# qirui-chen/RGA3-release

Hardware: AMD Instinct MI355X
Metric: video-QA samples/sec (fwd+bwd) at 7B/16-frame — full RGA3 training step (Qwen2.5-VL-7B + SAM2-L + mask losses + AdamW) (higher is better)
Workload: dtype bf16

## Files before the change

### include/rga3_hip.h

```cpp
#ifndef RGA3_HIP_H
#define RGA3_HIP_H

#include <stddef.h>
#include <stdint.h>

#ifdef __cplusplus
extern "C" {
#endif

#define RGA3_EINVAL (-22)

#define RGA3_BF16 0
#define RGA3_F32 1

#define RGA3_ACT_NONE 0
#define RGA3_ACT_GELU 1
#define RGA3_ACT_SWIGLU 2
#define RGA3_ACT_RELU 3

int rga3_version(void);
int rga3_last_error(char* buf, size_t n);

int rga3_gemm_bf16(const void* A, const void* W, const void* bias, const void* residual, const void* colscale, void* C, int64_t M, int64_t N,
                   int64_t K, int64_t lda, int64_t ldw, int64_t ldc, int64_t ldr, int act, int out_dtype, int tile,
                   void* workspace, int64_t workspace_bytes, void* stream);
int rga3_gemm_rms_bf16(const void* A, const void* W, const void* bias, const void* residual, void* C, int64_t M, int64_t N, int64_t K, int64_t lda,
                       int64_t ldw, int64_t ldc, int64_t ldr, int act, int tile, void* workspace, int64_t workspace_bytes, const uint64_t* row_sumsq_in,
                       int64_t norm_width, float eps, uint64_t* row_sumsq_out, void* stream);
int rga3_gemm_swiglu_pre_bf16(const void* A, const void* W, const void* bias, void* C, void* pre, int64_t M, int64_t N, int64_t K, int64_t lda, int64_t ldw,
                              int64_t ldc, int64_t ldpre, int tile, void* workspace, int64_t workspace_bytes, void* stream);
int rga3_gemm_cat_bf16(const void* A, const void* W, const void* bias, void* C, int64_t M, int64_t N, int64_t K, int64_t lda, int64_t ldw, int64_t ldc,
                       const void* A2, const void* W2, int64_t K2, int64_t lda2, int64_t ldw2, const void* Wn, void* Cn, int64_t N2, int64_t ldwn, int64_t ldcn,
                       int tile, void* stream);

int64_t rga3_gemm_workspace_bytes(void);
int rga3_gemm_tn_bf16(const void* A, const void* B, const void* bias, void* C, int64_t M, int64_t N, int64_t K, int64_t lda, int64_t ldb,
                      int64_t ldc, int out_dtype, void* workspace, int64_t workspace_bytes, void* counters, void* stream);
int rga3_gemm_tn_many(const void* const* ptrs, const int64_t* dims, int n, void* workspace, int64_t workspace_bytes, void* stream);


int rga3_attn_varlen_fwd(const void* q, const void* k, const void* v, void* o, float* lse, const int32_t* cu_q,
                         const int32_t* cu_k, int nseg, int max_q, int64_t total_q, int Hq, int Hkv, int D, int64_t q_st, int64_t q_sh,
                         int64_t k_st, int64_t k_sh, int64_t v_st, int64_t v_sh, int64_t o_st, int64_t o_sh,
                         float scale, int causal, int impl, float* split_ws, int64_t split_ws_elems, int max_k, int block_q, int block_k, void* stream);
int rga3_attn_varlen_fwd_rope(const void* q, const void* k, const void* v, void* o, float* lse, const int32_t* cu_q, const int32_t* cu_k, int nseg, int max_q,
                              int64_t total_q, int Hq, int Hkv, int D, int64_t q_st, int64_t q_sh, int64_t k_st, int64_t k_sh, int64_t v_st, int64_t v_sh,
                              int64_t o_st, int64_t o_sh, float scale, int causal, const float* cos_q, const float* sin_q, const float* cos_k,
                              const float* sin_k, void* stream);

int rga3_rmsnorm_fwd(const void* x, const void* add, const void* weight, void* y, void* res_out, int64_t rows,
                     int64_t dim, int64_t ldx, float eps, void* stream);

int rga3_layernorm_fwd(const void* x, const void* weight, const void* bias, void* y, int64_t rows, int64_t dim,
                       int64_t ldx, int64_t ldy, float eps, int act, void* stream);
int rga3_layernorm_stats(const void* x, float* stats, int64_t rows, int64_t dim, int64_t ldx, float eps, void* stream);
int rga3_gemm_ln_bf16(const void* A, const void* Wf, const void* bias, const float* colc, const float* rowstat, void* C, int64_t M, int64_t N, int64_t K,
                      int64_t lda, int64_t ldw, int64_t ldc, int act, int tile, void* stream);
int64_t rga3_gemm_lnsum_slices(int64_t N, int tile);
int rga3_gemm_lnsum_bf16(const void* A, const void* W, const void* bias, const void* residual, void* C, int64_t M, int64_t N, int64_t K, int64_t lda,
                         int64_t ldw, int64_t ldc, int64_t ldr, int tile, float* row_parts, void* stream);
int rga3_gemm_lnq_bf16(const void* A, const void* Wf, const void* bias, const float* colc, const float* row_parts, int64_t slices, int64_t norm_width, float eps,
                       void* C, int64_t M, int64_t N, int64_t K, int64_t lda, int64_t ldw, int64_t ldc, int act, int tile, void* stream);

int rga3_rope_inplace(void* x, const float* cos, const float* sin, int64_t T, int h0, int nh, int D, int64_t st,
                      int64_t sh, void* stream);

int rga3_gather_rows(const void* table, const int64_t* idx, void* out, int64_t n_idx, int64_t rows_per_idx,
                     int64_t dim, int64_t ld_table, int64_t ld_out, void* stream);
int rga3_scatter_rows(const void* src, const int64_t* idx, void* out, int64_t n_idx, int64_t rows_per_idx, int64_t dim,
                      int64_t ld_src, int64_t ld_out, void* stream);

int rga3_pad_cols(const void* src, void* dst, int64_t rows, int64_t cols, int64_t ld_src, int64_t ld_dst, void* stream);

int rga3_silu_mul(const void* a, const void* b, void* out, int64_t n, void* stream);
int rga3_add(const void* a, const void* b, void* out, int64_t n, void* stream);

int rga3_cross_entropy_rows(const void* logits, int logits_dtype, const int64_t* labels, float* row_loss,
                            void* dlogits, int64_t rows, int64_t V, int64_t ld, float grad_scale, void* stream);


int rga3_im2col(const void* img, void* out, int64_t F, int C, int H, int W, int ks, int stride, int pad, int64_t ld_out,
                void* stream);
int rga3_maxpool2x2_win(const void* x, void* y, int64_t nwin, int w, int C, int64_t ldx, int64_t ldy, void* stream);
int rga3_upsample2x_add(const void* a, const void* b, void* out, int64_t F, int H, int W, int C, void* stream);
int rga3_add_bcast(const void* a, const void* b, void* out, int64_t rows, int64_t rows_b, int C, int64_t lda, int64_t ldb,
                   int64_t ldo, float alpha, void* stream);
int rga3_bilinear(const void* in, int in_dtype, float* out, const int32_t* plane_idx, int64_t N, int Hi, int Wi, int Ho, int Wo,
                  void* stream);
int rga3_conv3x3s2(const void* x, int x_dtype, const void* w, const void* bias, void* y, int64_t F, int H, int W, int Cin, int Cout,
                   float sig_scale, float sig_bias, void* stream);
int rga3_decimg_rows(const void* keys, int64_t keys_stride, const void* pe, int64_t pe_stride, int hw, const void* kt, const void* vt, int nk, const void* wq, const void* bq,
                     const void* wo, const void* bo, const void* ln_w, const void* ln_b, float eps, const void* wk2, const void* bk2, const void* wv2, const void* bv2,
                     void* keys_out, int64_t keys_out_stride, void* k2, void* v2, int64_t kv_stride, int v2_transposed, float scale, int64_t M, void* stream);
int rga3_attn_fewq(const void* q, int64_t q_stride, const void* k, int64_t k_stride, int64_t k_head_stride, const void* vt, const void* vbias, void* out, int64_t out_stride,
                   int frames, int nq, int nk, int H, float scale, void* stream);
int rga3_copy_many(void* const* dst, const void* const* src, const int64_t* bytes, int n, void* stream);
int rga3_conv3x3s2_ln_gelu(const void* x, int x_dtype, const void* w, const void* bias, const void* ln_w, const void* ln_b, float eps, void* y, int64_t F, int H, int W,
                           int Cin, int Cout, float sig_scale, float sig_bias, void* stream);
int rga3_im2col3x3s2(const void* x, void* cols, int64_t F, int H, int W, int C, void* stream);
int rga3_dwconv7x7(const void* x, const void* w, const void* bias, void* y, int64_t F, int H, int W, int C, void* stream);
int rga3_rope_axial_inplace(void* x, const float* cos, const float* sin, int64_t n_rope, int nq, int C, int64_t ldx, void* stream);
int rga3_pixel_shuffle2x(const void* g, const void* bias, const void* add, void* out, int64_t F, int H, int W, int Co, int act, void* stream);
int rga3_bce_dice_sums(const float* logits, const float* targets, float* out4, int64_t n_masks, int64_t hw, void* stream);
int64_t rga3_bce_dice_sums_ws_floats(int64_t n_masks, int64_t hw);
int rga3_bce_dice_sums_det(const float* logits, const float* targets, float* out4, float* ws, int64_t ws_floats, int64_t n_masks, int64_t hw, void* stream);


int rga3_attn_varlen_bwd(const void* q, const void* k, const void* v, const void* o, const void* dout, const float* lse, void* dq,
                         void* dk, void* dv, float* delta_ws, const int32_t* cu_q, const int32_t* cu_k, int nseg, int max_q,
                         int max_k, int64_t total_q, int Hq, int Hkv, int D, const int64_t* strides16, float scale, int causal,
                         float* dkv_ws, int64_t total_k, void* stream);
int rga3_hiera_mlp144(const void* x, const void* w1f, const float* c1, const void* d1, const void* w2, const void* b2, void* y, int64_t M, float eps, void* stream);
int64_t rga3_hiera_mlp288_pack_bytes(void);
int rga3_hiera_mlp288_pack(const void* w1f, const float* c1, const void* d1, const void* w2, void* pack, void* stream);
int rga3_hiera_mlp288(const void* x, const void* pack, const void* b2, void* y, int64_t M, float eps, void* stream);
int rga3_mlp3_rows(const void* const* ptrs, const int64_t* dims, int n, int64_t B, void* stream);
int rga3_sam_select_objptr(const void* iou, const void* obj, const void* toks, int64_t tok_bstride, int C, const void* w0, const void* b0, const void* w1, const void* b1,
                           const void* w2, const void* b2, const void* no_obj_ptr, int64_t* best, int32_t* sel, void* obj_ptr, int64_t B, void* stream);
int64_t rga3_memattn_cross_ws_floats(int64_t Nq, int nsplit);
int rga3_memattn_cross(const void* q, const void* k, const void* m, void* out, int64_t Nq, int64_t Nk, int64_t q_stride, int64_t k_stride, int64_t m_stride,
                       int64_t out_stride, float scale, int nsplit, float* ws, void* stream);
int rga3_memlayer_rows(const void* a, int64_t a_stride, int K1, const float* part_o, const float* part_ml, int nsplit, const void* w1, const void* b1,
                       const void* res, int64_t res_stride, void* x_out, int64_t x_stride, const void* ln_w, const void* ln_b, float eps, void* t_out,
                       int64_t t_stride, const void* w2, const void* b2, int N2, void* y_out, int64_t y_stride, const float* cos, const float* sin,
                       int rope_cols, int nq, int64_t M, void* stream);
int rga3_gemm_rows16_many(const void* const* ptrs, const int64_t* dims, int n, void* stream);
int rga3_gemm_stream_k_timeouts(const void* workspace);
int64_t rga3_gemm_timeout_counter_offset(void);
int rga3_gemm_ragged_plan(int64_t M, int64_t N, int64_t K, int cus, int split, int* plan, unsigned* start);
int rga3_rmsnorm_bwd(const void* x, const void* weight, const void* dy, const void* add, void* dx, int64_t rows, int64_t dim, float eps,
                     void* stream);
int rga3_dropout_bf16(const void* x, void* y, int64_t n, float p, int64_t seed, int accumulate, void* stream);
int rga3_dropout_pair_bf16(const void* xa, const void* xb, void* ya, void* yb, int64_t n, float pa, int64_t seed_a, float pb, int64_t seed_b, int sum, void* stream);
int rga3_swiglu_fwd(const void* gu, void* a, int64_t T, int64_t I, void* stream);
int rga3_swiglu_bwd(const void* gu, const void* da, void* dgu, int64_t T, int64_t I, void* stream);
int rga3_transpose16(const void* in, void* out, int64_t R, int64_t C, int64_t ld_in, int64_t ld_out, void* stream);
int rga3_transpose16_many(const void* const* ptrs, const int64_t* dims, int n, void* stream);
int rga3_segment_sum_rows(const void* x, const int64_t* rows, const int64_t* offsets, void* out, int64_t n_out, int64_t dim, int64_t ldx,
                          void* stream);
int rga3_adamw_step(void* param, float* master, const void* grad, float* m, float* v, int64_t n, float lr, float beta1, float beta2,
                    float eps, float weight_decay, int step, float grad_scale, void* stream);
int rga3_sumsq_accum(const void* g, float* out, int64_t n, void* stream);
int rga3_sumsq_det(const void* g, int64_t n, float* partials, int64_t partials_cap, float* out, int accumulate, void* stream);
int rga3_adamw_step_clip(void* param, float* master, const void* grad, float* m, float* v, int64_t n, float lr, float beta1, float beta2,
                         float eps, float weight_decay, int step, const float* sumsq, float max_norm, void* stream);
int rga3_adamw_step_clip_rows(void* param, float* master, const void* grad, float* m, float* v, int64_t rows, int64_t row_len, const uint8_t* row_active,
                              float lr, float beta1, float beta2, float eps, int step, const float* sumsq, float max_norm, void* stream);
int rga3_scatter_add_rows(void* dst, const int64_t* idx, const void* src, int64_t n, int64_t dim, int64_t ld_dst, int64_t ld_src, float scale,
                          void* stream);


int64_t rga3_layernorm_bwd_ws_floats(int64_t rows, int64_t dim);
int rga3_layernorm_bwd(const void* x, const void* weight, const void* dy, void* dx, float* dweight, float* dbias, int64_t rows, int64_t dim,
                       float eps, float* ws, int64_t ws_floats, void* stream);
int rga3_colsum_accum(const void* x, float* out, int64_t rows, int64_t cols, int64_t ld, void* stream);
int64_t rga3_colsum_ws_floats(int64_t rows, int64_t cols);
int rga3_colsum(const void* x, float* out, int64_t rows, int64_t cols, int64_t ld, float* ws, int64_t ws_floats, void* counters, void* stream);
int rga3_act(const void* a, const void* dy, void* out, int64_t n, int kind, void* stream);
int rga3_bilinear_bwd(const float* dout, float* din, const int32_t* plane_idx, int64_t N, int Hi, int Wi, int Ho, int Wo, void* stream);
int rga3_mask_product(const void* hyper, const void* up, float* masks, int64_t B, int64_t NM, int64_t P, int64_t C, void* stream);
int64_t rga3_mask_product_bwd_ws_floats(int64_t B, int64_t NM, int64_t P, int64_t C);
int rga3_mask_product_bwd(const float* dmasks, const void* hyper, const void* up, void* dup, void* dhyper, int64_t B, int64_t NM, int64_t P, int64_t C,
                          float* ws, int64_t ws_floats, void* stream);
int rga3_pixel_shuffle2x_bwd(const void* dout, void* dg, int64_t F, int H, int W, int Co, void* stream);
int rga3_bce_dice_grad(const float* logits, const float* targets, const float* sums4, float* dlogits, int64_t n_masks, int64_t hw,
                       float coef_bce, float coef_dice, void* stream);
int rga3_bce_dice_grad_dev(const float* logits, const float* targets, const float* sums4, float* dlogits, int64_t n_masks, int64_t hw,
                           const float* coef_bce_dev, const float* coef_dice_dev, void* stream);

int rga3_pil_bicubic_coeffs(int in_size, int out_size, int32_t* bounds, int32_t* kk, int64_t kk_capacity, int* ksize_out);
int rga3_sam_preprocess_u8(const void* frames, int64_t T, int H, int W, int out_h, int out_w, const int32_t* bh, const int32_t* kh,
                           int ksize_h, const int32_t* bv, const int32_t* kv, int ksize_v, void* tmp, void* dst_u8, void* dst_bf16,
                           const float* mean3, const float* std3, void* stream);

int rga3_qwen_norm_lut(const float* mean3, const float* std3, int fused, float* lut768);
int rga3_qwen_patchify_u8(const void* frames, int64_t T, int h, int w, const float* lut768, void* out, int out_dtype, int patch, int tpatch,
                          int merge, void* stream);

int rga3_quant_fp8_rows(const void* x, void* q, float* scales, int64_t rows, int64_t K, int64_t ldx, int64_t ldq, void* stream);
int rga3_gemm_fp8(const void* Aq, const void* Wq, const float* sa, const float* sw, const void* bias, const void* residual, void* C, int64_t M,
                  int64_t N, int64_t K, int64_t lda, int64_t ldw, int64_t ldc, int64_t ldr, void* stream);
int rga3_swiglu_fwd_quant_fp8(const void* gu, void* q, float* scales, int64_t T, int64_t I, void* stream);
int rga3_swiglu_bwd_quant_fp8(const void* gu, const void* da, void* q, float* scales, int64_t T, int64_t I, void* stream);

#ifdef __cplusplus
}
#endif
#endif
```

### rga3-release_amd/csrc/attn_bwd.hip

```cpp
#include "common.h"

#include <mutex>
#include <set>

namespace rga3 {

struct AttnBwdArgs {
    const unsigned short *q, *k, *v, *o, *dout;
    unsigned short *dq, *dk, *dv;
    const float* lse;
    float* delta;
    const int *cu_q, *cu_k;
    long q_st, q_sh, k_st, k_sh, v_st, v_sh, o_st, o_sh, do_st, do_sh, dq_st, dq_sh, dk_st, dk_sh, dv_st, dv_sh;
    int Hq, Hkv, D;
    long total_q;
    float scale, scale_log2;
    int causal;
    float* dkv_ws;
    long total_k;
    int gx, gy;
};

constexpr int BT = 64;

template <int DP, int QT, int NWAVE, bool PAIR>
__global__ __launch_bounds__(64 * NWAVE) void attn_bwd_dq_kernel(AttnBwdArgs p) {
    constexpr int NT = 64 * NWAVE;
    constexpr int BLOCK_M = NWAVE * QT * 16;
    constexpr int CH = DP / 8;
    constexpr int STRIDE = DP * 2 + 32;
    constexpr int DS = DP / 32, DT = DP / 16;
    constexpr int LOADS = (BT * CH) / NT;
    static_assert((BT * CH) % NT == 0, "tile chunks must divide evenly over threads");

    extern __shared__ __attribute__((aligned(16))) char smem[];
    char* Ks = smem;
    char* Vs = smem + BT * STRIDE;

    const int tid = threadIdx.x, lane = tid & 63;
    const int wid = __builtin_amdgcn_readfirstlane(tid >> 6);
    const int g = lane >> 4, c = lane & 15;
    const Wg3 wg = xcd_decode3(p.gx, p.gy);
    const int seg = wg.z, hq = wg.y;
    const int hk = hq / (p.Hq / p.Hkv);
    const int qs = p.cu_q[seg], Lq = p.cu_q[seg + 1] - qs;
    const int ks = p.cu_k[seg], Lk = p.cu_k[seg + 1] - ks;
    const int shift = Lk - Lq;
    const int nqb = (Lq + BLOCK_M - 1) / BLOCK_M;
    int qb_first = wg.x, qb_second = -1;
    if constexpr (PAIR) {
        qb_first = nqb - 1 - wg.x;
        qb_second = wg.x;
        if (qb_second > qb_first) return;
        if (qb_second == qb_first) qb_second = -1;
    } else if (qb_first >= nqb) {
        return;
    }
    for (int pass = 0; pass < (PAIR ? 2 : 1); ++pass) {
    const int qbi = pass == 0 ? qb_first : qb_second;
    if (qbi < 0) break;
    if (pass == 1) __syncthreads();
    const int qb0 = qbi * BLOCK_M;
    const int qw0 = qb0 + wid * (QT * 16);

    bf16x8 qf[QT][DS], dof[QT][DS];
    float lse2[QT], dl[QT];
#pragma unroll
    for (int t = 0; t < QT; ++t) {
        const int qi = qw0 + t * 16 + c;
        const bool ok = qi < Lq;
#pragma unroll
        for (int ds = 0; ds < DS; ++ds) {
            const int d = ds * 32 + g * 8;
            u32x4 z = {0u, 0u, 0u, 0u}, y = {0u, 0u, 0u, 0u};
            if (ok && d < p.D) {
                z = *(const u32x4*)(p.q + (long)(qs + qi) * p.q_st + (long)hq * p.q_sh + d);
                y = *(const u32x4*)(p.dout + (long)(qs + qi) * p.do_st + (long)hq * p.do_sh + d);
            }
            qf[t][ds] = __builtin_bit_cast(bf16x8, z);
            dof[t][ds] = __builtin_bit_cast(bf16x8, y);
        }
        lse2[t] = ok ? p.lse[(long)hq * p.total_q + qs + qi] * 1.4426950408889634f : 0.f;
    }
#pragma unroll
    for (int t = 0; t < QT; ++t) {
        const int qi = qw0 + t * 16 + c;
        const bool ok = qi < Lq;
        float dp = 0.f;
#pragma unroll
        for (int ds = 0; ds < DS; ++ds) {
            const int d = ds * 32 + g * 8;
            if (ok && d < p.D) {
                const u32x4 ov = *(const u32x4*)(p.o + (long)(qs + qi) * p.o_st + (long)hq * p.o_sh + d);
                const u32x4 dv = __builtin_bit_cast(u32x4, dof[t][ds]);
#pragma unroll
                for (int i = 0; i < 4; ++i) {
                    dp += __uint_as_float(ov[i] << 16) * __uint_as_float(dv[i] << 16);
                    dp += __uint_as_float(ov[i] & 0xffff0000u) * __uint_as_float(dv[i] & 0xffff0000u);
                }
            }
        }
        dp += __shfl_xor(dp, 16, 64);
        dp += __shfl_xor(dp, 32, 64);
        dl[t] = ok ? dp : 0.f;
        if (ok && g == 0) p.delta[(long)hq * p.total_q + qs + qi] = dp;
    }

    f32x4 dqacc[QT][DT];
#pragma unroll
    for (int t = 0; t < QT; ++t)
#pragma unroll
        for (int d = 0; d < DT; ++d) dqacc[t][d] = f32x4{0.f, 0.f, 0.f, 0.f};

    int kv_end = Lk;
    if (p.causal) kv_end = min(Lk, qb0 + BLOCK_M + shift);
    if (kv_end < 0) kv_end = 0;
    const int ntiles = (kv_end + BT - 1) / BT;

    u32x4 kreg[LOADS], vreg[LOADS];
    auto load_tile = [&](int kt) {
#pragma unroll
        for (int i = 0; i < LOADS; ++i) {
            const int idx = tid + i * NT;
            const int r = idx / CH, ch = idx % CH;
            const int key = kt * BT + r;
            u32x4 zk = {0u, 0u, 0u, 0u}, zv = {0u, 0u, 0u, 0u};
            if (key < Lk && ch * 8 < p.D) {
                zk = *(const u32x4*)(p.k + (long)(ks + key) * p.k_st + (long)hk * p.k_sh + ch * 8);
                zv = *(const u32x4*)(p.v + (long)(ks + key) * p.v_st + (long)hk * p.v_sh + ch * 8);
            }
            kreg[i] = zk;
            vreg[i] = zv;
        }
    };
    auto store_tile = [&]() {
#pragma unroll
        for (int i = 0; i < LOADS; ++i) {
            const int idx = tid + i * NT;
            const int r = idx / CH, ch = idx % CH;
            *(u32x4*)(Ks + r * STRIDE + ch * 16) = kreg[i];
            *(u32x4*)(Vs + r * STRIDE + ch * 16) = vreg[i];
        }
    };

    if (ntiles > 0) load_tile(0);
    for (int kt = 0; kt < ntiles; ++kt) {
        __syncthreads();
        store_tile();
        __syncthreads();
        if (kt + 1 < ntiles) load_tile(kt + 1);
        const int k0 = kt * BT;
        const bool need_mask = (k0 + BT > Lk) || (p.causal && (k0 + BT - 1 > qb0 + shift));
#pragma unroll
        for (int t = 0; t < QT; ++t) {
            const int qi = qw0 + t * 16 + c;
            f32x4 s[4], dp[4];
#pragma unroll
            for (int j = 0; j < 4; ++j) { s[j] = f32x4{0.f, 0.f, 0.f, 0.f}; dp[j] = f32x4{0.f, 0.f, 0.f, 0.f}; }
#pragma unroll
            for (int j = 0; j < 4; ++j)
#pragma unroll
                for (int ds = 0; ds < DS; ++ds) {
                    bf16x8 kf = *(const bf16x8*)(Ks + (j * 16 + c) * STRIDE + ds * 64 + g * 16);
                    bf16x8 vf = *(const bf16x8*)(Vs + (j * 16 + c) * STRIDE + ds * 64 + g * 16);
                    s[j] = __builtin_amdgcn_mfma_f32_16x16x32_bf16(kf, qf[t][ds], s[j], 0, 0, 0);
                    dp[j] = __builtin_amdgcn_mfma_f32_16x16x32_bf16(vf, dof[t][ds], dp[j], 0, 0, 0);
                }
            bf16x8 dsf[2];
#pragma unroll
            for (int ss = 0; ss < 2; ++ss) {
                float e[8];
#pragma unroll
                for (int u = 0; u < 8; ++u) {
                    const int j = 2 * ss + (u >> 2), r = u & 3;
                    float pr = __builtin_amdgcn_exp2f(s[j][r] * p.scale_log2 - lse2[t]);
                    if (need_mask) {
                        const int key = k0 + j * 16 + 4 * g + r;
                        const bool ok = (key < Lk) && (!p.causal || key <= qi + shift);
                        pr = ok ? pr : 0.f;
                    }
                    if (qi >= Lq) pr = 0.f;
                    e[u] = pr * (dp[j][r] - dl[t]) * p.scale;
                }
                u32x4 pk;
                pk[0] = pack_bf2(e[0], e[1]); pk[1] = pack_bf2(e[2], e[3]); pk[2] = pack_bf2(e[4], e[5]); pk[3] = pack_bf2(e[6], e[7]);
                dsf[ss] = __builtin_bit_cast(bf16x8, pk);
            }
#pragma unroll
            for (int d = 0; d < DT; ++d)
#pragma unroll
                for (int ss = 0; ss < 2; ++ss) {
                    const char* a0 = Ks + (ss * 32 + 4 * g + (c >> 2)) * STRIDE + (d * 16 + 4 * (c & 3)) * 2;
                    bf16x4 lo = __builtin_amdgcn_ds_read_tr16_b64_v4bf16((__attribute__((address_space(3))) bf16x4*)(a0));
                    bf16x4 hi = __builtin_amdgcn_ds_read_tr16_b64_v4bf16((__attribute__((address_space(3))) bf16x4*)(a0 + 16 * STRIDE));
                    bf16x8 kt8;
                    kt8[0] = lo[0]; kt8[1] = lo[1]; kt8[2] = lo[2]; kt8[3] = lo[3];
                    kt8[4] = hi[0]; kt8[5] = hi[1]; kt8[6] = hi[2]; kt8[7] = hi[3];
                    dqacc[t][d] = __builtin_amdgcn_mfma_f32_16x16x32_bf16(kt8, dsf[ss], dqacc[t][d], 0, 0, 0);
                }
        }
    }
#pragma unroll
    for (int t = 0; t < QT; ++t) {
        const int qi = qw0 + t * 16 + c;
        if (qi < Lq) {
            unsigned short* row = p.dq + (long)(qs + qi) * p.dq_st + (long)hq * p.dq_sh;
#pragma unroll
            for (int d = 0; d < DT; ++d) {
                const int dd = d * 16 + 4 * g;
                if (dd < p.D) {
                    u32x2 pk;
                    pk[0] = pack_bf2(dqacc[t][d][0], dqacc[t][d][1]);
                    pk[1] = pack_bf2(dqacc[t][d][2], dqacc[t][d][3]);
                    *(u32x2*)(row + dd) = pk;
                }
            }
        }
    }
    }
}

template <int DP, int NWAVE, bool SPLIT, bool PAIR>
__global__ __launch_bounds__(64 * NWAVE) void attn_bwd_dkv_kernel(AttnBwdArgs p) {
    constexpr int NT = 64 * NWAVE;
    constexpr int BLOCK_N = NWAVE * 16;
    constexpr int CH = DP / 8;
    constexpr int STRIDE = DP * 2 + 32;
    constexpr int DS = DP / 32, DT = DP / 16;
    constexpr int LOADS = (BT * CH) / NT;
    static_assert((BT * CH) % NT == 0, "tile chunks must divide evenly over threads");

    extern __shared__ __attribute__((aligned(16))) char smem[];
    char* Qs = smem;
    char* Os = smem + BT * STRIDE;
    float* Ls = (float*)(smem + 2 * BT * STRIDE);

    const int tid = threadIdx.x, lane = tid & 63;
    const int wid = __builtin_amdgcn_readfirstlane(tid >> 6);
    const int g = lane >> 4, c = lane & 15;
    const Wg3 wg = xcd_decode3(p.gx, p.gy);
    const int seg = wg.z;
    const int group = p.Hq / p.Hkv;
    const int hk = SPLIT ? wg.y / group : wg.y;
    const int hh0 = SPLIT ? wg.y % group : 0, hh1 = SPLIT ? hh0 + 1 : group;
    const int qs = p.cu_q[seg], Lq = p.cu_q[seg + 1] - qs;
    const int ks = p.cu_k[seg], Lk = p.cu_k[seg + 1] - ks;
    const int shift = Lk - Lq;
    const int nkb = (Lk + BLOCK_N - 1) / BLOCK_N;
    int kb_first = wg.x, kb_second = -1;
    if constexpr (PAIR) {
        kb_first = wg.x;
        kb_second = nkb - 1 - wg.x;
        if (kb_first > kb_second) return;
        if (kb_second == kb_first) kb_second = -1;
    } else if (kb_first >= nkb) {
        return;
    }
    for (int pass = 0; pass < (PAIR ? 2 : 1); ++pass) {
    const int kbi = pass == 0 ? kb_first : kb_second;
    if (kbi < 0) break;
    if (pass == 1) __syncthreads();
    const int kb0 = kbi * BLOCK_N;
    const int key = kb0 + wid * 16 + c;

    bf16x8 kf[DS], vf[DS];
#pragma unroll
    for (int ds = 0; ds < DS; ++ds) {
        const int d = ds * 32 + g * 8;
        u32x4 z = {0u, 0u, 0u, 0u}, y = {0u, 0u, 0u, 0u};
        if (key < Lk && d < p.D) {
            z = *(const u32x4*)(p.k + (long)(ks + key) * p.k_st + (long)hk * p.k_sh + d);
            y = *(const u32x4*)(p.v + (long)(ks + key) * p.v_st + (long)hk * p.v_sh + d);
        }
        kf[ds] = __builtin_bit_cast(bf16x8, z);
        vf[ds] = __builtin_bit_cast(bf16x8, y);
    }
    f32x4 dkacc[DT], dvacc[DT];
#pragma unroll
    for (int d = 0; d < DT; ++d) { dkacc[d] = f32x4{0.f, 0.f, 0.f, 0.f}; dvacc[d] = f32x4{0.f, 0.f, 0.f, 0.f}; }

    int q_begin = 0;
    if (p.causal) q_begin = max(0, kb0 - shift);
    const int t0 = q_begin / BT;
    const int ntq = (Lq + BT - 1) / BT;

    u32x4 qreg[LOADS], oreg[LOADS];
    float lreg = 0.f, dreg = 0.f;
    auto load_tile = [&](int hq_, int qt_) {
#pragma unroll
        for (int i = 0; i < LOADS; ++i) {
            const int idx = tid + i * NT;
            const int r = idx / CH, ch = idx % CH;
            const int qi = qt_ * BT + r;
            u32x4 zq = {0u, 0u, 0u, 0u}, zo = {0u, 0u, 0u, 0u};
            if (qi < Lq && ch * 8 < p.D) {
                zq = *(const u32x4*)(p.q + (long)(qs + qi) * p.q_st + (long)hq_ * p.q_sh + ch * 8);
                zo = *(const u32x4*)(p.dout + (long)(qs + qi) * p.do_st + (long)hq_ * p.do_sh + ch * 8);
            }
            qreg[i] = zq;
            oreg[i] = zo;
        }
        if (tid < BT) {
            const int qi = qt_ * BT + tid;
            lreg = (qi < Lq) ? p.lse[(long)hq_ * p.total_q + qs + qi] * 1.4426950408889634f : 0.f;
            dreg = (qi < Lq) ? p.delta[(long)hq_ * p.total_q + qs + qi] : 0.f;
        }
    };
    auto store_tile = [&]() {
#pragma unroll
        for (int i = 0; i < LOADS; ++i) {
            const int idx = tid + i * NT;
            const int r = idx / CH, ch = idx % CH;
            *(u32x4*)(Qs + r * STRIDE + ch * 16) = qreg[i];
            *(u32x4*)(Os + r * STRIDE + ch * 16) = oreg[i];
        }
        if (tid < BT) {
            Ls[tid] = lreg;
            Ls[BT + tid] = dreg;
        }
    };
    if (t0 < ntq) load_tile(hk * group + hh0, t0);
    for (int hh = hh0; hh < hh1; ++hh) {
        const int hq = hk * group + hh;
        for (int qt = t0; qt < ntq; ++qt) {
            __syncthreads();
            store_tile();
            __syncthreads();
            if (qt + 1 < ntq) load_tile(hq, qt + 1);
            else if (hh + 1 < hh1) load_tile(hq + 1, t0);
            const int q0 = qt * BT;
            f32x4 s[4], dp[4];
#pragma unroll
            for (int j = 0; j < 4; ++j) { s[j] = f32x4{0.f, 0.f, 0.f, 0.f}; dp[j] = f32x4{0.f, 0.f, 0.f, 0.f}; }
#pragma unroll
            for (int j = 0; j < 4; ++j)
#pragma unroll
                for (int ds = 0; ds < DS; ++ds) {
                    bf16x8 qa = *(const bf16x8*)(Qs + (j * 16 + c) * STRIDE + ds * 64 + g * 16);
                    bf16x8 oa = *(const bf16x8*)(Os + (j * 16 + c) * STRIDE + ds * 64 + g * 16);
                    s[j] = __builtin_amdgcn_mfma_f32_16x16x32_bf16(qa, kf[ds], s[j], 0, 0, 0);
                    dp[j] = __builtin_amdgcn_mfma_f32_16x16x32_bf16(oa, vf[ds], dp[j], 0, 0, 0);
                }
            bf16x8 pf[2], dsf[2];
#pragma unroll
            for (int ss = 0; ss < 2; ++ss) {
                float e[8], f[8];
#pragma unroll
                for (int u = 0; u < 8; ++u) {
                    const int j = 2 * ss + (u >> 2), r = u & 3;
                    const int ql = j * 16 + 4 * g + r;
                    const int qi = q0 + ql;
                    float pr = __builtin_amdgcn_exp2f(s[j][r] * p.scale_log2 - Ls[ql]);
                    const bool ok = (qi < Lq) && (key < Lk) && (!p.causal || key <= qi + shift);
                    pr = ok ? pr : 0.f;
                    e[u] = pr;
                    f[u] = pr * (dp[j][r] - Ls[BT + ql]) * p.scale;
                }
                u32x4 a, b;
                a[0] = pack_bf2(e[0], e[1]); a[1] = pack_bf2(e[2], e[3]); a[2] = pack_bf2(e[4], e[5]); a[3] = pack_bf2(e[6], e[7]);
                b[0] = pack_bf2(f[0], f[1]); b[1] = pack_bf2(f[2], f[3]); b[2] = pack_bf2(f[4], f[5]); b[3] = pack_bf2(f[6], f[7]);
                pf[ss] = __builtin_bit_cast(bf16x8, a);
                dsf[ss] = __builtin_bit_cast(bf16x8, b);
            }
#pragma unroll
            for (int d = 0; d < DT; ++d)
#pragma unroll
                for (int ss = 0; ss < 2; ++ss) {
                    const int roff = (ss * 32 + 4 * g + (c >> 2)) * STRIDE + (d * 16 + 4 * (c & 3)) * 2;
                    bf16x4 ol = __builtin_amdgcn_ds_read_tr16_b64_v4bf16((__attribute__((address_space(3))) bf16x4*)(Os + roff));
                    bf16x4 oh = __builtin_amdgcn_ds_read_tr16_b64_v4bf16((__attribute__((address_space(3))) bf16x4*)(Os + roff + 16 * STRIDE));
                    bf16x4 ql_ = __builtin_amdgcn_ds_read_tr16_b64_v4bf16((__attribute__((address_space(3))) bf16x4*)(Qs + roff));
                    bf16x4 qh_ = __builtin_amdgcn_ds_read_tr16_b64_v4bf16((__attribute__((address_space(3))) bf16x4*)(Qs + roff + 16 * STRIDE));
                    bf16x8 ot, qt8;
                    ot[0] = ol[0]; ot[1] = ol[1]; ot[2] = ol[2]; ot[3] = ol[3]; ot[4] = oh[0]; ot[5] = oh[1]; ot[6] = oh[2]; ot[7] = oh[3];
                    qt8[0] = ql_[0]; qt8[1] = ql_[1]; qt8[2] = ql_[2]; qt8[3] = ql_[3]; qt8[4] = qh_[0]; qt8[5] = qh_[1]; qt8[6] = qh_[2]; qt8[7] = qh_[3];
                    dvacc[d] = __builtin_amdgcn_mfma_f32_16x16x32_bf16(ot, pf[ss], dvacc[d], 0, 0, 0);
                    dkacc[d] = __builtin_amdgcn_mfma_f32_16x16x32_bf16(qt8, dsf[ss], dkacc[d], 0, 0, 0);
                }
        }
    }
    if constexpr (SPLIT) {
        if (key < Lk) {
            const long half = (long)group * p.total_k * p.Hkv * p.D;
            float* wk = p.dkv_ws + (((long)hh0 * p.total_k + ks + key) * p.Hkv + hk) * p.D;
#pragma unroll
            for (int d = 0; d < DT; ++d) {
                const int dd = d * 16 + 4 * g;
                if (dd < p.D) {
                    *(f32x4*)(wk + dd) = dkacc[d];
                    *(f32x4*)(wk + half + dd) = dvacc[d];
                }
            }
        }
        continue;
    }
    if (key < Lk) {
        unsigned short* rk = p.dk + (long)(ks + key) * p.dk_st + (long)hk * p.dk_sh;
        unsigned short* rv = p.dv + (long)(ks + key) * p.dv_st + (long)hk * p.dv_sh;
#pragma unroll
        for (int d = 0; d < DT; ++d) {
            const int dd = d * 16 + 4 * g;
            if (dd < p.D) {
                u32x2 a, b;
                a[0] = pack_bf2(dkacc[d][0], dkacc[d][1]); a[1] = pack_bf2(dkacc[d][2], dkacc[d][3]);
                b[0] = pack_bf2(dvacc[d][0], dvacc[d][1]); b[1] = pack_bf2(dvacc[d][2], dvacc[d][3]);
                *(u32x2*)(rk + dd) = a;
                *(u32x2*)(rv + dd) = b;
            }
        }
    }
    }
}

__global__ __launch_bounds__(256) void attn_dkv_reduce_kernel(AttnBwdArgs p) {
    const int group = p.Hq / p.Hkv;
    const int d4 = p.D / 4;
    const long idx = (long)blockIdx.x * 256 + threadIdx.x;
    const long total = p.total_k * p.Hkv * d4;
    if (idx >= total) return;
    const int dd = (int)(idx % d4) * 4;
    const long row = idx / d4;
    const int hk = (int)(row % p.Hkv);
    const long key = row / p.Hkv;
    const long plane = p.total_k * p.Hkv * (long)p.D, half = (long)group * plane;
    const float* w = p.dkv_ws + row * p.D + dd;
    f32x4 sk = *(const f32x4*)w, sv = *(const f32x4*)(w + half);
    for (int h = 1; h < group; ++h) {
        sk += *(const f32x4*)(w + h * plane);
        sv += *(const f32x4*)(w + half + h * plane);
    }
    u32x2 a, b;
    a[0] = pack_bf2(sk[0], sk[1]); a[1] = pack_bf2(sk[2], sk[3]);
    b[0] = pack_bf2(sv[0], sv[1]); b[1] = pack_bf2(sv[2], sv[3]);
    *(u32x2*)(p.dk + key * p.dk_st + (long)hk * p.dk_sh + dd) = a;
    *(u32x2*)(p.dv + key * p.dv_st + (long)hk * p.dv_sh + dd) = b;
}

template <int DP>
static int launch_bwd(const AttnBwdArgs& a0, int nseg, int max_q, int max_k, hipStream_t st) {
    AttnBwdArgs a = a0;
    a.gx = 1; a.gy = 1;
    constexpr int NW = (DP == 128) ? 8 : 4;
#ifdef RGA3_BWD_DQ_QT2
    constexpr int QT = 2, NWQ = 4;
#else
    constexpr int QT = (DP >= 128) ? 1 : 2, NWQ = NW;
#endif
    constexpr int BLOCK_M = NWQ * QT * 16;
    constexpr int LDS_DQ = 2 * BT * (DP * 2 + 32);
    constexpr int LDS_DKV = 2 * BT * (DP * 2 + 32) + 2 * BT * 4;
    auto prep = [](const void* k, int lds) -> int {
        if (lds <= 48 * 1024) return 0;
        static std::mutex mu;
        static std::set<std::pair<const void*, int>> done;
        int dev = 0;
        if (hipGetDevice(&dev) != hipSuccess) dev = 0;
        std::lock_guard<std::mutex> lk(mu);
        if (done.count({k, dev})) return 0;
        hipError_t e = hipFuncSetAttribute(k, hipFuncAttributeMaxDynamicSharedMemorySize, lds);
        if (e != hipSuccess) return fail(-(int)e, "attn_bwd: hipFuncSetAttribute: %s", hipGetErrorString(e));
        done.insert({k, dev});
        return 0;
    };
    const unsigned nqb = (unsigned)cdiv(max_q, BLOCK_M), nkb = (unsigned)cdiv(max_k, 16 * NW);
    const bool pair = a.causal && nqb >= 4 && nkb >= 4;
    if (pair) {
        auto kq = attn_bwd_dq_kernel<DP, QT, NWQ, true>;
        if (int rc = prep((const void*)kq, LDS_DQ)) return rc;
        a.gx = (int)((nqb + 1) / 2); a.gy = a.Hq;
        hipLaunchKernelGGL(kq, dim3((unsigned)a.gx * (unsigned)a.gy * (unsigned)nseg), dim3(64 * NWQ), LDS_DQ, st, a);
    } else {
        auto kq = attn_bwd_dq_kernel<DP, QT, NWQ, false>;
        if (int rc = prep((const void*)kq, LDS_DQ)) return rc;
        a.gx = (int)nqb; a.gy = a.Hq;
        hipLaunchKernelGGL(kq, dim3((unsigned)a.gx * (unsigned)a.gy * (unsigned)nseg), dim3(64 * NWQ), LDS_DQ, st, a);
    }
    RGA3_CHECK_LAUNCH("attn_bwd_dq_kernel");
    const unsigned gx = pair ? (nkb + 1) / 2 : nkb;
    if (a.dkv_ws && a.Hq > a.Hkv) {
        if (pair) {
            auto ks_ = attn_bwd_dkv_kernel<DP, NW, true, true>;
            if (int rc = prep((const void*)ks_, LDS_DKV)) return rc;
            a.gx = (int)gx; a.gy = a.Hq;
            hipLaunchKernelGGL(ks_, dim3((unsigned)a.gx * (unsigned)a.gy * (unsigned)nseg), dim3(64 * NW), LDS_DKV, st, a);
        } else {
            auto ks_ = attn_bwd_dkv_kernel<DP, NW, true, false>;
            if (int rc = prep((const void*)ks_, LDS_DKV)) return rc;
            a.gx = (int)gx; a.gy = a.Hq;
            hipLaunchKernelGGL(ks_, dim3((unsigned)a.gx * (unsigned)a.gy * (unsigned)nseg), dim3(64 * NW), LDS_DKV, st, a);
        }
        RGA3_CHECK_LAUNCH("attn_bwd_dkv_kernel<split>");
        const long rows = a.total_k * a.Hkv;
        hipLaunchKernelGGL(attn_dkv_reduce_kernel, dim3((unsigned)cdiv(rows * (a.D / 4), 256)), dim3(256), 0, st, a);
        RGA3_CHECK_LAUNCH("attn_dkv_reduce_kernel");
        return 0;
    }
    if (pair) {
        auto kk = attn_bwd_dkv_kernel<DP, NW, false, true>;
        if (int rc = prep((const void*)kk, LDS_DKV)) return rc;
        a.gx = (int)gx; a.gy = a.Hkv;
        hipLaunchKernelGGL(kk, dim3((unsigned)a.gx * (unsigned)a.gy * (unsigned)nseg), dim3(64 * NW), LDS_DKV, st, a);
    } else {
        auto kk = attn_bwd_dkv_kernel<DP, NW, false, false>;
        if (int rc = prep((const void*)kk, LDS_DKV)) return rc;
        a.gx = (int)gx; a.gy = a.Hkv;
        hipLaunchKernelGGL(kk, dim3((unsigned)a.gx * (unsigned)a.gy * (unsigned)nseg), dim3(64 * NW), LDS_DKV, st, a);
    }
    RGA3_CHECK_LAUNCH("attn_bwd_dkv_kernel");
    return 0;
}

}

using namespace rga3;

extern "C" int rga3_attn_varlen_bwd(const void* q, const void* k, const void* v, const void* o, const void* dout, const float* lse,
                                    void* dq, void* dk, void* dv, float* delta_ws, const int32_t* cu_q, const int32_t* cu_k, int nseg,
                                    int max_q, int max_k, int64_t total_q, int Hq, int Hkv, int D, const int64_t* strides16, float scale,
                                    int causal, float* dkv_ws, int64_t total_k, void* stream) {
    RGA3_CHECK_ARG(q && k && v && o && dout && lse && dq && dk && dv && delta_ws && cu_q && cu_k && strides16, "attn_bwd: null pointer");
    RGA3_CHECK_ARG(nseg > 0 && max_q > 0 && max_k > 0 && total_q > 0, "attn_bwd: sizes");
    RGA3_CHECK_ARG(Hq > 0 && Hkv > 0 && Hq % Hkv == 0, "attn_bwd: Hq=%d Hkv=%d", Hq, Hkv);
    RGA3_CHECK_ARG(D >= 8 && D <= 128 && D % 8 == 0, "attn_bwd: head dim %d unsupported (multiple of 8, <= 128)", D);
    for (int i = 0; i < 16; ++i) RGA3_CHECK_ARG(strides16[i] % 4 == 0, "attn_bwd: stride %d must be a multiple of 4 elements", i);
    for (int i = 0; i < 10; ++i) RGA3_CHECK_ARG(strides16[i] % 8 == 0, "attn_bwd: input stride %d must be a multiple of 8 elements", i);
    AttnBwdArgs a;
    a.q = (const unsigned short*)q; a.k = (const unsigned short*)k; a.v = (const unsigned short*)v; a.o = (const unsigned short*)o;
    a.dout = (const unsigned short*)dout; a.dq = (unsigned short*)dq; a.dk = (unsigned short*)dk; a.dv = (unsigned short*)dv;
    a.lse = lse; a.delta = delta_ws; a.cu_q = cu_q; a.cu_k = cu_k;
    a.q_st = strides16[0]; a.q_sh = strides16[1]; a.k_st = strides16[2]; a.k_sh = strides16[3]; a.v_st = strides16[4]; a.v_sh = strides16[5];
    a.o_st = strides16[6]; a.o_sh = strides16[7]; a.do_st = strides16[8]; a.do_sh = strides16[9]; a.dq_st = strides16[10]; a.dq_sh = strides16[11];
    a.dk_st = strides16[12]; a.dk_sh = strides16[13]; a.dv_st = strides16[14]; a.dv_sh = strides16[15];
    a.Hq = Hq; a.Hkv = Hkv; a.D = D; a.total_q = total_q; a.scale = scale; a.scale_log2 = scale * 1.4426950408889634f; a.causal = causal;
    a.dkv_ws = dkv_ws; a.total_k = total_k;
    RGA3_CHECK_ARG(!dkv_ws || (total_k > 0 && D % 4 == 0), "attn_bwd: dkv_ws needs total_k");
    hipStream_t st = (hipStream_t)stream;
    if (D <= 32) return launch_bwd<32>(a, nseg, max_q, max_k, st);
    if (D <= 64) return launch_bwd<64>(a, nseg, max_q, max_k, st);
    if (D <= 96) return launch_bwd<96>(a, nseg, max_q, max_k, st);
    return launch_bwd<128>(a, nseg, max_q, max_k, st);
}
```

### rga3-release_amd/csrc/gemm_bf16.hip

```cpp
#include "common.h"
#include "act_table.h"
#include <cstdlib>
#include <type_traits>
#include <utility>

namespace rga3 {


enum { ACT_NONE = 0, ACT_GELU = 1, ACT_SWIGLU = 2, ACT_RELU = 3 };

struct GemmArgs {
    const unsigned short* A;
    const unsigned short* W;
    void* C;
    const unsigned short* bias;
    const unsigned short* res;
    const unsigned short* colscale;
    int M, N, K;
    long lda, ldw, ldc, ldr;
    int ntm, ntn;
    int group_m;
    void* ws;
    long ws_bytes;
    const float* rowstat;
    const float* colc;
    int ksl;
    const unsigned long long* rs_in = nullptr;
    float rs_in_scale = 0.f;
    float rs_eps = 0.f;
    unsigned long long* rs_out = nullptr;
    float* ln_parts = nullptr;
    const float* ln_in = nullptr;
    int ln_ns = 0;
    const unsigned short* A2 = nullptr;
    const unsigned short* W2 = nullptr;
    long lda2 = 0, ldw2 = 0;
    int K2 = 0;
    unsigned short* pre = nullptr;
    long ldpre = 0;
    const unsigned short* Wn = nullptr;
    void* Cn = nullptr;
    long ldwn = 0, ldcn = 0;
    int N2 = 0;
};

constexpr float kRowSumFix = 1048576.0f;

__device__ const u32x4 g_zero16 = {0u, 0u, 0u, 0u};

__device__ __forceinline__ float gelu_erf(float x) {
    const float z = fabsf(x) * 0.70710678118654752f;
    const float t = __builtin_amdgcn_rcpf(1.0f + 0.3275911f * z);
    float poly = 1.061405429f;
    poly = poly * t - 1.453152027f;
    poly = poly * t + 1.421413741f;
    poly = poly * t - 0.284496736f;
    poly = poly * t + 0.254829592f;
    const float e = 1.0f - poly * t * __expf(-z * z);
    return 0.5f * x + 0.5f * fabsf(x) * e;
}
__device__ __forceinline__ float silu_f(float x) { return x * __builtin_amdgcn_rcpf(1.0f + __expf(-x)); }

template <int ACT> constexpr bool act_uses_table() { return ACT == ACT_GELU || ACT == ACT_SWIGLU; }

__device__ __forceinline__ f32x2 splat2(float s) {
    f32x2 v = {s, s};
    asm volatile("" : "+v"(v));
    return v;
}
__device__ __forceinline__ f32x2 widen_bf2(unsigned pk) { return f32x2{__uint_as_float(pk << 16), __uint_as_float(pk & 0xffff0000u)}; }
template <int NWAVES>
__device__ __forceinline__ void stage_act_table(char* dst, int which, int wid, int lane) {
    const char* src = (const char*)g_act_tab[which] + lane * 16;
#pragma unroll
    for (int pc = 0; pc < kActTabBytes / 1024; pc += NWAVES) {
        const int q = pc + wid;
        if (q < kActTabBytes / 1024) __builtin_amdgcn_global_load_lds((gbl_void*)(src + q * 1024), (lds_void*)(dst + q * 1024), 16, 0, 0);
    }
}

template <int NTL, int ACT, bool OUT_F32>
constexpr int epi_wave_bytes() {
    return 1024;
}

template <int ACT, bool OUT_F32>
constexpr bool pp_res_lds() { return ACT == ACT_NONE && !OUT_F32; }
template <int MT, int OW>
constexpr int res_stage_bytes() { return ((MT * 16 * (OW / 8 + 1) * 16 + 1023) / 1024) * 1024; }

template <int MT, int OW>
__device__ __forceinline__ void stage_residual(const GemmArgs& p, char* dst, int row0, int col0, int lane) {
    constexpr int CPR = OW / 8, CPRP = CPR + 1, SLOTS = MT * 16 * CPRP, NI = (SLOTS + 63) / 64;
#pragma unroll
    for (int k = 0; k < NI; ++k) {
        const int sl = min(k * 64 + lane, SLOTS - 1);
        const int row = sl / CPRP, ch = min(sl - row * CPRP, CPR - 1);
        const unsigned short* src = p.res + (long)min(row0 + row, p.M - 1) * p.ldr + col0 + ch * 8;
        __builtin_amdgcn_global_load_lds((gbl_void*)src, (lds_void*)(dst + k * 1024), 16, 0, 0);
    }
}
template <int OW, bool OUT_F32>
__device__ __forceinline__ bool residual_stageable(const GemmArgs& p, int col0, int Nout) {
    return !OUT_F32 && p.res && col0 + OW <= Nout && (p.ldr & 7) == 0 && (p.ldc & 7) == 0 && ((((size_t)p.res) & 15) == 0);
}

template <int MT, int NTL, int WTM, int WTN, int ACT, bool OUT_F32, int LNM = 0, bool PARTS = false>
__device__ __forceinline__ void gemm_epilogue(f32x4 (&acc)[MT][NTL], const GemmArgs& p, char* est, const char* tab, int lane, int m0, int n0,
                                              int wm, int wn, const f32x4* part1 = nullptr, const f32x4* part2 = nullptr, const char* resl = nullptr,
                                              float poison = 0.f, int nwn = 1) {
    constexpr bool LNF = LNM == 1, LNP = LNM == 2;
    static_assert(!(LNM != 0 && ACT == ACT_SWIGLU), "the LayerNorm-folded epilogues have no SwiGLU form");
    static_assert(!(LNP && (OUT_F32 || PARTS)), "the LayerNorm-sum producer writes bf16 from the single-pass kernels");
    constexpr int PD = 1;
    f32x4 pn[PD][NTL];
    auto load_part = [&](int i) {
#pragma unroll
        for (int j = 0; j < NTL; ++j) {
            f32x4 v = part1[(i * NTL + j) * 64];
            if (part2) v += part2[(i * NTL + j) * 64];
            v += f32x4{poison, poison, poison, poison};
            pn[i % PD][j] = v;
        }
    };
    if constexpr (PARTS) {
        load_part(0);
        if (PD > 1 && MT > 1) load_part(1);
    }
    auto load4 = [&](const unsigned short* v, int col, int n) -> u32x2 {
        u32x2 r;
        if (col + 3 < n && (((size_t)(v + col)) & 7) == 0) {
            r = *(const u32x2*)(v + col);
        } else {
            const unsigned a0 = v[min(col, n - 1)], a1 = v[min(col + 1, n - 1)], a2 = v[min(col + 2, n - 1)], a3 = v[min(col + 3, n - 1)];
            r[0] = a0 | (a1 << 16);
            r[1] = a2 | (a3 << 16);
        }
        return r;
    };
    auto pick = [](const u32x2& pk, int r) -> float { return __uint_as_float((r & 1) ? (pk[r >> 1] & 0xffff0000u) : (pk[r >> 1] << 16)); };
    u32x2 bpk[NTL];
    f32x4 cc[LNF ? NTL : 1];
    {
        const int g4 = (lane >> 4) * 4;
        if (p.bias) {
            if (n0 + wn * WTN + NTL * 16 <= p.N && (((size_t)p.bias) & 7) == 0) {
#pragma unroll
                for (int j = 0; j < NTL; ++j) bpk[j] = *(const u32x2*)(p.bias + n0 + wn * WTN + j * 16 + g4);
            } else {
#pragma unroll
                for (int j = 0; j < NTL; ++j) bpk[j] = load4(p.bias, n0 + wn * WTN + j * 16 + g4, p.N);
            }
        }
        if constexpr (LNF) {
#pragma unroll
            for (int j = 0; j < NTL; ++j) {
                const int col = n0 + wn * WTN + j * 16 + g4;
                cc[j] = (col + 3 < p.N) ? *(const f32x4*)(p.colc + col) : f32x4{0.f, 0.f, 0.f, 0.f};
            }
        }
    }

    constexpr int OUT_NT = (ACT == ACT_SWIGLU) ? NTL / 2 : NTL;
    constexpr int OW = OUT_NT * 16;
    constexpr int ESZ = OUT_F32 ? 4 : 2;
    constexpr int EDAT = OW * ESZ;
    constexpr int EROW = EDAT + 16;
    const int g = lane >> 4, c = lane & 15;
    const int ncol0 = (ACT == ACT_SWIGLU) ? (n0 / 2 + wn * OW) : (n0 + wn * OW);
    const int Nout = (ACT == ACT_SWIGLU) ? p.N / 2 : p.N;

    float* const rs_lds = (float*)est;
    const unsigned tb = act_uses_table<ACT>() ? act_tab_base(tab) : 0u;
    if constexpr (LNF) {
        if (p.ln_in) {
            const double sc = (double)p.rs_in_scale;
#pragma unroll
            for (int q = 0; q < (MT * 16 + 63) / 64; ++q) {
                const int rl = lane + 64 * q;
                if (rl < MT * 16) {
                    const float2* pp = (const float2*)p.ln_in + (long)min(m0 + wm * WTM + rl, p.M - 1) * p.ln_ns;
                    double sx = 0.0, sxx = 0.0;
                    for (int k = 0; k < p.ln_ns; ++k) {
                        const float2 v = pp[k];
                        sx += (double)v.x;
                        sxx += (double)v.y;
                    }
                    const double mean = sx * sc;
                    const double var = fmax(sxx * sc - mean * mean, 0.0);
                    *(float2*)(rs_lds + 2 * rl) = make_float2((float)mean, __builtin_amdgcn_rsqf((float)var + p.rs_eps));
                }
            }
        } else {
#pragma unroll
            for (int q = 0; q < (MT * 16 + 63) / 64; ++q) {
                const int rl = lane + 64 * q;
                if (rl < MT * 16) *(float2*)(rs_lds + 2 * rl) = *(const float2*)(p.rowstat + 2L * min(m0 + wm * WTM + rl, p.M - 1));
            }
        }
    }
    if (p.rs_in) {
#pragma unroll
        for (int q = 0; q < (MT * 16 + 63) / 64; ++q) {
            const int rl = lane + 64 * q;
            if (rl < MT * 16) {
                const uint2 raw = *(const uint2*)(p.rs_in + min(m0 + wm * WTM + rl, p.M - 1));
                rs_lds[rl] = __builtin_amdgcn_rsqf(__builtin_fmaf((float)raw.y, 4294967296.0f, (float)raw.x) * p.rs_in_scale + p.rs_eps);
            }
        }
    }
    if (resl) asm volatile("s_waitcnt vmcnt(0)" ::: "memory");
#pragma unroll
    for (int i = 0; i < MT; ++i) {
        f32x4 x[NTL];
#pragma unroll
        for (int j = 0; j < NTL; ++j) {
            x[j] = acc[i][j];
            if constexpr (PARTS) x[j] += pn[i % PD][j];
        }
        if constexpr (PARTS) {
            if (i + PD < MT) load_part(i + PD);
        }
        if constexpr (LNF) {
            const float2 st2 = *(const float2*)(rs_lds + 2 * (i * 16 + (lane & 15)));
            const float ln_rinv = st2.y, nmr = -st2.x * st2.y;
            const f32x2 ri2 = splat2(ln_rinv), nm2 = splat2(nmr);
#pragma unroll
            for (int j = 0; j < NTL; ++j) {
                const f32x2 lo = x[j].xy * ri2 + cc[j].xy * nm2, hi = x[j].zw * ri2 + cc[j].zw * nm2;
                x[j] = f32x4{lo[0], lo[1], hi[0], hi[1]};
            }
        } else if (p.rs_in) {
            const float rs_rinv = rs_lds[i * 16 + (lane & 15)];
            const f32x2 rs2 = splat2(rs_rinv);
#pragma unroll
            for (int j = 0; j < NTL; ++j) {
                const f32x2 lo = x[j].xy * rs2, hi = x[j].zw * rs2;
                x[j] = f32x4{lo[0], lo[1], hi[0], hi[1]};
            }
        }
        if (p.bias) {
#pragma unroll
            for (int j = 0; j < NTL; ++j)
                x[j] += f32x4{__uint_as_float(bpk[j][0] << 16), __uint_as_float(bpk[j][0] & 0xffff0000u), __uint_as_float(bpk[j][1] << 16),
                              __uint_as_float(bpk[j][1] & 0xffff0000u)};
        }
        f32x4 v[OUT_NT];
#pragma unroll
        for (int jo = 0; jo < OUT_NT; ++jo) {
            if constexpr (ACT == ACT_SWIGLU) {
                const f32x4 &gq = x[2 * jo], &uq = x[2 * jo + 1];
                const unsigned pg0 = pack_bf2(gq[0], gq[1]), pg1 = pack_bf2(gq[2], gq[3]), pu0 = pack_bf2(uq[0], uq[1]), pu1 = pack_bf2(uq[2], uq[3]);
                const f32x2 s01 = act_tab2(pg0, tb), s23 = act_tab2(pg1, tb);
                const f32x2 v01 = widen_bf2(pack_bf2(s01[0], s01[1])) * widen_bf2(pu0);
                const f32x2 v23 = widen_bf2(pack_bf2(s23[0], s23[1])) * widen_bf2(pu1);
                v[jo] = f32x4{v01[0], v01[1], v23[0], v23[1]};
                if (p.pre) {
                    const auto q0 = __builtin_amdgcn_permlane16_swap(pg0, pu0, false, false);
                    const auto q1 = __builtin_amdgcn_permlane16_swap(pg1, pu1, false, false);
                    const u32x4 pv = {(unsigned)q0[0], (unsigned)q1[0], (unsigned)q0[1], (unsigned)q1[1]};
                    const int prow = m0 + wm * WTM + i * 16 + (lane & 15);
                    const int pcol = n0 + wn * WTN + ((g & 1) ? (2 * jo + 1) * 16 + 4 * (g - 1) : 2 * jo * 16 + 4 * g);
                    if (prow < p.M && pcol < p.N) {
                        unsigned short* dp = p.pre + (long)prow * p.ldpre + pcol;
                        if (pcol + 8 <= p.N && (p.ldpre & 7) == 0) {
                            *(u32x4*)dp = pv;
                        } else {
                            for (int e = 0; e < 8 && pcol + e < p.N; ++e) dp[e] = (unsigned short)(pv[e >> 1] >> (16 * (e & 1)));
                        }
                    }
                }
            } else if constexpr (ACT == ACT_GELU) {
                const f32x2 y01 = act_tab2(pack_bf2(x[jo][0], x[jo][1]), tb), y23 = act_tab2(pack_bf2(x[jo][2], x[jo][3]), tb);
                v[jo] = f32x4{y01[0], y01[1], y23[0], y23[1]};
            } else if constexpr (ACT == ACT_RELU) {
#pragma unroll
                for (int r = 0; r < 4; ++r) v[jo][r] = fmaxf(x[jo][r], 0.f);
            } else {
                v[jo] = x[jo];
            }
        }
        if (p.colscale) {
#pragma unroll
            for (int jo = 0; jo < OUT_NT; ++jo)
#pragma unroll
                for (int r = 0; r < 4; ++r) {
                    const float cs = bf2f(p.colscale[min(ncol0 + jo * 16 + 4 * g + r, Nout - 1)]);
                    v[jo][r] = ((ACT == ACT_SWIGLU) ? v[jo][r] : bf2f(f2bf(v[jo][r]))) * cs;
                }
        }
        u32x2 pk[OUT_NT];
        f32x4 vf[OUT_F32 ? OUT_NT : 1];
#pragma unroll
        for (int jo = 0; jo < OUT_NT; ++jo) {
            if constexpr (OUT_F32) {
                vf[jo] = v[jo];
            } else {
                pk[jo][0] = pack_bf2(v[jo][0], v[jo][1]);
                pk[jo][1] = pack_bf2(v[jo][2], v[jo][3]);
            }
        }
        const int row = m0 + wm * WTM + i * 16 + c;
        const bool row_ok = row < p.M;
        if constexpr (OUT_F32) {
#pragma unroll
            for (int jo = 0; jo < OUT_NT; ++jo) {
                const int col = ncol0 + jo * 16 + 4 * g;
                if (row_ok && col < Nout) {
                    float* dst = (float*)p.C + (long)row * p.ldc + col;
                    if (col + 4 <= Nout && ((p.ldc & 3) == 0)) {
                        *(f32x4*)dst = vf[jo];
                    } else {
                        for (int e = 0; e < 4 && col + e < Nout; ++e) dst[e] = vf[jo][e];
                    }
                }
            }
        } else {
            float rs_ss = 0.f, rs_s = 0.f;
#pragma unroll
            for (int jo = 0; jo + 1 < OUT_NT; jo += 2) {
                const auto r0 = __builtin_amdgcn_permlane16_swap(pk[jo][0], pk[jo + 1][0], false, false);
                const auto r1 = __builtin_amdgcn_permlane16_swap(pk[jo][1], pk[jo + 1][1], false, false);
                u32x4 val = {(unsigned)r0[0], (unsigned)r1[0], (unsigned)r0[1], (unsigned)r1[1]};
                const int col = ncol0 + ((g & 1) ? (jo + 1) * 16 + 4 * (g - 1) : jo * 16 + 4 * g);
                if (row_ok && col < Nout) {
                    unsigned short* dst = (unsigned short*)p.C + (long)row * p.ldc + col;
                    const bool vec = (col + 8 <= Nout) && ((p.ldc & 7) == 0);
                    if (p.res) {
                        const unsigned short* rs = p.res + (long)row * p.ldr + col;
                        u32x4 rv;
                        if (resl) {
                            rv = *(const u32x4*)(resl + (((i * 16 + c) * (OW / 8 + 1) + ((col - ncol0) >> 3)) << 4));
                        } else if (vec && ((p.ldr & 7) == 0) && ((((size_t)p.res) & 15) == 0)) {
                            rv = *(const u32x4*)rs;
                        } else {
#pragma unroll
                            for (int e = 0; e < 4; ++e) {
                                const unsigned lo = (col + 2 * e < Nout) ? rs[2 * e] : 0u, hi = (col + 2 * e + 1 < Nout) ? rs[2 * e + 1] : 0u;
                                rv[e] = lo | (hi << 16);
                            }
                        }
#pragma unroll
                        for (int e = 0; e < 4; ++e)
                            val[e] = pack_bf2(__uint_as_float(val[e] << 16) + __uint_as_float(rv[e] << 16),
                                              __uint_as_float(val[e] & 0xffff0000u) + __uint_as_float(rv[e] & 0xffff0000u));
                    }
                    if (vec) {
                        *(u32x4*)dst = val;
                    } else {
                        for (int e = 0; e < 8 && col + e < Nout; ++e) dst[e] = (unsigned short)(val[e >> 1] >> (16 * (e & 1)));
                    }
                    if (LNP || p.rs_out) {
#pragma unroll
                        for (int e = 0; e < 8; ++e) {
                            const float v1 = (col + e < Nout) ? __uint_as_float((e & 1) ? (val[e >> 1] & 0xffff0000u) : (val[e >> 1] << 16)) : 0.f;
                            rs_ss = __builtin_fmaf(v1, v1, rs_ss);
                            if constexpr (LNP) rs_s += v1;
                        }
                    }
                }
            }
            if constexpr (OUT_NT % 2 == 1) {
            const int col = ncol0 + (OUT_NT - 1) * 16 + 4 * g;
            if (row_ok && col < Nout) {
                u32x2 val = pk[OUT_NT - 1];
                unsigned short* dst = (unsigned short*)p.C + (long)row * p.ldc + col;
                if (p.res && resl) {
                    const u32x2 rv = *(const u32x2*)(resl + (((i * 16 + c) * (OW / 8 + 1) + ((col - ncol0) >> 3)) << 4) + (((col - ncol0) & 4) << 1));
#pragma unroll
                    for (int e = 0; e < 2; ++e)
                        val[e] = pack_bf2(__uint_as_float(val[e] << 16) + __uint_as_float(rv[e] << 16), __uint_as_float(val[e] & 0xffff0000u) + __uint_as_float(rv[e] & 0xffff0000u));
                } else if (p.res) {
                    const unsigned short* rs = p.res + (long)row * p.ldr + col;
#pragma unroll
                    for (int e = 0; e < 2; ++e) {
                        const float lo = (col + 2 * e < Nout) ? bf2f(rs[2 * e]) : 0.f, hi = (col + 2 * e + 1 < Nout) ? bf2f(rs[2 * e + 1]) : 0.f;
                        val[e] = pack_bf2(__uint_as_float(val[e] << 16) + lo, __uint_as_float(val[e] & 0xffff0000u) + hi);
                    }
                }
                if (col + 4 <= Nout && ((p.ldc & 3) == 0)) {
                    *(u32x2*)dst = val;
                } else {
                    for (int e = 0; e < 4 && col + e < Nout; ++e) dst[e] = (unsigned short)(val[e >> 1] >> (16 * (e & 1)));
                }
                if (LNP || p.rs_out) {
#pragma unroll
                    for (int e = 0; e < 4; ++e) {
                        const float v1 = (col + e < Nout) ? __uint_as_float((e & 1) ? (val[e >> 1] & 0xffff0000u) : (val[e >> 1] << 16)) : 0.f;
                        rs_ss = __builtin_fmaf(v1, v1, rs_ss);
                        if constexpr (LNP) rs_s += v1;
                    }
                }
            }
            }
            if constexpr (LNP) {
                rs_ss += __shfl_xor(rs_ss, 16, 64);
                rs_ss += __shfl_xor(rs_ss, 32, 64);
                rs_s += __shfl_xor(rs_s, 16, 64);
// ... 1855 lines not shown
    __syncthreads();
    if (w != 0) return;
    f32x4 v = red[0][lane];
#pragma unroll
    for (int i = 1; i < R16_NW; ++i) v += red[i][lane];
    const int col = n0 + 4 * g;
    if (c >= p.M || col >= p.N) return;
    unsigned short* dst = (unsigned short*)p.C + (long)c * p.ldc + col;
#pragma unroll
    for (int r = 0; r < 4; ++r) {
        if (col + r >= p.N) break;
        float x = v[r];
        if (p.bias) x += bf2f(p.bias[col + r]);
        if constexpr (ACT == ACT_GELU) x = gelu_erf(bf2f(f2bf(x)));
        if constexpr (ACT == ACT_RELU) x = fmaxf(x, 0.f);
        if (p.res) x = bf2f(f2bf(x)) + bf2f(p.res[(long)c * p.ldr + col + r]);
        dst[r] = f2bf(x);
    }
}

constexpr int R16_MAXSETS = 4;
struct Rows16Set {
    const unsigned short *A, *A2, *W, *bias, *res;
    unsigned short* C;
    int M, N, K, act;
    long lda, lda2, ldw, ldc, ldr;
};
struct Rows16Many { Rows16Set s[R16_MAXSETS]; };

__global__ __launch_bounds__(64 * R16_NW) void gemm_rows16_many_kernel(Rows16Many P) {
    __shared__ f32x4 red[R16_NW][64];
    const Rows16Set& p = P.s[blockIdx.y];
    const int n0 = blockIdx.x * 16;
    if (n0 >= p.N) return;
    const int lane = threadIdx.x & 63, w = threadIdx.x >> 6;
    const int c = lane & 15, g = lane >> 4;
    const unsigned short* arow = p.W + (long)min(n0 + c, p.N - 1) * p.ldw + g * 8;
    const unsigned short* brow = p.A + (long)min(c, p.M - 1) * p.lda + g * 8;
    const unsigned short* brow2 = p.A2 ? p.A2 + (long)min(c, p.M - 1) * p.lda2 + g * 8 : nullptr;
    const int nks = (p.K + 31) >> 5;
    f32x4 acc = {0.f, 0.f, 0.f, 0.f};
    for (int ks0 = w; ks0 < nks; ks0 += R16_NW * R16_U) {
        bf16x8 af[R16_U], bf[R16_U];
#pragma unroll
        for (int u = 0; u < R16_U; ++u) {
            const int k = (ks0 + u * R16_NW) * 32 + g * 8;
            u32x4 za = {0u, 0u, 0u, 0u}, zb = {0u, 0u, 0u, 0u};
            if (k < p.K) {
                za = *(const u32x4*)(arow + (ks0 + u * R16_NW) * 32);
                zb = *(const u32x4*)(brow + (ks0 + u * R16_NW) * 32);
                if (brow2) {
                    const u32x4 z2 = *(const u32x4*)(brow2 + (ks0 + u * R16_NW) * 32);
#pragma unroll
                    for (int e = 0; e < 4; ++e)
                        zb[e] = pack_bf2(__uint_as_float(zb[e] << 16) + __uint_as_float(z2[e] << 16), __uint_as_float(zb[e] & 0xffff0000u) + __uint_as_float(z2[e] & 0xffff0000u));
                }
            }
            af[u] = __builtin_bit_cast(bf16x8, za);
            bf[u] = __builtin_bit_cast(bf16x8, zb);
        }
#pragma unroll
        for (int u = 0; u < R16_U; ++u) acc = __builtin_amdgcn_mfma_f32_16x16x32_bf16(af[u], bf[u], acc, 0, 0, 0);
    }
    red[w][lane] = acc;
    __syncthreads();
    if (w != 0) return;
    f32x4 v = red[0][lane];
#pragma unroll
    for (int i = 1; i < R16_NW; ++i) v += red[i][lane];
    const int col = n0 + 4 * g;
    if (c >= p.M || col >= p.N) return;
    unsigned short* dst = p.C + (long)c * p.ldc + col;
#pragma unroll
    for (int r = 0; r < 4; ++r) {
        if (col + r >= p.N) break;
        float x = v[r];
        if (p.bias) x += bf2f(p.bias[col + r]);
        if (p.act == ACT_GELU) x = gelu_erf(bf2f(f2bf(x)));
        if (p.act == ACT_RELU) x = fmaxf(x, 0.f);
        if (p.res) x = bf2f(f2bf(x)) + bf2f(p.res[(long)c * p.ldr + col + r]);
        dst[r] = f2bf(x);
    }
}

template <int ACT, bool OUT_F32>
static int launch_rows16(const GemmArgs& a, hipStream_t st) {
    if constexpr (OUT_F32 || ACT == ACT_SWIGLU) {
        return fail(-1, "gemm: tile 41 (token rows) writes bf16 and has no SwiGLU form");
    } else {
        hipLaunchKernelGGL(gemm_rows16_kernel<ACT>, dim3((unsigned)cdiv(a.N, 16)), dim3(64 * R16_NW), 0, st, a);
        RGA3_CHECK_LAUNCH("gemm_rows16_kernel");
        return 0;
    }
}

static int pick_tile(int M, int N, int K, bool plain, int forced) {
    if (forced >= 0) return forced;
    if (plain && K >= 8192 && cdiv(M, 256) * cdiv(N, 256) <= 4 && K % 64 == 0) return 25;
    struct Cfg { int bm, bn, slots; double prior; };
    static const Cfg cfgs[3] = {{256, 256, 1, 1.00}, {256, 128, 1, 0.90}, {128, 128, 2, 0.78}};
    int best = 0;
    double bs = -1;
    for (int i = 0; i < 3; ++i) {
        double tiles = (double)cdiv(M, cfgs[i].bm) * (double)cdiv(N, cfgs[i].bn);
        double cap = 256.0 * cfgs[i].slots;
        double waves = (double)cdiv((int64_t)tiles, (int64_t)cap);
        double fill = tiles / (waves * cap);
        double useful = ((double)M * N) / (tiles * cfgs[i].bm * cfgs[i].bn);
        double s = fill * useful * cfgs[i].prior;
        if (s > bs) { bs = s; best = i; }
    }
    static const int ids[3] = {20, 11, 12};
    return ids[best];
}

template <int ACT, bool OUT_F32>
static int launch_act(const GemmArgs& a, int tile, hipStream_t st) {
    switch (tile) {
        case 3: return launch_cfg<128, 256, 2, 4, ACT, OUT_F32, 0>(a, st);
        case 4:
            if constexpr (ACT != ACT_SWIGLU) return launch_cfg<128, 320, 2, 4, ACT, OUT_F32, 0>(a, st);
            else return launch_cfg<128, 256, 2, 4, ACT, OUT_F32, 0>(a, st);
        case 5:
            if constexpr (ACT != ACT_SWIGLU) return launch_cfg<128, 192, 2, 4, ACT, OUT_F32, 0>(a, st);
            else return launch_cfg<128, 256, 2, 4, ACT, OUT_F32, 0>(a, st);
        case 6: return launch_cfg<128, 256, 2, 4, ACT, OUT_F32, 3>(a, st);
        case 7:
            if constexpr (ACT != ACT_SWIGLU) return launch_cfg<128, 192, 2, 4, ACT, OUT_F32, 3>(a, st);
            else return launch_cfg<128, 256, 2, 4, ACT, OUT_F32, 3>(a, st);
        case 8: return launch_cfg<128, 128, 2, 2, ACT, OUT_F32, 3>(a, st);
        case 10: return launch_cfg<256, 256, 2, 4, ACT, OUT_F32, 0>(a, st);
        case 13: return launch_cfg<64, 64, 2, 2, ACT, OUT_F32, 0>(a, st);
        case 14:
            if constexpr (ACT == ACT_NONE) return launch_split64<OUT_F32>(a, st);
            else return launch_cfg<64, 64, 2, 2, ACT, OUT_F32, 0>(a, st);
        case 20: return launch_pp<ACT, OUT_F32>(a, st);
        case 23:
            if constexpr (ACT == ACT_NONE) return launch_pp<ACT, OUT_F32, false, true>(a, st);
            else return launch_pp<ACT, OUT_F32>(a, st);
        case 21: return launch_sk<ACT, OUT_F32>(a, false, st);
        case 22: return launch_sk<ACT, OUT_F32>(a, true, st);
        case 26: return launch_sk<ACT, OUT_F32>(a, true, st, true);
        case 27: return launch_sk<ACT, OUT_F32>(a, false, st, true);
        case 31: return launch_sk<ACT, OUT_F32, 3>(a, false, st);
        case 32: return launch_sk<ACT, OUT_F32, 3>(a, true, st);
        case 25: return launch_splitk<ACT, OUT_F32>(a, st);
        case 28: return launch_w4<ACT, OUT_F32>(a, st);
        case 40: return launch_gemv<ACT, OUT_F32>(a, st);
        case 41: return launch_rows16<ACT, OUT_F32>(a, st);
        default: return launch_cfg<128, 128, 2, 2, ACT, OUT_F32, 0>(a, st);
    }
}

}

using namespace rga3;

extern "C" int rga3_gemm_rows16_many(const void* const* ptrs, const int64_t* dims, int n, void* stream) {
    RGA3_CHECK_ARG(ptrs && dims && n >= 1 && n <= R16_MAXSETS, "gemm_rows16_many: n %d (1..%d)", n, R16_MAXSETS);
    Rows16Many P;
    int64_t maxn = 0;
    for (int i = 0; i < n; ++i) {
        Rows16Set& s = P.s[i];
        const void* const* q = ptrs + 6 * i;
        const int64_t* d = dims + 9 * i;
        s.A = (const unsigned short*)q[0]; s.A2 = (const unsigned short*)q[1]; s.W = (const unsigned short*)q[2]; s.bias = (const unsigned short*)q[3];
        s.res = (const unsigned short*)q[4]; s.C = (unsigned short*)q[5];
        s.M = (int)d[0]; s.N = (int)d[1]; s.K = (int)d[2]; s.act = (int)d[3]; s.lda = d[4]; s.lda2 = d[5]; s.ldw = d[6]; s.ldc = d[7]; s.ldr = d[8];
        RGA3_CHECK_ARG(s.A && s.W && s.C && s.M >= 1 && s.M <= 16 && s.N >= 1 && s.K >= 8 && s.K % 8 == 0, "gemm_rows16_many: set %d: M %d (1..16), N %d, K %d", i, s.M, s.N, s.K);
        RGA3_CHECK_ARG(s.lda % 8 == 0 && s.ldw % 8 == 0 && (!s.A2 || s.lda2 % 8 == 0), "gemm_rows16_many: set %d: strides must be multiples of 8", i);
        RGA3_CHECK_ARG((((uintptr_t)s.A | (uintptr_t)s.A2 | (uintptr_t)s.W) & 15) == 0, "gemm_rows16_many: set %d: 16-byte alignment", i);
        RGA3_CHECK_ARG(s.act == ACT_NONE || s.act == ACT_GELU || s.act == ACT_RELU, "gemm_rows16_many: set %d: act %d", i, s.act);
        RGA3_CHECK_ARG(s.ldc >= s.N && (!s.res || s.ldr >= s.N), "gemm_rows16_many: set %d: ldc %ld / ldr %ld shorter than N %d (a residual row stride below N reads out of bounds)",
                       i, (long)s.ldc, (long)s.ldr, s.N);
        if (s.N > maxn) maxn = s.N;
    }
    hipLaunchKernelGGL(gemm_rows16_many_kernel, dim3((unsigned)cdiv(maxn, 16), (unsigned)n), dim3(64 * R16_NW), 0, (hipStream_t)stream, P);
    RGA3_CHECK_LAUNCH("gemm_rows16_many_kernel");
    return 0;
}

extern "C" int64_t rga3_gemm_workspace_bytes(void) {
    const int cus = cu_count();
    return cus > 0 ? (int64_t)(kSkFlagBytes + (size_t)cus * 512 * 32 * 16) : 0;
}

extern "C" int rga3_gemm_stream_k_timeouts(const void* workspace) {
    SkWorkspace ws;
    if (sk_workspace((void*)workspace, (int64_t)1 << 40, ws)) return -1;
    unsigned v = 0;
    if (hipDeviceSynchronize() != hipSuccess || hipMemcpy(&v, ws.flags + ws.P, sizeof(v), hipMemcpyDeviceToHost) != hipSuccess) return -1;
    return (int)(v > 0x7fffffffu ? 0x7fffffffu : v);
}

extern "C" int rga3_gemm_ragged_plan(int64_t M, int64_t N, int64_t K, int cus, int split, int* plan, unsigned* start) {
    RGA3_CHECK_ARG(M > 0 && N > 0 && K > 0 && K % 64 == 0 && cus > 0 && cus <= kSkMaxP && plan && start, "gemm_ragged_plan: M, N > 0, K a multiple of 64, 0 < cus <= %d", kSkMaxP);
    GemmArgs a{};
    a.M = (int)M; a.N = (int)N; a.K = (int)K;
    a.ntm = (int)cdiv(M, 256);
    a.ntn = (int)cdiv(N, 256);
    for (int i = 0; i < 8; ++i) plan[i] = 0;
    if (a.ntm < 2 || M - (int64_t)(a.ntm - 1) * 256 > 64) return 1;
    a.group_m = pick_group_m(a.ntm - 1, 256);
    SkArgs sk;
    if (!sk_plan_ragged(sk, a, (int)(K / 64), cus, split != 0)) return 1;
    plan[0] = sk.t_dp; plan[1] = sk.sk_tiles; plan[2] = sk.ragged; plan[3] = sk.rg_wgs; plan[4] = 0; plan[5] = sk.P; plan[6] = sk.P_sk; plan[7] = a.group_m;
    for (int w = 0; w <= cus; ++w) start[w] = sk.start[w];
    return 0;
}

extern "C" int64_t rga3_gemm_timeout_counter_offset(void) {
    const int cus = cu_count();
    if (cus <= 0 || cus * 4 + 16 > (int)kSkFlagBytes) return -1;
    return (int64_t)cus * 4;
}

static int gemm_bf16_impl(const void* A, const void* W, const void* bias, const void* residual, const void* colscale, void* C,
                          int64_t M, int64_t N, int64_t K, int64_t lda, int64_t ldw, int64_t ldc, int64_t ldr,
                          int act, int out_dtype, int tile, void* workspace, int64_t workspace_bytes, const unsigned long long* rs_in, int64_t rs_width, float rs_eps,
                          unsigned long long* rs_out, void* stream, void* pre = nullptr, int64_t ldpre = 0);

extern "C" int rga3_gemm_bf16(const void* A, const void* W, const void* bias, const void* residual, const void* colscale, void* C,
                              int64_t M, int64_t N, int64_t K, int64_t lda, int64_t ldw, int64_t ldc, int64_t ldr,
                              int act, int out_dtype, int tile, void* workspace, int64_t workspace_bytes, void* stream) {
    return gemm_bf16_impl(A, W, bias, residual, colscale, C, M, N, K, lda, ldw, ldc, ldr, act, out_dtype, tile, workspace, workspace_bytes, nullptr, 0, 0.f, nullptr, stream);
}

extern "C" int rga3_gemm_rms_bf16(const void* A, const void* W, const void* bias, const void* residual, void* C, int64_t M, int64_t N, int64_t K, int64_t lda,
                                  int64_t ldw, int64_t ldc, int64_t ldr, int act, int tile, void* workspace, int64_t workspace_bytes, const uint64_t* row_sumsq_in,
                                  int64_t norm_width, float eps, uint64_t* row_sumsq_out, void* stream) {
    RGA3_CHECK_ARG(row_sumsq_in || row_sumsq_out, "gemm_rms: neither row_sumsq_in nor row_sumsq_out given (use rga3_gemm_bf16)");
    RGA3_CHECK_ARG(!row_sumsq_in || (norm_width > 0 && eps >= 0.f), "gemm_rms: norm_width %ld eps %g", (long)norm_width, (double)eps);
    RGA3_CHECK_ARG((((uintptr_t)row_sumsq_in | (uintptr_t)row_sumsq_out) & 7) == 0, "gemm_rms: row sums must be 8-byte aligned");
    RGA3_CHECK_ARG(tile != 14 && tile != 25 && tile != 40 && tile != 41, "gemm_rms: tile %d has its own epilogue", tile);
    RGA3_CHECK_ARG(M > 16, "gemm_rms: M %ld (token-row products take the unfused route)", (long)M);
    return gemm_bf16_impl(A, W, bias, residual, nullptr, C, M, N, K, lda, ldw, ldc, ldr, act, RGA3_BF16, tile, workspace, workspace_bytes,
                          (const unsigned long long*)row_sumsq_in, norm_width, eps, (unsigned long long*)row_sumsq_out, stream);
}

static int lnsum_tile_width(int tile) { return (tile == 3 || tile == 20) ? 256 : (tile == 5 || tile == 23) ? 192 : (tile == 13) ? 64 : 128; }
extern "C" int64_t rga3_gemm_lnsum_slices(int64_t N, int tile) {
    if (N <= 0 || !(tile == -1 || tile == 3 || tile == 5 || tile == 12 || tile == 13 || tile == 20 || tile == 23)) return -1;
    return cdiv(N, lnsum_tile_width(tile));
}
extern "C" int rga3_gemm_lnsum_bf16(const void* A, const void* W, const void* bias, const void* residual, void* C, int64_t M, int64_t N, int64_t K, int64_t lda,
                                    int64_t ldw, int64_t ldc, int64_t ldr, int tile, float* row_parts, void* stream) {
    RGA3_CHECK_ARG(A && W && C && row_parts && (((uintptr_t)row_parts) & 7) == 0, "gemm_lnsum: null pointer / row_parts must be 8-byte aligned");
    RGA3_CHECK_ARG(M > 16 && N > 0 && K > 0 && K % 8 == 0, "gemm_lnsum: bad shape M=%ld N=%ld K=%ld (M > 16, K %% 8)", (long)M, (long)N, (long)K);
    RGA3_CHECK_ARG(lda % 8 == 0 && ldw % 8 == 0, "gemm_lnsum: lda/ldw must be multiples of 8 elements (16-byte rows)");
    RGA3_CHECK_ARG((((uintptr_t)A | (uintptr_t)W | (uintptr_t)C) & 15) == 0, "gemm_lnsum: pointers must be 16-byte aligned");
    RGA3_CHECK_ARG(tile == -1 || tile == 3 || tile == 5 || tile == 12 || tile == 13 || tile == 20 || tile == 23, "gemm_lnsum: tile %d (3 / 5 / 12 / 13 / 20 / 23)", tile);
    RGA3_CHECK_ARG(M * lda < (1LL << 32) && N * ldw < (1LL << 32), "gemm_lnsum: operands must be < 2^32 elements (32-bit staging offsets)");
    GemmArgs a;
    a.A = (const unsigned short*)A; a.W = (const unsigned short*)W; a.C = C;
    a.bias = (const unsigned short*)bias; a.res = (const unsigned short*)residual; a.colscale = nullptr;
    a.M = (int)M; a.N = (int)N; a.K = (int)K;
    a.lda = lda; a.ldw = ldw; a.ldc = ldc; a.ldr = ldr;
    a.ws = nullptr; a.ws_bytes = 0; a.ksl = 0; a.rowstat = nullptr; a.colc = nullptr;
    a.ln_parts = row_parts;
    hipStream_t st = (hipStream_t)stream;
    switch (tile) {
        case 3: return launch_cfg<128, 256, 2, 4, ACT_NONE, false, 0, 2>(a, st);
        case 5: return launch_cfg<128, 192, 2, 4, ACT_NONE, false, 0, 2>(a, st);
        case 13: return launch_cfg<64, 64, 2, 2, ACT_NONE, false, 0, 2>(a, st);
        case 20: return launch_pp<ACT_NONE, false, 2, false>(a, st);
        case 23: return launch_pp<ACT_NONE, false, 2, true>(a, st);
        default: return launch_cfg<128, 128, 2, 2, ACT_NONE, false, 0, 2>(a, st);
    }
}

extern "C" int rga3_gemm_swiglu_pre_bf16(const void* A, const void* W, const void* bias, void* C, void* pre, int64_t M, int64_t N, int64_t K, int64_t lda, int64_t ldw,
                                         int64_t ldc, int64_t ldpre, int tile, void* workspace, int64_t workspace_bytes, void* stream) {
    RGA3_CHECK_ARG(pre, "gemm_swiglu_pre: null pre-activation output");
    return gemm_bf16_impl(A, W, bias, nullptr, nullptr, C, M, N, K, lda, ldw, ldc, 0, ACT_SWIGLU, RGA3_BF16, tile, workspace, workspace_bytes, nullptr, 0, 0.f, nullptr, stream, pre,
                          ldpre);
}

extern "C" int rga3_gemm_cat_bf16(const void* A, const void* W, const void* bias, void* C, int64_t M, int64_t N, int64_t K, int64_t lda, int64_t ldw, int64_t ldc,
                                  const void* A2, const void* W2, int64_t K2, int64_t lda2, int64_t ldw2, const void* Wn, void* Cn, int64_t N2, int64_t ldwn,
                                  int64_t ldcn, int tile, void* stream) {
    RGA3_CHECK_ARG(A && W && C && M > 16 && N > 0 && K > 0, "gemm_cat: bad args");
    RGA3_CHECK_ARG((A2 != nullptr) == (W2 != nullptr) && (A2 != nullptr) == (K2 > 0), "gemm_cat: the K side takes A2, W2 and K2 together");
    RGA3_CHECK_ARG((Wn != nullptr) == (Cn != nullptr) && (Wn != nullptr) == (N2 > 0), "gemm_cat: the N side takes Wn, Cn and N2 together");
    RGA3_CHECK_ARG(A2 || Wn, "gemm_cat: nothing concatenated (use rga3_gemm_bf16)");
    RGA3_CHECK_ARG(K % 64 == 0 && K2 % 64 == 0, "gemm_cat: K = %ld and K2 = %ld must be multiples of 64", (long)K, (long)K2);
    RGA3_CHECK_ARG(lda % 8 == 0 && ldw % 8 == 0 && lda2 % 8 == 0 && ldw2 % 8 == 0 && ldwn % 8 == 0 && N % 8 == 0 && N2 % 8 == 0, "gemm_cat: strides / widths must be multiples of 8 elements");
    RGA3_CHECK_ARG((((uintptr_t)A | (uintptr_t)W | (uintptr_t)C | (uintptr_t)A2 | (uintptr_t)W2 | (uintptr_t)Wn | (uintptr_t)Cn) & 15) == 0, "gemm_cat: pointer alignment");
    RGA3_CHECK_ARG(M * lda < (1LL << 32) && N * ldw < (1LL << 32) && M * (lda2 ? lda2 : 1) < (1LL << 32) && N * (ldw2 ? ldw2 : 1) < (1LL << 32) && N2 * (ldwn ? ldwn : 1) < (1LL << 32),
                   "gemm_cat: operands must be < 2^32 elements");
    const int bn = (tile == 3 || tile == 6) ? 256 : (tile == 4) ? 320 : (tile == 5) ? 192 : (tile == 13) ? 64 : 128;
    RGA3_CHECK_ARG(tile == -1 || tile == 3 || tile == 6 || tile == 12 || tile == 13 || (!Wn && (tile == 4 || tile == 5)), "gemm_cat: tile %d", tile);
    RGA3_CHECK_ARG(!Wn || N % bn == 0, "gemm_cat: with an N side, N = %ld must be a multiple of the tile width %d", (long)N, bn);
    GemmArgs a;
    a.A = (const unsigned short*)A; a.W = (const unsigned short*)W; a.C = C;
    a.bias = (const unsigned short*)bias; a.res = nullptr; a.colscale = nullptr;
    a.M = (int)M; a.N = (int)N; a.K = (int)K;
    a.lda = lda; a.ldw = ldw; a.ldc = ldc; a.ldr = 0;
    a.ws = nullptr; a.ws_bytes = 0; a.ksl = 0; a.rowstat = nullptr; a.colc = nullptr;
    a.A2 = (const unsigned short*)A2; a.W2 = (const unsigned short*)W2; a.K2 = (int)K2; a.lda2 = lda2; a.ldw2 = ldw2;
    a.Wn = (const unsigned short*)Wn; a.Cn = Cn; a.N2 = (int)N2; a.ldwn = ldwn; a.ldcn = ldcn;
    hipStream_t st = (hipStream_t)stream;
    switch (tile) {
        case 3: return launch_cfg<128, 256, 2, 4, ACT_NONE, false, 0>(a, st);
        case 4: return launch_cfg<128, 320, 2, 4, ACT_NONE, false, 0>(a, st);
        case 5: return launch_cfg<128, 192, 2, 4, ACT_NONE, false, 0>(a, st);
        case 6: return launch_cfg<128, 256, 2, 4, ACT_NONE, false, 3>(a, st);
        case 13: return launch_cfg<64, 64, 2, 2, ACT_NONE, false, 0>(a, st);
        default: return launch_cfg<128, 128, 2, 2, ACT_NONE, false, 0>(a, st);
    }
}

static int gemm_bf16_impl(const void* A, const void* W, const void* bias, const void* residual, const void* colscale, void* C,
                          int64_t M, int64_t N, int64_t K, int64_t lda, int64_t ldw, int64_t ldc, int64_t ldr,
                          int act, int out_dtype, int tile, void* workspace, int64_t workspace_bytes, const unsigned long long* rs_in, int64_t rs_width, float rs_eps,
                          unsigned long long* rs_out, void* stream, void* pre, int64_t ldpre) {
    RGA3_CHECK_ARG(A && W && C, "gemm: null pointer");
    RGA3_CHECK_ARG(!pre || (act == ACT_SWIGLU && M > 4 && tile != 40 && tile != 41 && (((uintptr_t)pre) & 15) == 0 && ldpre >= N), "gemm: the pre-activation output goes with the SwiGLU tile epilogues (M > 4)");
    RGA3_CHECK_ARG(M > 0 && N > 0 && K > 0, "gemm: bad shape M=%ld N=%ld K=%ld", (long)M, (long)N, (long)K);
    RGA3_CHECK_ARG(K % 8 == 0, "gemm: K=%ld must be a multiple of 8 (16-byte staging chunks)", (long)K);
    RGA3_CHECK_ARG(lda % 8 == 0 && ldw % 8 == 0, "gemm: lda/ldw must be multiples of 8 elements (16-byte rows)");
    RGA3_CHECK_ARG((((uintptr_t)A | (uintptr_t)W | (uintptr_t)C) & 15) == 0, "gemm: pointers must be 16-byte aligned");
    RGA3_CHECK_ARG(out_dtype == RGA3_BF16 || out_dtype == RGA3_F32, "gemm: out_dtype %d", out_dtype);
    RGA3_CHECK_ARG(act >= 0 && act <= 3, "gemm: act %d", act);
    RGA3_CHECK_ARG(!(out_dtype == RGA3_F32 && (act != ACT_NONE || residual || colscale)), "gemm: f32 output supports bias only");
    RGA3_CHECK_ARG(act != ACT_SWIGLU || N % 32 == 0, "gemm: swiglu needs N %% 32 == 0");
    RGA3_CHECK_ARG(tile == -1 || (tile >= 3 && tile <= 8) || (tile >= 10 && tile <= 14) || (tile >= 20 && tile <= 23) || tile == 25 || (tile >= 26 && tile <= 28) || tile == 31 || tile == 32 || tile == 40 || tile == 41, "gemm: tile %d", tile);
    RGA3_CHECK_ARG(M * lda < (1LL << 32) && N * ldw < (1LL << 32), "gemm: operands must be < 2^32 elements (32-bit staging offsets)");
    GemmArgs a;
    a.A = (const unsigned short*)A;
    a.W = (const unsigned short*)W;
    a.C = C;
    a.bias = (const unsigned short*)bias;
    a.res = (const unsigned short*)residual;
    a.colscale = (const unsigned short*)colscale;
    a.M = (int)M; a.N = (int)N; a.K = (int)K;
    a.lda = lda; a.ldw = ldw; a.ldc = ldc; a.ldr = ldr;
    a.ws = workspace; a.ws_bytes = workspace_bytes; a.ksl = 0; a.rowstat = nullptr; a.colc = nullptr;
    a.rs_in = rs_in; a.rs_in_scale = rs_in ? 1.0f / (kRowSumFix * (float)rs_width) : 0.f; a.rs_eps = rs_eps; a.rs_out = rs_out;
    a.pre = (unsigned short*)pre; a.ldpre = ldpre;
    hipStream_t st = (hipStream_t)stream;
    RGA3_CHECK_ARG(tile != 40 || (M <= 4 && !colscale), "gemm: the skinny kernel (tile 40) takes M <= 4 rows and no column scale");
    const bool rows16_ok = M <= 16 && !colscale && out_dtype == RGA3_BF16 && act != ACT_SWIGLU;
    RGA3_CHECK_ARG(tile != 41 || rows16_ok, "gemm: the token-row kernel (tile 41) takes M <= 16 rows, bf16 output, no column scale, no SwiGLU");
    int tl = (tile == -1 && M <= 4 && !colscale) ? 40 : (tile == -1 && rows16_ok) ? 41 : pick_tile((int)M, (int)N, (int)K, act == ACT_NONE && !residual && !colscale && !rs_in && !rs_out, tile);
    if (out_dtype == RGA3_F32) return launch_act<ACT_NONE, true>(a, tl, st);
    switch (act) {
        case ACT_NONE: return launch_act<ACT_NONE, false>(a, tl, st);
        case ACT_GELU: return launch_act<ACT_GELU, false>(a, tl, st);
        case ACT_SWIGLU: return launch_act<ACT_SWIGLU, false>(a, tl, st);
        default: return launch_act<ACT_RELU, false>(a, tl, st);
    }
}

template <int ACT>
static int launch_ln(const GemmArgs& a, int tile, hipStream_t st) {
    switch (tile) {
        case 3: return launch_cfg<128, 256, 2, 4, ACT, false, 0, true>(a, st);
        case 5: return launch_cfg<128, 192, 2, 4, ACT, false, 0, true>(a, st);
        case 6: return launch_cfg<128, 256, 2, 4, ACT, false, 3, true>(a, st);
        case 7: return launch_cfg<128, 192, 2, 4, ACT, false, 3, true>(a, st);
        case 13: return launch_cfg<64, 64, 2, 2, ACT, false, 0, true>(a, st);
        case 20: return launch_pp<ACT, false, true>(a, st);
        default: return launch_cfg<128, 128, 2, 2, ACT, false, 0, true>(a, st);
    }
}

extern "C" int rga3_gemm_ln_bf16(const void* A, const void* Wf, const void* bias, const float* colc, const float* rowstat, void* C, int64_t M, int64_t N, int64_t K,
                                 int64_t lda, int64_t ldw, int64_t ldc, int act, int tile, void* stream) {
    RGA3_CHECK_ARG(A && Wf && C && colc && rowstat, "gemm_ln: null pointer");
    RGA3_CHECK_ARG(M > 0 && N > 0 && K > 0 && K % 8 == 0 && N % 4 == 0, "gemm_ln: bad shape M=%ld N=%ld K=%ld (K %% 8, N %% 4)", (long)M, (long)N, (long)K);
    RGA3_CHECK_ARG(lda % 8 == 0 && ldw % 8 == 0, "gemm_ln: lda/ldw must be multiples of 8 elements");
    RGA3_CHECK_ARG((((uintptr_t)A | (uintptr_t)Wf | (uintptr_t)C | (uintptr_t)colc) & 15) == 0 && (((uintptr_t)rowstat) & 7) == 0, "gemm_ln: pointer alignment");
    RGA3_CHECK_ARG(act == ACT_NONE || act == ACT_GELU || act == ACT_RELU, "gemm_ln: act %d", act);
    RGA3_CHECK_ARG(tile == -1 || tile == 3 || (tile >= 5 && tile <= 7) || tile == 12 || tile == 13 || tile == 20, "gemm_ln: tile %d", tile);
    RGA3_CHECK_ARG(M * lda < (1LL << 32) && N * ldw < (1LL << 32), "gemm_ln: operands must be < 2^32 elements");
    GemmArgs a;
    a.A = (const unsigned short*)A; a.W = (const unsigned short*)Wf; a.C = C;
    a.bias = (const unsigned short*)bias; a.res = nullptr; a.colscale = nullptr;
    a.M = (int)M; a.N = (int)N; a.K = (int)K;
    a.lda = lda; a.ldw = ldw; a.ldc = ldc; a.ldr = 0;
    a.ws = nullptr; a.ws_bytes = 0; a.ksl = 0; a.rowstat = rowstat; a.colc = colc;
    hipStream_t st = (hipStream_t)stream;
    if (act == ACT_GELU) return launch_ln<ACT_GELU>(a, tile, st);
    if (act == ACT_RELU) return launch_ln<ACT_RELU>(a, tile, st);
    return launch_ln<ACT_NONE>(a, tile, st);
}

extern "C" int rga3_gemm_lnq_bf16(const void* A, const void* Wf, const void* bias, const float* colc, const float* row_parts, int64_t slices, int64_t norm_width,
                                  float eps, void* C, int64_t M, int64_t N, int64_t K, int64_t lda, int64_t ldw, int64_t ldc, int act, int tile, void* stream) {
    RGA3_CHECK_ARG(A && Wf && C && colc && row_parts, "gemm_lnq: null pointer");
    RGA3_CHECK_ARG(M > 0 && N > 0 && K > 0 && K % 8 == 0 && N % 4 == 0 && norm_width > 0 && eps >= 0.f && slices >= 1 && slices <= 4096,
                   "gemm_lnq: bad shape M=%ld N=%ld K=%ld slices=%ld (K %% 8, N %% 4)", (long)M, (long)N, (long)K, (long)slices);
    RGA3_CHECK_ARG(lda % 8 == 0 && ldw % 8 == 0, "gemm_lnq: lda/ldw must be multiples of 8 elements");
    RGA3_CHECK_ARG((((uintptr_t)A | (uintptr_t)Wf | (uintptr_t)C | (uintptr_t)colc) & 15) == 0 && (((uintptr_t)row_parts) & 7) == 0, "gemm_lnq: pointer alignment");
    RGA3_CHECK_ARG(act == ACT_NONE || act == ACT_GELU || act == ACT_RELU, "gemm_lnq: act %d", act);
    RGA3_CHECK_ARG(tile == -1 || tile == 3 || (tile >= 5 && tile <= 7) || tile == 12 || tile == 13 || tile == 20, "gemm_lnq: tile %d", tile);
    RGA3_CHECK_ARG(M * lda < (1LL << 32) && N * ldw < (1LL << 32), "gemm_lnq: operands must be < 2^32 elements");
    GemmArgs a;
    a.A = (const unsigned short*)A; a.W = (const unsigned short*)Wf; a.C = C;
    a.bias = (const unsigned short*)bias; a.res = nullptr; a.colscale = nullptr;
    a.M = (int)M; a.N = (int)N; a.K = (int)K;
    a.lda = lda; a.ldw = ldw; a.ldc = ldc; a.ldr = 0;
    a.ws = nullptr; a.ws_bytes = 0; a.ksl = 0; a.rowstat = nullptr; a.colc = colc;
    a.ln_in = row_parts; a.ln_ns = (int)slices; a.rs_in_scale = 1.0f / (float)norm_width; a.rs_eps = eps;
    hipStream_t st = (hipStream_t)stream;
    if (act == ACT_GELU) return launch_ln<ACT_GELU>(a, tile, st);
    if (act == ACT_RELU) return launch_ln<ACT_RELU>(a, tile, st);
    return launch_ln<ACT_NONE>(a, tile, st);
}

extern "C" int rga3_gemm_tn_bf16(const void* A, const void* B, const void* bias, void* C, int64_t M, int64_t N, int64_t K, int64_t lda,
                                 int64_t ldb, int64_t ldc, int out_dtype, void* workspace, int64_t workspace_bytes, void* counters, void* stream) {
    RGA3_CHECK_ARG(A && B && C, "gemm_tn: null pointer");
    RGA3_CHECK_ARG(M >= 8 && N >= 8 && K > 0 && M % 8 == 0 && N % 8 == 0, "gemm_tn: bad shape M=%ld N=%ld K=%ld (M, N multiples of 8)", (long)M, (long)N, (long)K);
    RGA3_CHECK_ARG(lda % 8 == 0 && ldb % 8 == 0 && ldc % 4 == 0, "gemm_tn: lda/ldb must be multiples of 8 elements, ldc of 4");
    RGA3_CHECK_ARG((((uintptr_t)A | (uintptr_t)B | (uintptr_t)C | (uintptr_t)workspace) & 15) == 0, "gemm_tn: pointers must be 16-byte aligned");
    RGA3_CHECK_ARG(out_dtype == RGA3_BF16 || out_dtype == RGA3_F32, "gemm_tn: out_dtype %d", out_dtype);
    RGA3_CHECK_ARG(cdiv(M, 128) <= 65535, "gemm_tn: M too large");
    GemmArgs a;
    a.A = nullptr; a.W = nullptr; a.C = C;
    a.bias = (const unsigned short*)bias; a.res = nullptr; a.colscale = nullptr;
    a.M = (int)M; a.N = (int)N; a.K = (int)K;
    a.lda = 0; a.ldw = 0; a.ldc = ldc; a.ldr = 0;
    a.ntm = (int)cdiv(M, 128); a.ntn = (int)cdiv(N, 128); a.group_m = 1;
    a.ws = nullptr; a.ws_bytes = 0; a.ksl = 0; a.rowstat = nullptr; a.colc = nullptr;
    TnArgs t;
    t.A = (const unsigned short*)A; t.B = (const unsigned short*)B; t.lda = lda; t.ldb = ldb; t.K = (int)K;
    t.counters = nullptr; t.out = nullptr; t.ldo = 0; t.out_f32 = 0;
// ... 96 lines not shown
```

### rga3-release_amd/rga3/hip/lib.py

```python
from __future__ import annotations

import ctypes as C
import os

_HERE = os.path.dirname(os.path.abspath(__file__))
LIB_PATH = os.path.normpath(os.path.join(_HERE, "..", "..", "librga3_hip.so"))

_p, _i, _i64, _f, _sz = C.c_void_p, C.c_int, C.c_int64, C.c_float, C.c_size_t

SIGNATURES = {
    "rga3_version": [],
    "rga3_last_error": [C.c_char_p, _sz],
    "rga3_gemm_bf16": [_p, _p, _p, _p, _p, _p, _i64, _i64, _i64, _i64, _i64, _i64, _i64, _i, _i, _i, _p, _i64, _p],
    "rga3_gemm_rms_bf16": [_p, _p, _p, _p, _p, _i64, _i64, _i64, _i64, _i64, _i64, _i64, _i, _i, _p, _i64, _p, _i64, _f, _p, _p],
    "rga3_gemm_workspace_bytes": [],
    "rga3_gemm_tn_bf16": [_p, _p, _p, _p, _i64, _i64, _i64, _i64, _i64, _i64, _i, _p, _i64, _p, _p],
    "rga3_gemm_tn_many": [_p, _p, _i, _p, _i64, _p],
    "rga3_gemm_swiglu_pre_bf16": [_p, _p, _p, _p, _p, _i64, _i64, _i64, _i64, _i64, _i64, _i64, _i, _p, _i64, _p],
    "rga3_gemm_cat_bf16": [_p, _p, _p, _p, _i64, _i64, _i64, _i64, _i64, _i64, _p, _p, _i64, _i64, _i64, _p, _p, _i64, _i64, _i64, _i, _p],
    "rga3_attn_varlen_fwd": [_p, _p, _p, _p, _p, _p, _p, _i, _i, _i64, _i, _i, _i, _i64, _i64, _i64, _i64, _i64, _i64,
                             _i64, _i64, _f, _i, _i, _p, _i64, _i, _i, _i, _p],
    "rga3_attn_varlen_fwd_rope": [_p, _p, _p, _p, _p, _p, _p, _i, _i, _i64, _i, _i, _i, _i64, _i64, _i64, _i64, _i64, _i64, _i64, _i64, _f, _i, _p, _p, _p, _p, _p],
    "rga3_rmsnorm_fwd": [_p, _p, _p, _p, _p, _i64, _i64, _i64, _f, _p],
    "rga3_layernorm_fwd": [_p, _p, _p, _p, _i64, _i64, _i64, _i64, _f, _i, _p],
    "rga3_layernorm_stats": [_p, _p, _i64, _i64, _i64, _f, _p],
    "rga3_gemm_ln_bf16": [_p, _p, _p, _p, _p, _p, _i64, _i64, _i64, _i64, _i64, _i64, _i, _i, _p],
    "rga3_gemm_lnsum_slices": [_i64, _i],
    "rga3_gemm_lnsum_bf16": [_p, _p, _p, _p, _p, _i64, _i64, _i64, _i64, _i64, _i64, _i64, _i, _p, _p],
    "rga3_gemm_lnq_bf16": [_p, _p, _p, _p, _p, _i64, _i64, _f, _p, _i64, _i64, _i64, _i64, _i64, _i64, _i, _i, _p],
    "rga3_rope_inplace": [_p, _p, _p, _i64, _i, _i, _i, _i64, _i64, _p],
    "rga3_gather_rows": [_p, _p, _p, _i64, _i64, _i64, _i64, _i64, _p],
    "rga3_scatter_rows": [_p, _p, _p, _i64, _i64, _i64, _i64, _i64, _p],
    "rga3_pad_cols": [_p, _p, _i64, _i64, _i64, _i64, _p],
    "rga3_silu_mul": [_p, _p, _p, _i64, _p],
    "rga3_add": [_p, _p, _p, _i64, _p],
    "rga3_cross_entropy_rows": [_p, _i, _p, _p, _p, _i64, _i64, _i64, _f, _p],
    "rga3_im2col": [_p, _p, _i64, _i, _i, _i, _i, _i, _i, _i64, _p],
    "rga3_maxpool2x2_win": [_p, _p, _i64, _i, _i, _i64, _i64, _p],
    "rga3_upsample2x_add": [_p, _p, _p, _i64, _i, _i, _i, _p],
    "rga3_add_bcast": [_p, _p, _p, _i64, _i64, _i, _i64, _i64, _i64, _f, _p],
    "rga3_bilinear": [_p, _i, _p, _p, _i64, _i, _i, _i, _i, _p],
    "rga3_conv3x3s2": [_p, _i, _p, _p, _p, _i64, _i, _i, _i, _i, _f, _f, _p],
    "rga3_decimg_rows": [_p, _i64, _p, _i64, _i, _p, _p, _i, _p, _p, _p, _p, _p, _p, _f, _p, _p, _p, _p, _p, _i64, _p, _p, _i64, _i, _f, _i64, _p],
    "rga3_attn_fewq": [_p, _i64, _p, _i64, _i64, _p, _p, _p, _i64, _i, _i, _i, _i, _f, _p],
    "rga3_copy_many": [_p, _p, _p, _i, _p],
    "rga3_conv3x3s2_ln_gelu": [_p, _i, _p, _p, _p, _p, _f, _p, _i64, _i, _i, _i, _i, _f, _f, _p],
    "rga3_dwconv7x7": [_p, _p, _p, _p, _i64, _i, _i, _i, _p],
    "rga3_rope_axial_inplace": [_p, _p, _p, _i64, _i, _i, _i64, _p],
    "rga3_pixel_shuffle2x": [_p, _p, _p, _p, _i64, _i, _i, _i, _i, _p],
    "rga3_bce_dice_sums": [_p, _p, _p, _i64, _i64, _p],
    "rga3_bce_dice_sums_ws_floats": [_i64, _i64],
    "rga3_bce_dice_sums_det": [_p, _p, _p, _p, _i64, _i64, _i64, _p],
    "rga3_attn_varlen_bwd": [_p, _p, _p, _p, _p, _p, _p, _p, _p, _p, _p, _p, _i, _i, _i, _i64, _i, _i, _i, _p, _f, _i, _p, _i64, _p],
    "rga3_transpose16_many": [_p, _p, _i, _p],
    "rga3_hiera_mlp144": [_p, _p, _p, _p, _p, _p, _p, _i64, _f, _p],
    "rga3_hiera_mlp288_pack_bytes": [],
    "rga3_hiera_mlp288_pack": [_p, _p, _p, _p, _p, _p],
    "rga3_hiera_mlp288": [_p, _p, _p, _p, _i64, _f, _p],
    "rga3_mlp3_rows": [_p, _p, _i, _i64, _p],
    "rga3_sam_select_objptr": [_p, _p, _p, _i64, _i, _p, _p, _p, _p, _p, _p, _p, _p, _p, _p, _i64, _p],
    "rga3_memattn_cross_ws_floats": [_i64, _i],
    "rga3_memattn_cross": [_p, _p, _p, _p, _i64, _i64, _i64, _i64, _i64, _i64, _f, _i, _p, _p],
    "rga3_memlayer_rows": [_p, _i64, _i, _p, _p, _i, _p, _p, _p, _i64, _p, _i64, _p, _p, _f, _p, _i64, _p, _p, _i, _p, _i64, _p, _p, _i, _i, _i64, _p],
    "rga3_gemm_rows16_many": [_p, _p, _i, _p],
    "rga3_gemm_stream_k_timeouts": [_p],
    "rga3_gemm_timeout_counter_offset": [],
    "rga3_gemm_ragged_plan": [_i64, _i64, _i64, _i, _i, _p, _p],
    "rga3_quant_fp8_rows": [_p, _p, _p, _i64, _i64, _i64, _i64, _p],
    "rga3_gemm_fp8": [_p, _p, _p, _p, _p, _p, _p, _i64, _i64, _i64, _i64, _i64, _i64, _i64, _p],
    "rga3_swiglu_fwd_quant_fp8": [_p, _p, _p, _i64, _i64, _p],
    "rga3_swiglu_bwd_quant_fp8": [_p, _p, _p, _p, _i64, _i64, _p],
    "rga3_im2col3x3s2": [_p, _p, _i64, _i, _i, _i, _p],
    "rga3_pil_bicubic_coeffs": [_i, _i, _p, _p, _i64, _p],
    "rga3_sam_preprocess_u8": [_p, _i64, _i, _i, _i, _i, _p, _p, _i, _p, _p, _i, _p, _p, _p, _p, _p, _p],
    "rga3_qwen_norm_lut": [_p, _p, _i, _p],
    "rga3_qwen_patchify_u8": [_p, _i64, _i, _i, _p, _p, _i, _i, _i, _i, _p],
    "rga3_rmsnorm_bwd": [_p, _p, _p, _p, _p, _i64, _i64, _f, _p],
    "rga3_dropout_bf16": [_p, _p, _i64, _f, _i64, _i, _p],
    "rga3_dropout_pair_bf16": [_p, _p, _p, _p, _i64, _f, _i64, _f, _i64, _i, _p],
    "rga3_swiglu_fwd": [_p, _p, _i64, _i64, _p],
    "rga3_swiglu_bwd": [_p, _p, _p, _i64, _i64, _p],
    "rga3_transpose16": [_p, _p, _i64, _i64, _i64, _i64, _p],
    "rga3_segment_sum_rows": [_p, _p, _p, _p, _i64, _i64, _i64, _p],
    "rga3_adamw_step": [_p, _p, _p, _p, _p, _i64, _f, _f, _f, _f, _f, _i, _f, _p],
    "rga3_sumsq_accum": [_p, _p, _i64, _p],
    "rga3_sumsq_det": [_p, _i64, _p, _i64, _p, _i, _p],
    "rga3_adamw_step_clip": [_p, _p, _p, _p, _p, _i64, _f, _f, _f, _f, _f, _i, _p, _f, _p],
    "rga3_adamw_step_clip_rows": [_p, _p, _p, _p, _p, _i64, _i64, _p, _f, _f, _f, _f, _i, _p, _f, _p],
    "rga3_scatter_add_rows": [_p, _p, _p, _i64, _i64, _i64, _i64, _f, _p],
    "rga3_layernorm_bwd_ws_floats": [_i64, _i64],
    "rga3_layernorm_bwd": [_p, _p, _p, _p, _p, _p, _i64, _i64, _f, _p, _i64, _p],
    "rga3_colsum_accum": [_p, _p, _i64, _i64, _i64, _p],
    "rga3_colsum_ws_floats": [_i64, _i64],
    "rga3_colsum": [_p, _p, _i64, _i64, _i64, _p, _i64, _p, _p],
    "rga3_act": [_p, _p, _p, _i64, _i, _p],
    "rga3_bilinear_bwd": [_p, _p, _p, _i64, _i, _i, _i, _i, _p],
    "rga3_mask_product": [_p, _p, _p, _i64, _i64, _i64, _i64, _p],
    "rga3_mask_product_bwd_ws_floats": [_i64, _i64, _i64, _i64],
    "rga3_mask_product_bwd": [_p, _p, _p, _p, _p, _i64, _i64, _i64, _i64, _p, _i64, _p],
    "rga3_pixel_shuffle2x_bwd": [_p, _p, _i64, _i, _i, _i, _p],
    "rga3_bce_dice_grad": [_p, _p, _p, _p, _i64, _i64, _f, _f, _p],
    "rga3_bce_dice_grad_dev": [_p, _p, _p, _p, _i64, _i64, _p, _p, _p],
}

_INT64_RESULTS = ("rga3_gemm_lnsum_slices", "rga3_hiera_mlp288_pack_bytes", "rga3_gemm_workspace_bytes", "rga3_memattn_cross_ws_floats", "rga3_gemm_timeout_counter_offset", "rga3_layernorm_bwd_ws_floats", "rga3_colsum_ws_floats", "rga3_mask_product_bwd_ws_floats", "rga3_bce_dice_sums_ws_floats")

_lib = None


class Rga3Error(RuntimeError):
    pass


def load():
    global _lib
    if _lib is not None:
        return _lib
    if not os.path.exists(LIB_PATH):
        raise Rga3Error(
            f"{LIB_PATH} not found: the HIP extension is required (no fallback path). "
            "Run `make -C rga3-release_amd/csrc` or `python -c 'import __graft_entry__ as g; g.build()'`.")
    import torch

    _thip = os.path.join(os.path.dirname(torch.__file__), "lib", "libamdhip64.so")
    if os.path.exists(_thip):
        C.CDLL(_thip, mode=C.RTLD_GLOBAL)
    lib = C.CDLL(LIB_PATH)
    for name, argtypes in SIGNATURES.items():
        fn = getattr(lib, name)
        fn.argtypes = argtypes
        fn.restype = C.c_int64 if name in _INT64_RESULTS else C.c_int
    _lib = lib
    return lib


def last_error() -> str:
    buf = C.create_string_buffer(512)
    load().rga3_last_error(buf, 512)
    return buf.value.decode("utf-8", "replace")


def check(rc: int, what: str):
    if rc != 0:
        raise Rga3Error(f"{what} failed (rc={rc}): {last_error()}")
```

### rga3-release_amd/rga3/hip/ops.py

```python
from __future__ import annotations

import torch

from . import lib as _lib
from . import tuner as _tuner

BF16, F32 = 0, 1
ACT = {"none": 0, "gelu": 1, "swiglu": 2, "relu": 3}


def _stream():
    return torch.cuda.current_stream().cuda_stream


def _ptr(t):
    return 0 if t is None else t.data_ptr()


def _need_cuda(*ts):
    for t in ts:
        if t is not None and not t.is_cuda:
            raise _lib.Rga3Error("rga3 HIP ops need device tensors (no CPU fallback on the product path)")


def pad_cols(x: torch.Tensor, ld: int) -> torch.Tensor:
    _need_cuda(x)
    assert x.dtype == torch.bfloat16 and x.dim() == 2 and x.stride(1) == 1
    rows, cols = x.shape
    out = torch.empty((rows, ld), dtype=torch.bfloat16, device=x.device)
    _lib.check(_lib.load().rga3_pad_cols(x.data_ptr(), out.data_ptr(), rows, cols, x.stride(0), ld, _stream()), "pad_cols")
    return out


_gemm_ws = {}
_ws_scope = [None]


class workspace_scope:

    def __init__(self, token):
        self.token = ("scope", token)

    def __enter__(self):
        self.old, _ws_scope[0] = _ws_scope[0], self.token
        return self

    def __exit__(self, *exc):
        _ws_scope[0] = self.old


def _ws_key(device):
    dev = device.index if device.index is not None else torch.cuda.current_device()
    return (dev, _ws_scope[0] if _ws_scope[0] is not None else torch.cuda.current_stream(device).cuda_stream)


def gemm_workspace(device) -> torch.Tensor:
    key = _ws_key(device)
    t = _gemm_ws.get(key)
    if t is None:
        with torch.cuda.device(device):
            n = int(_lib.load().rga3_gemm_workspace_bytes())
        if n <= 0:
            raise _lib.Rga3Error("rga3_gemm_workspace_bytes failed: " + _lib.last_error())
        t = _gemm_ws[key] = torch.zeros(n, dtype=torch.uint8, device=device)
    return t


def gemm_stream_k_timeouts(device=None) -> int:
    tot = 0
    for (dev, _), t in _gemm_ws.items():
        if device is None or dev == (device.index if device.index is not None else torch.cuda.current_device()):
            with torch.cuda.device(dev):
                tot += int(_lib.load().rga3_gemm_stream_k_timeouts(t.data_ptr()))
    return tot


_LNSUM_TILES = (20, 3, 5, 12, 13, 23)


def gemm(a: torch.Tensor, w: torch.Tensor, bias=None, residual=None, act: str = "none", out_dtype=torch.bfloat16,
         out=None, tile: int = -1, colscale=None, rms_in=None, rms_out=None) -> torch.Tensor:
    _need_cuda(a, w, bias, residual, out, colscale)
    assert a.dtype == torch.bfloat16 and w.dtype == torch.bfloat16
    assert a.dim() == 2 and w.dim() == 2 and a.shape[1] == w.shape[1], (a.shape, w.shape)
    assert a.stride(1) == 1 and w.stride(1) == 1
    M, K = a.shape
    N = w.shape[0]
    if K % 8 != 0 or a.stride(0) % 8 != 0 or w.stride(0) % 8 != 0:
        Kp = (K + 7) // 8 * 8
        if a.shape[1] != Kp or a.stride(0) % 8 != 0:
            a = pad_cols(a, Kp)
        if w.shape[1] != Kp or w.stride(0) % 8 != 0:
            w = pad_cols(w, Kp)
        K = Kp
    n_out = N // 2 if act == "swiglu" else N
    if out is None:
        out = torch.empty((M, n_out), dtype=out_dtype, device=a.device)
    assert out.shape == (M, n_out) and out.stride(1) == 1 and out.dtype == out_dtype
    if bias is not None:
        assert bias.dtype == torch.bfloat16 and bias.numel() == N and bias.is_contiguous()
    ldr = 0
    if residual is not None:
        assert residual.dtype == torch.bfloat16 and residual.shape == (M, n_out) and residual.stride(1) == 1
        ldr = residual.stride(0)
    if colscale is not None:
        assert colscale.dtype == torch.bfloat16 and colscale.numel() == n_out and colscale.is_contiguous()
    fn = _lib.load().rga3_gemm_bf16
    odt = BF16 if out_dtype == torch.bfloat16 else F32
    ws = gemm_workspace(a.device)

    rms = rms_in is not None or rms_out is not None
    if rms:
        assert M > 16 and out_dtype == torch.bfloat16 and colscale is None, "gemm: the RMSNorm-folded form takes M > 16, bf16 output, no column scale"
        rs_t, rs_width, rs_eps = rms_in if rms_in is not None else (None, 0, 0.0)
        for t_ in (rs_t, rms_out):
            assert t_ is None or (t_.is_cuda and t_.dtype == torch.int64 and t_.numel() == M and t_.is_contiguous())
        fn_rms = _lib.load().rga3_gemm_rms_bf16

    def run(t, final=True):
        ro = rms_out if (rms and final) else None
        if rms and (rs_t is not None or ro is not None):
            _lib.check(fn_rms(a.data_ptr(), w.data_ptr(), _ptr(bias), _ptr(residual), out.data_ptr(), M, N, K, a.stride(0), w.stride(0), out.stride(0), ldr,
                              ACT[act], t, ws.data_ptr(), ws.numel(), _ptr(rs_t), int(rs_width), float(rs_eps), _ptr(ro), _stream()), "gemm_rms_bf16")
        else:
            _lib.check(fn(a.data_ptr(), w.data_ptr(), _ptr(bias), _ptr(residual), _ptr(colscale), out.data_ptr(), M, N, K, a.stride(0), w.stride(0),
                          out.stride(0), ldr, ACT[act], odt, t, ws.data_ptr(), ws.numel(), _stream()), "gemm_bf16")

    if rms:
        if tile == -1:
            tile = _tuner.pick(_tuner.key_of(M, N, K, act, odt, bias is not None, residual is not None), lambda t: run(t, final=False))
            if tile in (14, 25, 40, 41):
                tile = -1
        run(tile)
        return out
    if tile == -1 and M <= 4 and colscale is None:
        tile = 40
    if tile == -1 and M * N * K >= (1 << 24) and not (residual is not None and residual.data_ptr() == out.data_ptr()):
        plain = act == "none" and residual is None and colscale is None
        extra = (25,) if (M * N <= (1 << 20) and K >= 4096 and plain) else ()
        if plain and bias is None and N % 8 == 0 and M * N <= (1 << 19) and K >= 512:
            extra = extra + (14,)
        if M <= 16 and colscale is None and out_dtype == torch.bfloat16 and act != "swiglu":
            extra = extra + (41,)
        if act == "none" and N % 192 == 0 and N % 256 != 0 and M >= 1024:
            extra = extra + (23,)
        tile = _tuner.pick(_tuner.key_of(M, N, K, act, odt, bias is not None, residual is not None), run, extra)
    run(tile)
    return out


def gemm_swiglu_pre(a, w, bias=None, tile: int = -1):
    _need_cuda(a, w, bias)
    assert a.dtype == w.dtype == torch.bfloat16 and a.dim() == w.dim() == 2 and a.shape[1] == w.shape[1] and a.stride(1) == w.stride(1) == 1
    M, K = a.shape
    N = w.shape[0]
    assert N % 32 == 0 and M > 4
    out = torch.empty((M, N // 2), dtype=torch.bfloat16, device=a.device)
    pre = torch.empty((M, N), dtype=torch.bfloat16, device=a.device)
    ws = gemm_workspace(a.device)
    fn = _lib.load().rga3_gemm_swiglu_pre_bf16

    def run(t):
        _lib.check(fn(a.data_ptr(), w.data_ptr(), _ptr(bias), out.data_ptr(), pre.data_ptr(), M, N, K, a.stride(0), w.stride(0), out.stride(0), pre.stride(0), t,
                      ws.data_ptr(), ws.numel(), _stream()), "gemm_swiglu_pre_bf16")

    if tile == -1 and M * N * K >= (1 << 24):
        tile = _tuner.pick(_tuner.key_of(M, N, K, "swiglu+pre", BF16, bias is not None, False), run)
        if tile in (14, 25, 40, 41):
            tile = -1
    run(tile)
    return out, pre


def gemm_cat(a, w, bias=None, a2=None, w2=None, wn=None, tile: int = -1):
    _need_cuda(a, w, bias, a2, w2, wn)
    assert a.dtype == w.dtype == torch.bfloat16 and a.dim() == w.dim() == 2 and a.shape[1] == w.shape[1] and a.stride(1) == w.stride(1) == 1
    M, K = a.shape
    N = w.shape[0]
    assert (a2 is None) == (w2 is None) and (a2 is not None or wn is not None)
    K2 = 0
    if a2 is not None:
        assert a2.dtype == w2.dtype == torch.bfloat16 and a2.shape[0] == M and w2.shape[0] == N and a2.shape[1] == w2.shape[1] and a2.stride(1) == w2.stride(1) == 1
        K2 = a2.shape[1]
    N2 = 0
    out_n = None
    if wn is not None:
        assert wn.dtype == torch.bfloat16 and wn.dim() == 2 and wn.shape[1] == K and wn.stride(1) == 1
        N2 = wn.shape[0]
        out_n = torch.empty((M, N2), dtype=torch.bfloat16, device=a.device)
    out = torch.empty((M, N), dtype=torch.bfloat16, device=a.device)
    fn = _lib.load().rga3_gemm_cat_bf16

    def run(t):
        _lib.check(fn(a.data_ptr(), w.data_ptr(), _ptr(bias), out.data_ptr(), M, N, K, a.stride(0), w.stride(0), out.stride(0), _ptr(a2), _ptr(w2), K2,
                      a2.stride(0) if a2 is not None else 0, w2.stride(0) if w2 is not None else 0, _ptr(wn), _ptr(out_n), N2, wn.stride(0) if wn is not None else 0,
                      out_n.stride(0) if out_n is not None else 0, t, _stream()), "gemm_cat_bf16")

    if tile == -1:
        cands = tuple(t for t in ((12, 3, 6, 13) if wn is not None else (12, 3, 4, 5, 6, 13)) if wn is None or N % (256 if t in (3, 6) else 64 if t == 13 else 128) == 0)
        tile = _tuner.pick(_tuner.key_of(M, N + N2, K + K2, "cat", BF16, bias is not None, False), run, candidates=cands)
        if tile not in cands:
            tile = -1
    run(tile)
    return out if out_n is None else (out, out_n)


def gemm_rows16_many(sets):
    import ctypes
    n = len(sets)
    assert 1 <= n <= 4
    ptrs, dims, outs = (ctypes.c_void_p * (6 * n))(), (ctypes.c_int64 * (9 * n))(), []
    for i, st in enumerate(sets):
        a, a2, w, b = st[:4]
        res = st[4] if len(st) > 4 else None
        act = st[5] if len(st) > 5 else "none"
        _need_cuda(a, a2, w, b, res)
        assert a.dtype == w.dtype == torch.bfloat16 and a.dim() == 2 and w.dim() == 2 and a.shape[1] == w.shape[1] and a.stride(1) == 1 and w.stride(1) == 1
        M, K = a.shape
        N = w.shape[0]
        assert M <= 16 and K % 8 == 0 and (a2 is None or (a2.shape == a.shape and a2.stride(1) == 1 and a2.dtype == torch.bfloat16))
        assert b is None or (b.numel() == N and b.is_contiguous() and b.dtype == torch.bfloat16)
        assert res is None or (tuple(res.shape) == (M, N) and res.stride(1) == 1 and res.stride(0) >= N and res.dtype == torch.bfloat16)
        out = torch.empty((M, N), dtype=torch.bfloat16, device=a.device)
        outs.append(out)
        for j, t in enumerate((a, a2, w, b, res, out)):
            ptrs[6 * i + j] = _ptr(t) or None
        for j, v in enumerate((M, N, K, ACT[act], a.stride(0), a2.stride(0) if a2 is not None else 0, w.stride(0), N, res.stride(0) if res is not None else 0)):
            dims[9 * i + j] = int(v)
    _lib.check(_lib.load().rga3_gemm_rows16_many(ctypes.cast(ptrs, ctypes.c_void_p), ctypes.cast(dims, ctypes.c_void_p), n, _stream()), "gemm_rows16_many")
    return outs


def layernorm_stats(x, eps: float):
    _need_cuda(x)
    assert x.dtype == torch.bfloat16 and x.dim() == 2 and x.stride(1) == 1
    st = torch.empty((x.shape[0], 2), dtype=torch.float32, device=x.device)
    _lib.check(_lib.load().rga3_layernorm_stats(x.data_ptr(), st.data_ptr(), x.shape[0], x.shape[1], x.stride(0), float(eps), _stream()), "layernorm_stats")
    return st
# ... 480 lines not shown
        _lib.check(_lib.load().rga3_im2col3x3s2(x.data_ptr(), cols.data_ptr(), F, H, W, Cin, _stream()), "im2col3x3s2")
        return gemm(cols, wp, bias)
    y = torch.empty((F * (H // 2) * (W // 2), Cout), dtype=torch.bfloat16, device=x.device)
    rc = _lib.load().rga3_conv3x3s2(x.data_ptr(), F32 if x.dtype == torch.float32 else BF16, weight.data_ptr(), _ptr(bias), y.data_ptr(), F, H, W,
                                    Cin, Cout, float(sig_scale), float(sig_bias), _stream())
    _lib.check(rc, "conv3x3s2")
    return y


def dwconv7x7(x, weight, bias, F: int, H: int, W: int):
    _need_cuda(x, weight, bias)
    assert x.dtype == torch.bfloat16 and x.is_contiguous() and weight.is_contiguous()
    y = torch.empty_like(x)
    _lib.check(_lib.load().rga3_dwconv7x7(x.data_ptr(), weight.data_ptr(), _ptr(bias), y.data_ptr(), F, H, W, x.shape[1], _stream()), "dwconv7x7")
    return y


def rope_axial_(x, cos, sin, n_rope: int):
    _need_cuda(x, cos, sin)
    assert x.dtype == torch.bfloat16 and x.dim() == 2 and x.stride(1) == 1 and cos.dtype == torch.float32 and cos.is_contiguous() and sin.is_contiguous()
    assert cos.shape[1] * 2 == x.shape[1]
    _lib.check(_lib.load().rga3_rope_axial_inplace(x.data_ptr(), cos.data_ptr(), sin.data_ptr(), int(n_rope), cos.shape[0], x.shape[1], x.stride(0),
                                                  _stream()), "rope_axial")
    return x


def mlp3_rows(specs, B: int):
    import ctypes
    n = len(specs)
    assert 1 <= n <= 8
    ptrs, dims, outs, keep = (ctypes.c_void_p * (8 * n))(), (ctypes.c_int64 * (6 * n))(), [], []
    for i, sp in enumerate(specs):
        x, xs, (w0, b0, w1, b1, w2, b2), sig = sp[:4]
        _need_cuda(x, w0, b0, w1, b1, w2, b2)
        for t in (w0, w1, w2):
            assert t.dtype == torch.bfloat16 and t.is_contiguous()
        assert x.dtype == torch.bfloat16 and tuple(w1.shape) == (w0.shape[0], w0.shape[0]) and w2.shape[1] == w0.shape[0], (w0.shape, w1.shape, w2.shape)
        y = sp[4] if len(sp) > 4 and sp[4] is not None else torch.empty((B, w2.shape[0]), dtype=torch.bfloat16, device=x.device)
        assert y.dtype == torch.bfloat16 and tuple(y.shape) == (B, w2.shape[0]) and y.stride(1) == 1
        for j, t in enumerate((x, w0, b0, w1, b1, w2, b2, y)):
            ptrs[8 * i + j] = _ptr(t)
        for j, v in enumerate((int(xs), y.stride(0), w0.shape[1], w0.shape[0], w2.shape[0], 1 if sig else 0)):
            dims[6 * i + j] = v
        outs.append(y)
    _lib.check(_lib.load().rga3_mlp3_rows(ctypes.cast(ptrs, ctypes.c_void_p), ctypes.cast(dims, ctypes.c_void_p), n, int(B), _stream()), "mlp3_rows")
    return outs


def sam_select_objptr(iou, obj, toks, proj, no_obj_ptr):
    _need_cuda(iou, obj, toks, no_obj_ptr, *proj)
    B, _, C = toks.shape
    assert iou.dtype == obj.dtype == toks.dtype == torch.bfloat16 and iou.is_contiguous() and obj.is_contiguous() and toks.stride(2) == 1 and toks.stride(1) == C
    best = torch.empty((2, B), dtype=torch.int64, device=toks.device)
    sel = torch.empty(B, dtype=torch.int32, device=toks.device)
    ptr = torch.empty((B, C), dtype=torch.bfloat16, device=toks.device)
    w0, b0, w1, b1, w2, b2 = proj
    _lib.check(_lib.load().rga3_sam_select_objptr(iou.data_ptr(), obj.data_ptr(), toks.data_ptr(), toks.stride(0), C, w0.data_ptr(), _ptr(b0), w1.data_ptr(), _ptr(b1),
                                                  w2.data_ptr(), _ptr(b2), no_obj_ptr.data_ptr(), best.data_ptr(), sel.data_ptr(), ptr.data_ptr(), B, _stream()),
               "sam_select_objptr")
    return best[0], sel, best[1], ptr


_memattn_ws = {}


def memattn_cross(q, k, m, scale: float, nsplit: int = 0, partials: bool = False):
    _need_cuda(q, k, m)
    assert q.dtype == k.dtype == m.dtype == torch.bfloat16 and q.dim() == k.dim() == m.dim() == 2
    assert q.shape[1] == 256 and k.shape[1] == 256 and m.shape[1] == 64 and k.shape[0] == m.shape[0], (q.shape, k.shape, m.shape)
    assert q.stride(1) == 1 and k.stride(1) == 1 and m.stride(1) == 1
    Nq, Nk = q.shape[0], k.shape[0]
    if nsplit <= 0:
        nqb = (Nq + 255) // 256
        nsplit = max(1, min(32, 256 // nqb, (Nk + 63) // 64))
    L = _lib.load()
    n = int(L.rga3_memattn_cross_ws_floats(Nq, nsplit))
    if n < 0:
        raise _lib.Rga3Error("memattn_cross: bad workspace query")
    key = _ws_key(q.device)
    ws = _memattn_ws.get(key)
    if ws is None or ws.numel() < n:
        ws = _memattn_ws[key] = torch.empty(n, dtype=torch.float32, device=q.device)
    if partials:
        _lib.check(L.rga3_memattn_cross(q.data_ptr(), k.data_ptr(), m.data_ptr(), None, Nq, Nk, q.stride(0), k.stride(0), m.stride(0), 0,
                                        float(scale), int(nsplit), ws.data_ptr(), _stream()), "memattn_cross")
        return ws[:nsplit * Nq * 64], ws[nsplit * Nq * 64:nsplit * Nq * 66], nsplit
    out = torch.empty((Nq, 64), dtype=torch.bfloat16, device=q.device)
    _lib.check(L.rga3_memattn_cross(q.data_ptr(), k.data_ptr(), m.data_ptr(), out.data_ptr(), Nq, Nk, q.stride(0), k.stride(0), m.stride(0), out.stride(0),
                                    float(scale), int(nsplit), ws.data_ptr(), _stream()), "memattn_cross")
    return out


def memlayer_rows(res, ln, eps: float, a=None, partials=None, w1=None, b1=None, want_x=True, want_t=False, w2=None, b2=None, rope=None, rope_cols: int = 0):
    wln, bln = ln
    _need_cuda(res, wln, bln, a, w1, b1, w2, b2)
    assert res.dtype == torch.bfloat16 and res.dim() == 2 and res.shape[1] == 256 and res.stride(1) == 1
    M, dev = res.shape[0], res.device
    x = t = y = None
    K1, po, pml, ns = 0, None, None, 0
    if w1 is not None:
        assert w1.dtype == torch.bfloat16 and w1.is_contiguous() and w1.shape[0] == 256
        K1 = w1.shape[1]
        if partials is not None:
            po, pml, ns = partials
            assert a is None and K1 == 64 and po.numel() == ns * M * 64 and pml.numel() == ns * M * 2
        else:
            assert a is not None and a.dtype == torch.bfloat16 and tuple(a.shape) == (M, K1) and a.stride(1) == 1
        if want_x:
            x = torch.empty((M, 256), dtype=torch.bfloat16, device=dev)
    else:
        assert a is None and partials is None
    if want_t or w2 is None:
        t = torch.empty((M, 256), dtype=torch.bfloat16, device=dev)
    N2, cos, sin, nq = 0, None, None, 0
    if w2 is not None:
        assert w2.dtype == torch.bfloat16 and w2.is_contiguous() and w2.shape[1] == 256 and w2.shape[0] in (256, 768)
        N2 = w2.shape[0]
        y = torch.empty((M, N2), dtype=torch.bfloat16, device=dev)
        if rope_cols:
            cos, sin = rope
            assert cos.dtype == sin.dtype == torch.float32 and cos.is_contiguous() and sin.is_contiguous() and cos.shape[1] == 128 and cos.shape == sin.shape
            nq = cos.shape[0]
    _lib.check(_lib.load().rga3_memlayer_rows(_ptr(a), a.stride(0) if a is not None else 0, K1, _ptr(po), _ptr(pml), ns, _ptr(w1), _ptr(b1), res.data_ptr(), res.stride(0),
                                              _ptr(x), 256, wln.data_ptr(), _ptr(bln), float(eps), _ptr(t), 256, _ptr(w2), _ptr(b2), N2, _ptr(y), N2 if N2 else 0,
                                              _ptr(cos), _ptr(sin), int(rope_cols), nq, M, _stream()), "memlayer_rows")
    return x, t, y


def pixel_shuffle2x(g, bias, add, F: int, H: int, W: int, act: str = "none"):
    _need_cuda(g, bias, add)
    Co = g.shape[1] // 4
    assert g.dtype == torch.bfloat16 and g.is_contiguous()
    out = torch.empty((F * 4 * H * W, Co), dtype=torch.bfloat16, device=g.device)
    _lib.check(_lib.load().rga3_pixel_shuffle2x(g.data_ptr(), _ptr(bias), _ptr(add), out.data_ptr(), F, H, W, Co, 1 if act == "gelu" else 0, _stream()),
               "pixel_shuffle2x")
    return out


def bce_dice_sums(logits, targets):
    _need_cuda(logits, targets)
    assert logits.dtype == targets.dtype == torch.float32 and logits.is_contiguous() and targets.is_contiguous() and logits.shape == targets.shape
    n = logits.shape[0]
    out = torch.empty((n, 4), dtype=torch.float32, device=logits.device)
    if n == 0:
        return out
    L = _lib.load()
    hw = logits[0].numel()
    nws = int(L.rga3_bce_dice_sums_ws_floats(n, hw))
    ws = torch.empty(nws, dtype=torch.float32, device=logits.device)
    _lib.check(L.rga3_bce_dice_sums_det(logits.data_ptr(), targets.data_ptr(), out.data_ptr(), ws.data_ptr(), nws, n, hw, _stream()), "bce_dice_sums_det")
    return out


def attn_varlen_bwd(q, k, v, o, dout, lse, cu_q, cu_k, max_q: int, max_k: int, scale: float, causal: bool, dq=None, dk=None, dv=None):
    import ctypes
    _need_cuda(q, k, v, o, dout, lse)
    Tq, Hq, D = q.shape
    Hkv = k.shape[1]
    dq = torch.empty_like(q) if dq is None else dq
    dk = torch.empty((k.shape[0], Hkv, D), dtype=torch.bfloat16, device=q.device) if dk is None else dk
    dv = torch.empty((k.shape[0], Hkv, D), dtype=torch.bfloat16, device=q.device) if dv is None else dv
    for t in (q, k, v, o, dout, dq, dk, dv):
        assert t.dtype == torch.bfloat16 and t.stride(2) == 1
    delta = torch.empty((Hq, Tq), dtype=torch.float32, device=q.device)
    Tk = k.shape[0]
    dkv_ws = torch.empty((2 * Hq * Tk * D,), dtype=torch.float32, device=q.device) if (Hq > Hkv and D % 4 == 0) else None
    st = (ctypes.c_int64 * 16)(q.stride(0), q.stride(1), k.stride(0), k.stride(1), v.stride(0), v.stride(1), o.stride(0), o.stride(1),
                               dout.stride(0), dout.stride(1), dq.stride(0), dq.stride(1), dk.stride(0), dk.stride(1), dv.stride(0), dv.stride(1))
    rc = _lib.load().rga3_attn_varlen_bwd(q.data_ptr(), k.data_ptr(), v.data_ptr(), o.data_ptr(), dout.data_ptr(), lse.data_ptr(), dq.data_ptr(),
                                          dk.data_ptr(), dv.data_ptr(), delta.data_ptr(), cu_q.data_ptr(), cu_k.data_ptr(), cu_q.numel() - 1, int(max_q),
                                          int(max_k), Tq, Hq, Hkv, D, ctypes.cast(st, ctypes.c_void_p), float(scale), int(bool(causal)), _ptr(dkv_ws), Tk, _stream())
    _lib.check(rc, "attn_varlen_bwd")
    return dq, dk, dv


def rmsnorm_bwd(x, weight, dy, eps: float, add=None):
    _need_cuda(x, weight, dy, add)
    assert x.is_contiguous() and dy.is_contiguous() and x.dtype == dy.dtype == torch.bfloat16 and (add is None or add.is_contiguous())
    dx = torch.empty_like(x)
    _lib.check(_lib.load().rga3_rmsnorm_bwd(x.data_ptr(), weight.data_ptr(), dy.data_ptr(), _ptr(add), dx.data_ptr(), x.shape[0], x.shape[1], float(eps),
                                            _stream()), "rmsnorm_bwd")
    return dx


def quant_fp8_rows(x):
    _need_cuda(x)
    assert x.dtype == torch.bfloat16 and x.dim() == 2 and x.stride(1) == 1 and x.shape[1] % 8 == 0
    rows, K = x.shape
    q = torch.empty((rows, K), dtype=torch.uint8, device=x.device)
    sc = torch.empty((rows,), dtype=torch.float32, device=x.device)
    _lib.check(_lib.load().rga3_quant_fp8_rows(x.data_ptr(), q.data_ptr(), sc.data_ptr(), rows, K, x.stride(0), q.stride(0), _stream()), "quant_fp8_rows")
    return q, sc


def gemm_fp8(aq, sa, wq, sw, bias=None, residual=None, out=None):
    _need_cuda(aq, wq, sa, sw, bias, residual)
    assert aq.dtype == torch.uint8 and wq.dtype == torch.uint8 and aq.stride(1) == 1 and wq.stride(1) == 1 and aq.shape[1] == wq.shape[1]
    M, K = aq.shape
    N = wq.shape[0]
    if out is None:
        out = torch.empty((M, N), dtype=torch.bfloat16, device=aq.device)
    assert out.dtype == torch.bfloat16 and out.stride(1) == 1 and sa.dtype == torch.float32 and sw.dtype == torch.float32
    _lib.check(_lib.load().rga3_gemm_fp8(aq.data_ptr(), wq.data_ptr(), sa.data_ptr(), sw.data_ptr(), _ptr(bias), _ptr(residual), out.data_ptr(), M, N, K,
                                         aq.stride(0), wq.stride(0), out.stride(0), residual.stride(0) if residual is not None else 0, _stream()), "gemm_fp8")
    return out


def swiglu_fwd_quant(gu):
    _need_cuda(gu)
    assert gu.dtype == torch.bfloat16 and gu.is_contiguous() and gu.shape[1] % 32 == 0
    T, I = gu.shape[0], gu.shape[1] // 2
    q = torch.empty((T, I), dtype=torch.uint8, device=gu.device)
    sc = torch.empty((T,), dtype=torch.float32, device=gu.device)
    _lib.check(_lib.load().rga3_swiglu_fwd_quant_fp8(gu.data_ptr(), q.data_ptr(), sc.data_ptr(), T, I, _stream()), "swiglu_fwd_quant_fp8")
    return q, sc


def swiglu_bwd_quant(gu, da):
    _need_cuda(gu, da)
    assert gu.dtype == da.dtype == torch.bfloat16 and gu.is_contiguous() and da.is_contiguous() and gu.shape[1] == 2 * da.shape[1]
    T, I = da.shape
    q = torch.empty((T, 2 * I), dtype=torch.uint8, device=gu.device)
    sc = torch.empty((T,), dtype=torch.float32, device=gu.device)
    _lib.check(_lib.load().rga3_swiglu_bwd_quant_fp8(gu.data_ptr(), da.data_ptr(), q.data_ptr(), sc.data_ptr(), T, I, _stream()), "swiglu_bwd_quant_fp8")
    return q, sc


def dropout(x, p: float, seed: int, out=None, accumulate: bool = False):
    _need_cuda(x, out)
    assert x.dtype == torch.bfloat16 and x.is_contiguous() and x.numel() % 8 == 0
    if out is None:
        assert not accumulate
        out = torch.empty_like(x)
    assert out.is_contiguous() and out.shape == x.shape and out.dtype == torch.bfloat16
    _lib.check(_lib.load().rga3_dropout_bf16(x.data_ptr(), out.data_ptr(), x.numel(), float(p), int(seed) & 0x7FFFFFFFFFFFFFFF, int(bool(accumulate)), _stream()),
               "dropout")
    return out


def dropout_pair(xa, pa: float, seed_a: int, xb, pb: float, seed_b: int, accumulate_into=None):
    _need_cuda(xa, xb, accumulate_into)
    assert xa.dtype == xb.dtype == torch.bfloat16 and xa.is_contiguous() and xb.is_contiguous() and xa.shape == xb.shape and xa.numel() % 8 == 0
    L = _lib.load()
    if accumulate_into is None:
        ya, yb = torch.empty_like(xa), torch.empty_like(xb)
        _lib.check(L.rga3_dropout_pair_bf16(xa.data_ptr(), xb.data_ptr(), ya.data_ptr(), yb.data_ptr(), xa.numel(), float(pa), int(seed_a), float(pb), int(seed_b), 0,
                                            _stream()), "dropout_pair_bf16")
        return ya, yb
    out = accumulate_into
    assert out.dtype == torch.bfloat16 and out.is_contiguous() and out.shape == xa.shape
    _lib.check(L.rga3_dropout_pair_bf16(xa.data_ptr(), xb.data_ptr(), out.data_ptr(), None, xa.numel(), float(pa), int(seed_a), float(pb), int(seed_b), 1, _stream()),
               "dropout_pair_bf16")
    return out


def swiglu_fwd(gu):
    _need_cuda(gu)
    assert gu.dtype == torch.bfloat16 and gu.is_contiguous() and gu.shape[1] % 32 == 0
    a = torch.empty((gu.shape[0], gu.shape[1] // 2), dtype=torch.bfloat16, device=gu.device)
    _lib.check(_lib.load().rga3_swiglu_fwd(gu.data_ptr(), a.data_ptr(), gu.shape[0], gu.shape[1] // 2, _stream()), "swiglu_fwd")
    return a


def swiglu_bwd(gu, da):
    _need_cuda(gu, da)
    assert gu.is_contiguous() and da.is_contiguous() and gu.shape[1] == 2 * da.shape[1]
    dgu = torch.empty_like(gu)
    _lib.check(_lib.load().rga3_swiglu_bwd(gu.data_ptr(), da.data_ptr(), dgu.data_ptr(), gu.shape[0], da.shape[1], _stream()), "swiglu_bwd")
    return dgu


def transpose(x):
    _need_cuda(x)
    assert x.dim() == 2 and x.stride(1) == 1 and x.element_size() == 2
    R, C = x.shape
    out = torch.empty((C, R), dtype=x.dtype, device=x.device)
    _lib.check(_lib.load().rga3_transpose16(x.data_ptr(), out.data_ptr(), R, C, x.stride(0), R, _stream()), "transpose16")
    return out


def transpose_many(mats):
    import ctypes
    outs = []
    for a in range(0, len(mats), 64):
        grp = mats[a:a + 64]
        n = len(grp)
        ptrs, dims = (ctypes.c_void_p * (2 * n))(), (ctypes.c_int64 * (2 * n))()
        for i, x in enumerate(grp):
            _need_cuda(x)
            assert x.dim() == 2 and x.is_contiguous() and x.element_size() == 2
            o = torch.empty((x.shape[1], x.shape[0]), dtype=x.dtype, device=x.device)
            ptrs[2 * i], ptrs[2 * i + 1] = x.data_ptr(), o.data_ptr()
            dims[2 * i], dims[2 * i + 1] = x.shape[0], x.shape[1]
            outs.append(o)
        _lib.check(_lib.load().rga3_transpose16_many(ctypes.cast(ptrs, ctypes.c_void_p), ctypes.cast(dims, ctypes.c_void_p), n, _stream()), "transpose16_many")
    return outs


def segment_sum_rows(x, rows, offsets):
    _need_cuda(x, rows, offsets)
    assert x.dtype == torch.bfloat16 and x.stride(1) == 1 and rows.dtype == torch.int64 and offsets.dtype == torch.int64
    n = offsets.numel() - 1
    out = torch.empty((n, x.shape[1]), dtype=torch.bfloat16, device=x.device)
    if n > 0:
        _lib.check(_lib.load().rga3_segment_sum_rows(x.data_ptr(), rows.data_ptr(), offsets.data_ptr(), out.data_ptr(), n, x.shape[1], x.stride(0), _stream()),
                   "segment_sum_rows")
    return out


def adamw_step_(param, master, grad, m, v, lr, beta1, beta2, eps, weight_decay, step: int, grad_scale: float = 1.0):
    _need_cuda(param, master, grad, m, v)
    assert param.dtype == grad.dtype == torch.bfloat16 and master.dtype == m.dtype == v.dtype == torch.float32
    assert param.is_contiguous() and grad.is_contiguous() and master.is_contiguous()
    _lib.check(_lib.load().rga3_adamw_step(param.data_ptr(), master.data_ptr(), grad.data_ptr(), m.data_ptr(), v.data_ptr(), param.numel(), float(lr),
                                           float(beta1), float(beta2), float(eps), float(weight_decay), int(step), float(grad_scale), _stream()), "adamw_step")


def sumsq_accum_(g, out):
    _need_cuda(g, out)
    assert g.dtype == torch.bfloat16 and g.is_contiguous() and out.dtype == torch.float32
    _lib.check(_lib.load().rga3_sumsq_accum(g.data_ptr(), out.data_ptr(), g.numel(), _stream()), "sumsq_accum")


def sumsq_det_(g, partials, out, accumulate: bool):
    _need_cuda(g, partials, out)
# ... 189 lines not shown
```

### rga3-release_amd/rga3/model/qwen_train.py

```python
from __future__ import annotations

import math
import os

import numpy as np
import torch
import torch.nn as nn

from ..hip import ops
from ..utils.staging import upload
from . import qwen2_5_vl as _Q
from .qwen2_5_vl import GatedMLP, Linear, _versions


class LoRALinear(Linear):

    def __init__(self, base: Linear, r: int, alpha: float, dropout: float = 0.0):
        super().__init__(base.in_features, base.out_features, bias=base.bias is not None, device=base.weight.device, dtype=base.weight.dtype)
        self.weight, self.bias = base.weight, base.bias
        self.weight.requires_grad_(False)
        if self.bias is not None:
            self.bias.requires_grad_(False)
        mk = lambda i, o: Linear(i, o, bias=False, device=base.weight.device, dtype=base.weight.dtype)
        self.lora_A = nn.ModuleDict({"default": mk(base.in_features, r)})
        self.lora_B = nn.ModuleDict({"default": mk(r, base.out_features)})
        nn.init.kaiming_uniform_(self.lora_A["default"].weight, a=math.sqrt(5))
        nn.init.zeros_(self.lora_B["default"].weight)
        self.scaling = alpha / r
        self.r = r
        if not 0.0 <= dropout < 1.0:
            raise ValueError(f"lora dropout {dropout}")
        self.dropout_p = float(dropout)

    def forward(self, x, residual=None, act="none"):
        y = super().forward(x, residual=residual, act=act)
        xin = x.reshape(-1, x.shape[-1])
        if self.training and self.dropout_p > 0.0:
            xin = ops.dropout(xin.contiguous(), self.dropout_p, next_dropout_seed(0, 3))
        t = self.lora_A["default"](xin)
        bs = (self.lora_B["default"].weight.detach() * self.scaling).to(t.dtype)
        y2 = y.view(-1, y.shape[-1])
        ops.gemm(t, bs, residual=y2, out=y2)
        return y


def add_lora(model: nn.Module, r=128, alpha=256, dropout=0.0, targets=("q_proj", "v_proj"),
             exclude=("sam_model", "grounding_encodervisual", "text_hidden_fcs")):
    hits = []
    for name, mod in list(model.named_modules()):
        if isinstance(mod, nn.Linear) and not isinstance(mod, LoRALinear) and all(x not in name for x in exclude) and any(x in name for x in targets):
            parent = model
            parts = name.split(".")
            for p in parts[:-1]:
                parent = getattr(parent, p)
            setattr(parent, parts[-1], LoRALinear(mod, r, alpha, dropout))
            hits.append(name)
    return hits


def _wt(owner, key, *srcs, build):
    cache = owner.__dict__.setdefault("_wt_cache", {})
    ver = _versions(*srcs)
    hit = cache.get(key)
    if hit is None or hit[0] != ver:
        with torch.no_grad():
            cache[key] = (ver, build())
    return cache[key][1]


_fp8 = {"on": False}


def set_fp8_frozen_gemms(on: bool, vision: bool = True):
    _fp8["on"] = bool(on)
    _Q._VIT_BLOCK_FP8[0] = vision_block_forward_fp8 if (on and vision) else None


def fp8_frozen_gemms() -> bool:
    return _fp8["on"]


def _fp8_pack(owner, key, *srcs, build):
    def mk():
        w = build()
        q, sc = ops.quant_fp8_rows(w.contiguous())
        return (q, sc)
    return _wt(owner, "fp8:" + key, *srcs, build=mk)


_fp8_tap = [None]


def _fgemm(x, owner, key, srcs, build, bias=None, residual=None, out=None):
    if _fp8["on"] and x.shape[1] % 128 == 0:
        q, sc = _fp8_pack(owner, key, *srcs, build=build)
        xq, xs = ops.quant_fp8_rows(x)
        if _fp8_tap[0] is not None:
            _fp8_tap[0](key, xq, xs)
        return ops.gemm_fp8(xq, xs, q, sc, bias=bias, residual=residual, out=out)
    w = _wt(owner, key, *srcs, build=build)
    return ops.gemm(x, w, bias, residual=residual, out=out)


def _fgemm_q(xq, xs, owner, key, srcs, build, bias=None, residual=None, out=None):
    q, sc = _fp8_pack(owner, key, *srcs, build=build)
    if _fp8_tap[0] is not None:
        _fp8_tap[0](key, xq, xs)
    return ops.gemm_fp8(xq, xs, q, sc, bias=bias, residual=residual, out=out)


def _fp8_fused(k: int) -> bool:
    return _fp8["on"] and k % 128 == 0


def vision_block_forward_fp8(blk, x, cu, max_len, cos, sin):
    at, mlp = blk.attn, blk.mlp
    N = x.shape[0]
    H, D = at.num_heads, at.head_dim
    h1 = blk.norm1(x)
    qkv = _fgemm(h1, at, "wqkv", (at.qkv.weight,), lambda: at.qkv.weight.detach(), bias=at.qkv.bias).view(N, 3 * H, D)
    if ops.attn_rope_win_ok(max_len, D):
        att = ops.attn_varlen_rope(qkv[:, :H], qkv[:, H:2 * H], qkv[:, 2 * H:], cu, cu, max_len, D ** -0.5, cos, sin, causal=False, rope_k=True)
    else:
        ops.rope_(qkv, cos, sin, 0, 2 * H)
        att = ops.attn_varlen(qkv[:, :H], qkv[:, H:2 * H], qkv[:, 2 * H:], cu, cu, max_len, D ** -0.5, causal=False, max_k=max_len)
    x1 = _fgemm(att.view(N, H * D), at, "wproj", (at.proj.weight,), lambda: at.proj.weight.detach(), bias=at.proj.bias, residual=x)
    h2 = blk.norm2(x1)
    wgu, bgu, wd = mlp._packed()
    gu = _fgemm(h2, mlp, "wgu", (mlp.gate_proj.weight, mlp.up_proj.weight), lambda: wgu, bias=bgu)
    return _down_from_gu(mlp, gu, wd, x1)


def _lora_parts(lin):
    if isinstance(lin, LoRALinear):
        return lin.lora_A["default"].weight, lin.lora_B["default"].weight, lin.scaling
    return None


_lora_cache = {}


def _lora_versions(lin):
    A, B = lin.lora_A["default"].weight, lin.lora_B["default"].weight
    return A._version, A.data_ptr(), B._version, B.data_ptr()


def _lora_build(mods):
    groups = {}
    for m in mods:
        A, B = m.lora_A["default"].weight, m.lora_B["default"].weight
        groups.setdefault((tuple(A.shape), tuple(B.shape), float(m.scaling), A.dtype, A.device), []).append(m)
    with torch.no_grad():
        for (_, _, sc, _, _), grp in groups.items():
            A = torch.stack([m.lora_A["default"].weight.detach() for m in grp])
            B = torch.stack([m.lora_B["default"].weight.detach() for m in grp])
            As = A * sc
            At = A.transpose(1, 2).contiguous()
            Bts = (B * sc).transpose(1, 2).contiguous()
            for i, m in enumerate(grp):
                _lora_cache[id(m)] = (_lora_versions(m), As[i], At[i], Bts[i])


def lora_refresh(layers):
    mods = [p for layer in layers for p in (layer.self_attn.q_proj, layer.self_attn.v_proj) if isinstance(p, LoRALinear)]
    if mods and any((e := _lora_cache.get(id(m))) is None or e[0] != _lora_versions(m) for m in (mods[0], mods[-1])):
        _lora_build(mods)
    ats = [layer.self_attn for layer in layers if _lora_cat_ok(layer.self_attn)]
    if ats and len({(a.num_heads, a.num_kv, a.head_dim, a.q_proj.lora_A["default"].weight.shape[0], float(a.q_proj.scaling), float(a.v_proj.scaling)) for a in ats}) == 1:
        if any((e := _lora_cat.get(id(a))) is None or e[0] != _lora_versions(a.q_proj) + _lora_versions(a.v_proj) for a in (ats[0], ats[-1])):
            _lora_cat_build(ats)


_LORA_FOLD = os.environ.get("RGA3_LORA_FOLD", "1") != "0"
_SWIGLU_PRE = os.environ.get("RGA3_SWIGLU_PRE", "1") != "0"
_lora_cat = {}
_lora_cat_store = {}


def set_lora_fold(on: bool):
    global _LORA_FOLD
    _LORA_FOLD = bool(on)


def _lora_cat_ok(at) -> bool:
    q, v = at.q_proj, at.v_proj
    if not (_LORA_FOLD and isinstance(q, LoRALinear) and isinstance(v, LoRALinear)) or isinstance(at.k_proj, LoRALinear):
        return False
    rq, rv = q.lora_A["default"].weight.shape[0], v.lora_A["default"].weight.shape[0]
    return rq == rv and (2 * rq) % 64 == 0 and q.lora_A["default"].weight.dtype == torch.bfloat16 and q.weight.shape[1] % 64 == 0


def _lora_cat_build(ats):
    with torch.no_grad():
        at0 = ats[0]
        Hq, Hk, D = at0.num_heads, at0.num_kv, at0.head_dim
        r = at0.q_proj.lora_A["default"].weight.shape[0]
        Nq, Nall = Hq * D, (Hq + 2 * Hk) * D
        Bq = torch.stack([a.q_proj.lora_B["default"].weight.detach() for a in ats])
        Bv = torch.stack([a.v_proj.lora_B["default"].weight.detach() for a in ats])
        ids = tuple(id(a) for a in ats)
        key = (ids, Nall, r, Bq.dtype, Bq.device)
        st = _lora_cat_store.get(key)
        if st is None:
            for k in [k for k in _lora_cat_store if k != key and not set(k[0]).isdisjoint(ids)]:
                del _lora_cat_store[k]
            st = (torch.zeros((len(ats), Nall, 2 * r), dtype=Bq.dtype, device=Bq.device), torch.zeros((len(ats), 2 * r, Nall), dtype=Bq.dtype, device=Bq.device))
            _lora_cat_store[key] = st
        W2, Wn = st
        W2[:, :Nq, :r] = Bq
        W2[:, Nq + Hk * D:, r:] = Bv
        Wn[:, :r, :Nq] = (Bq * float(at0.q_proj.scaling)).transpose(1, 2)
        Wn[:, r:, Nq + Hk * D:] = (Bv * float(at0.v_proj.scaling)).transpose(1, 2)
        for i, a in enumerate(ats):
            _lora_cat[id(a)] = (_lora_versions(a.q_proj) + _lora_versions(a.v_proj), W2[i], Wn[i])


def _lora_cat_ops(at):
    e = _lora_cat.get(id(at))
    if e is None or e[0] != _lora_versions(at.q_proj) + _lora_versions(at.v_proj):
        _lora_cat_build([at])
        e = _lora_cat[id(at)]
    return e[1], e[2]


def _lora_ops(lin):
    e = _lora_cache.get(id(lin))
    if e is None or e[0] != _lora_versions(lin):
        _lora_build([lin])
        e = _lora_cache[id(lin)]
    return e[1], e[2], e[3]


_drop_state = {"step": 0}


def next_dropout_seed(layer_idx: int, which: int, advance: bool = True) -> int:
    if advance:
        _drop_state["step"] += 1
    base = torch.initial_seed() & 0xFFFFFF
    return ((base << 39) ^ (_drop_state["step"] << 12) ^ (layer_idx << 2) ^ which) & 0x7FFFFFFFFFFFFFFF


def preview_dropout_seeds(n_layers: int):
    saved = _drop_state["step"]
    try:
        return [(next_dropout_seed(li, 0), next_dropout_seed(li, 1, advance=False)) for li in range(n_layers)]
    finally:
        _drop_state["step"] = saved


def _lora_dropout(at):
    pq = at.q_proj.dropout_p if isinstance(at.q_proj, LoRALinear) and at.q_proj.training else 0.0
    pv = at.v_proj.dropout_p if isinstance(at.v_proj, LoRALinear) and at.v_proj.training else 0.0
    return pq, pv


def _drop_pair(h1, pq, pv, seeds):
    if pq > 0.0 and pv > 0.0 and h1.is_contiguous():
        return ops.dropout_pair(h1, pq, seeds[0], h1, pv, seeds[1])
    return (ops.dropout(h1, pq, seeds[0]) if pq > 0.0 else h1), (ops.dropout(h1, pv, seeds[1]) if pv > 0.0 else h1)


def qkv_with_lora(at, h1, seeds=None, want_inputs=False):
    Hq, Hk, D = at.num_heads, at.num_kv, at.head_dim
    wqkv, bqkv = at._packed()
    lq, lv = _lora_parts(at.q_proj), _lora_parts(at.v_proj)
    pq, pv = _lora_dropout(at)
    if seeds is None and (pq > 0.0 or pv > 0.0):
        lid = getattr(at, "layer_idx", 0) or 0
        seeds = (next_dropout_seed(lid, 0), next_dropout_seed(lid, 1, advance=False))
    if not _fp8["on"] and h1.shape[0] > 16 and _lora_cat_ok(at):
        r = lq[0].shape[0]
        hq, hv = _drop_pair(h1, pq, pv, seeds)
        tt = torch.empty((h1.shape[0], 2 * r), dtype=h1.dtype, device=h1.device)
        tq = ops.gemm(hq, _lora_ops(at.q_proj)[0], out=tt[:, :r])
        tv = ops.gemm(hv, _lora_ops(at.v_proj)[0], out=tt[:, r:])
        qkv2 = ops.gemm_cat(h1, wqkv, bqkv, a2=tt, w2=_lora_cat_ops(at)[0])
        return (qkv2, tq, tv, hq, hv) if want_inputs else (qkv2, tq, tv)
    if _fp8["on"] and h1.shape[1] % 128 == 0:
        qkv2 = _fgemm(h1, at, "wqkv", (at.q_proj.weight, at.k_proj.weight, at.v_proj.weight), lambda: wqkv, bias=bqkv)
    else:
        qkv2 = ops.gemm(h1, wqkv, bqkv)
    tq = tv = None
    hq = hv = h1
    if lq is not None and lv is not None and pq > 0.0 and pv > 0.0:
        hq, hv = _drop_pair(h1, pq, pv, seeds)
        pq = pv = 0.0
    if lq is not None:
        if pq > 0.0:
            hq = ops.dropout(h1, pq, seeds[0])
        tq = ops.gemm(hq, _lora_ops(at.q_proj)[0])
        oq = qkv2[:, : Hq * D]
        ops.gemm(tq, lq[1].detach(), residual=oq, out=oq)
    if lv is not None:
        if pv > 0.0:
            hv = ops.dropout(h1, pv, seeds[1])
        tv = ops.gemm(hv, _lora_ops(at.v_proj)[0])
        ov = qkv2[:, (Hq + Hk) * D:]
        ops.gemm(tv, lv[1].detach(), residual=ov, out=ov)
    return (qkv2, tq, tv, hq, hv) if want_inputs else (qkv2, tq, tv)


def _layer_forward_fp8(layer, x, cos, sin, cu, max_len, seeds):
    at, mlp = layer.self_attn, layer.mlp
    Hq, Hk, D = at.num_heads, at.num_kv, at.head_dim
    T = x.shape[0]
    w1, w2 = layer.input_layernorm, layer.post_attention_layernorm
    h1 = ops.rmsnorm(x, w1.weight, w1.variance_epsilon)
    qkv2 = qkv_with_lora(at, h1, seeds=seeds)[0]
    qkv = qkv2.view(T, Hq + 2 * Hk, D)
    ops.rope_(qkv, cos, sin, 0, Hq + Hk)
    att = ops.attn_varlen(qkv[:, :Hq], qkv[:, Hq:Hq + Hk], qkv[:, Hq + Hk:], cu, cu, max_len, D ** -0.5, causal=True)
    x1 = _fgemm(att.view(T, Hq * D), at, "wo", (at.o_proj.weight,), lambda: at.o_proj.weight.detach(), residual=x)
    h2 = ops.rmsnorm(x1, w2.weight, w2.variance_epsilon)
    wgu, bgu, wd = mlp._packed()
    gu = _fgemm(h2, mlp, "wgu", (mlp.gate_proj.weight, mlp.up_proj.weight), lambda: wgu, bias=bgu)
    return _down_from_gu(mlp, gu, wd, x1)


def _down_from_gu(mlp, gu, wd, x1):
    if _fp8_fused(gu.shape[1] // 2):
        aq, asc = ops.swiglu_fwd_quant(gu)
        return _fgemm_q(aq, asc, mlp, "wd", (mlp.down_proj.weight,), lambda: wd, bias=mlp.down_proj.bias, residual=x1)
    return _fgemm(ops.swiglu_fwd(gu), mlp, "wd", (mlp.down_proj.weight,), lambda: wd, bias=mlp.down_proj.bias, residual=x1)


_acts = {"store": True}


def set_activation_recompute(on: bool):
    _acts["store"] = not on


def _layer_forward_store(layer, x, cos, sin, cu, max_len, seeds):
    at, mlp = layer.self_attn, layer.mlp
    Hq, Hk, D = at.num_heads, at.num_kv, at.head_dim
    T = x.shape[0]
    w1, w2 = layer.input_layernorm, layer.post_attention_layernorm
    h1 = ops.rmsnorm(x, w1.weight, w1.variance_epsilon)
    qkv2, tq, tv, hq_in, hv_in = qkv_with_lora(at, h1, seeds=seeds, want_inputs=True)
    qkv = qkv2.view(T, Hq + 2 * Hk, D)
    ops.rope_(qkv, cos, sin, 0, Hq + Hk)
    att, lse = ops.attn_varlen(qkv[:, :Hq], qkv[:, Hq:Hq + Hk], qkv[:, Hq + Hk:], cu, cu, max_len, D ** -0.5, causal=True, return_lse=True)
    x1 = _fgemm(att.view(T, Hq * D), at, "wo", (at.o_proj.weight,), lambda: at.o_proj.weight.detach(), residual=x)
    h2 = ops.rmsnorm(x1, w2.weight, w2.variance_epsilon)
    wgu, bgu, wd = mlp._packed()
    if not _fp8["on"] and _SWIGLU_PRE and T > 4:
        a_, gu = ops.gemm_swiglu_pre(h2, wgu, bgu)
        y = _fgemm(a_, mlp, "wd", (mlp.down_proj.weight,), lambda: wd, bias=mlp.down_proj.bias, residual=x1)
    else:
        gu = _fgemm(h2, mlp, "wgu", (mlp.gate_proj.weight, mlp.up_proj.weight), lambda: wgu, bias=bgu)
        y = _down_from_gu(mlp, gu, wd, x1)
    return y, (h1, qkv, att, lse, x1, h2, gu, tq, tv, hq_in, hv_in)


_neg = {}


def _neg_table(sin):
    key = (sin.data_ptr(), sin._version, tuple(sin.shape))
    if _neg.get("key") != key:
        _neg["key"], _neg["t"] = key, (-sin).contiguous()
        _neg["src"] = sin
    return _neg["t"]


class DecoderLayerFn(torch.autograd.Function):

    @staticmethod
    def forward(ctx, x, aq, bq, av, bv, layer, cos, sin, cu, max_len, seeds):
        at0 = layer.self_attn
        ctx.stored = False
        if _acts["store"]:
            with torch.no_grad():
                y, saved = _layer_forward_store(layer, x, cos, sin, cu, max_len, seeds)
            ctx.stored = True
            ctx.seeds = seeds
            ctx.layer, ctx.cos, ctx.sin, ctx.cu, ctx.max_len = layer, cos, sin, cu, max_len
            ctx.save_for_backward(x, *saved)
            return y
        if _fp8["on"]:
            with torch.no_grad():
                y = _layer_forward_fp8(layer, x, cos, sin, cu, max_len, seeds)
        else:
            at0._lora_drop_seeds = seeds
            try:
                with torch.no_grad():
                    y = layer(x, cos, sin, cu, max_len, None)
            finally:
                at0._lora_drop_seeds = None
        ctx.seeds = seeds
        ctx.layer, ctx.cos, ctx.sin, ctx.cu, ctx.max_len = layer, cos, sin, cu, max_len
        ctx.save_for_backward(x)
        return y

    @staticmethod
    def backward(ctx, dy):
        x = ctx.saved_tensors[0]
        layer, cos, sin, cu, max_len = ctx.layer, ctx.cos, ctx.sin, ctx.cu, ctx.max_len
        at, mlp = layer.self_attn, layer.mlp
        Hq, Hk, D = at.num_heads, at.num_kv, at.head_dim
        T = x.shape[0]
        dy = dy.contiguous()
        with torch.no_grad():
            w1, w2 = layer.input_layernorm, layer.post_attention_layernorm
            wqkv, bqkv = at._packed()
            lq, lv = _lora_parts(at.q_proj), _lora_parts(at.v_proj)
            pq, pv = _lora_dropout(at)
            wgu, bgu, wd = mlp._packed()
            if ctx.stored:
                h1, qkv, att, lse, x1, h2, gu, tq, tv, hq_in, hv_in = ctx.saved_tensors[1:]
            else:
                h1 = ops.rmsnorm(x, w1.weight, w1.variance_epsilon)
                qkv2, tq, tv, hq_in, hv_in = qkv_with_lora(at, h1, seeds=ctx.seeds, want_inputs=True)
                qkv = qkv2.view(T, Hq + 2 * Hk, D)
                ops.rope_(qkv, cos, sin, 0, Hq + Hk)
                att, lse = ops.attn_varlen(qkv[:, :Hq], qkv[:, Hq:Hq + Hk], qkv[:, Hq + Hk:], cu, cu, max_len, D ** -0.5, causal=True, return_lse=True)
                x1 = _fgemm(att.view(T, Hq * D), at, "wo", (at.o_proj.weight,), lambda: at.o_proj.weight.detach(), residual=x)
                h2 = ops.rmsnorm(x1, w2.weight, w2.variance_epsilon)
                gu = _fgemm(h2, mlp, "wgu", (mlp.gate_proj.weight, mlp.up_proj.weight), lambda: wgu, bias=bgu)
            q, k, v = qkv[:, :Hq], qkv[:, Hq:Hq + Hk], qkv[:, Hq + Hk:]
            da = _fgemm(dy, mlp, "wd_t", (mlp.down_proj.weight,), lambda: ops.transpose(wd))
            if _fp8_fused(gu.shape[1]):
                dq, dsc = ops.swiglu_bwd_quant(gu, da)
                del gu, da
                dh2 = _fgemm_q(dq, dsc, mlp, "wgu_t", (mlp.gate_proj.weight, mlp.up_proj.weight), lambda: ops.transpose(wgu))
                del dq
            else:
                dgu = ops.swiglu_bwd(gu, da)
                del gu, da
                dh2 = _fgemm(dgu, mlp, "wgu_t", (mlp.gate_proj.weight, mlp.up_proj.weight), lambda: ops.transpose(wgu))
                del dgu
            dx1 = ops.rmsnorm_bwd(x1, w2.weight, dh2, w2.variance_epsilon, add=dy)
            datt = _fgemm(dx1, at, "wo_t", (at.o_proj.weight,), lambda: ops.transpose(at.o_proj.weight.detach())).view(T, Hq, D)
            dqkv = torch.empty_like(qkv)
            ops.attn_varlen_bwd(q, k, v, att, datt, lse, cu, cu, max_len, max_len, D ** -0.5, True, dq=dqkv[:, :Hq], dk=dqkv[:, Hq:Hq + Hk],
                                dv=dqkv[:, Hq + Hk:])
            ops.rope_(dqkv, cos, _neg_table(sin), 0, Hq + Hk)
            dqkv2 = dqkv.view(T, (Hq + 2 * Hk) * D)
            fold = (not _fp8["on"]) and T > 16 and _lora_cat_ok(at)
            dtt = None
            if fold:
                wqkv_t = _wt(at, "wqkv_t", at.q_proj.weight, at.k_proj.weight, at.v_proj.weight, build=lambda: ops.transpose(wqkv))
                dh1, dtt = ops.gemm_cat(dqkv2, wqkv_t, wn=_lora_cat_ops(at)[1])
            else:
                dh1 = _fgemm(dqkv2, at, "wqkv_t", (at.q_proj.weight, at.k_proj.weight, at.v_proj.weight), lambda: ops.transpose(wqkv))
            grads = [None, None, None, None]
            if lq is not None or lv is not None:
                tn_pairs, tn_slots = [], []
                pend = []
                for slot, lp, lin, t_, cols, pdrop, hin, sd in ((0, lq, at.q_proj, tq, (0, Hq * D), pq, hq_in, 0),
                                                                (2, lv, at.v_proj, tv, ((Hq + Hk) * D, (Hq + 2 * Hk) * D), pv, hv_in, 1)):
                    if lp is None:
                        continue
                    _, At, Bts = _lora_ops(lin)
                    dsl = dqkv2[:, cols[0]:cols[1]]
                    if dtt is not None:
                        rr = dtt.shape[1] // 2
                        dt = dtt[:, :rr] if slot == 0 else dtt[:, rr:]
                    else:
                        dt = ops.gemm(dsl, Bts)
                    tn_pairs += [(dt, h1 if pdrop == 0.0 else hin), (dsl, t_)]
                    tn_slots += [slot, slot + 1]
                    if pdrop == 0.0:
                        ops.gemm(dt, At, residual=dh1, out=dh1)
                    else:
                        pend.append((ops.gemm(dt, At), pdrop, ctx.seeds[sd]))
                if len(pend) == 2 and dh1.is_contiguous():
                    ops.dropout_pair(pend[0][0], pend[0][1], pend[0][2], pend[1][0], pend[1][1], pend[1][2], accumulate_into=dh1)
                else:
                    for xg, pg, sg in pend:
                        ops.dropout(xg, pg, sg, out=dh1, accumulate=True)
                for sl, gw in zip(tn_slots, ops.gemm_tn_many(tn_pairs)):
                    grads[sl] = gw
            dx = ops.rmsnorm_bwd(x, w1.weight, dh1, w1.variance_epsilon, add=dx1)
        return (dx, grads[0], grads[1], grads[2], grads[3], None, None, None, None, None, None)


class EmbedFn(torch.autograd.Function):

    @staticmethod
    def forward(ctx, weight, ids_dev, ids_np, grad_rows_np, plan=None):
        from ..parallel.ddp import sparse_sink_for

        ctx.shape = weight.shape
        ctx.sink = sparse_sink_for(weight)
        ctx.weight = weight
        plan = plan if plan is not None else {}
        if "embed_bwd" not in plan:
            rows = grad_rows_np
            ids = ids_np[rows]
            order = np.argsort(ids, kind="stable")
            uniq, counts = np.unique(ids[order], return_counts=True)
            off = np.concatenate([[0], np.cumsum(counts)]).astype(np.int64)
            dev = weight.device
            plan["embed_bwd"] = (upload(rows[order].astype(np.int64), dev), upload(off, dev), upload(uniq.astype(np.int64), dev),
                                 uniq.astype(np.int64))
        ctx.csr = plan["embed_bwd"]
        if ctx.sink is not None:
            ctx.sink.announce_sparse(weight, ctx.csr[3])
        return ops.gather_rows(weight, ids_dev)

    @staticmethod
    def backward(ctx, dx):
        rows_dev, off_dev, uniq_dev, _ = ctx.csr
        seg = ops.segment_sum_rows(dx.contiguous(), rows_dev, off_dev)
        if ctx.sink is not None:
            ctx.sink.add_sparse(ctx.weight, uniq_dev, seg)
            return None, None, None, None, None
        dW = torch.zeros(ctx.shape, dtype=dx.dtype, device=dx.device)
        ops.scatter_rows_(dW, uniq_dev, seg)
        return dW, None, None, None, None


class NormHeadCEFn(torch.autograd.Function):

    @staticmethod
    def forward(ctx, h, lm_w, norm_w, eps, valid_rows_dev, targets_dev, n_valid):
        hn = ops.rmsnorm(h, norm_w, eps)
        if n_valid == 0:
            ctx.n = 0
            ctx.save_for_backward(h, norm_w)
            ctx.eps = eps
            return torch.zeros((), device=h.device, dtype=torch.float32), hn
        hv = ops.gather_rows(hn, valid_rows_dev)
        logits = ops.gemm(hv, lm_w)
        row_loss, dlogits = ops.cross_entropy_rows(logits, targets_dev, want_grad=True, grad_scale=1.0 / n_valid)
        ctx.save_for_backward(h, lm_w, norm_w, hv, dlogits, valid_rows_dev)
        ctx.eps, ctx.n = eps, n_valid
        return row_loss.sum() / n_valid, hn

    @staticmethod
    def backward(ctx, gloss, ghn):
        if ctx.n == 0:
            h, norm_w = ctx.saved_tensors
            with torch.no_grad():
                dh = ops.rmsnorm_bwd(h, norm_w, ghn.contiguous() if ghn is not None else torch.zeros_like(h), ctx.eps)
            return dh, None, None, None, None, None, None
        h, lm_w, norm_w, hv, dlogits, rows = ctx.saved_tensors
        n = ctx.n
        with torch.no_grad():
            dlogits = (dlogits.float() * gloss).to(dlogits.dtype)
            dW = None
            if lm_w.requires_grad:
                from ..parallel.ddp import dense_grad_out_for
                dW = ops.gemm_tn(dlogits, hv, out=dense_grad_out_for(lm_w))
            n8 = (n + 7) // 8 * 8
            dl = dlogits
            if n8 != n:
                dl = torch.zeros((n8, dlogits.shape[1]), dtype=dlogits.dtype, device=dlogits.device)
                dl[:n] = dlogits
            dhv = ops.gemm_tn(ops.transpose(dl), lm_w.detach())[:n].contiguous()
            dhn = ghn.contiguous().clone() if ghn is not None else torch.zeros_like(h)
            dhn_rows = ops.add(ops.gather_rows(dhn, rows), dhv)
            ops.scatter_rows_(dhn, rows, dhn_rows)
            dh = ops.rmsnorm_bwd(h, norm_w, dhn, ctx.eps)
        return dh, dW, None, None, None, None, None


def lm_train_forward(model, x, pos3, cu, max_len, labels_np, am_cur, flat_keep, lens, plan=None):
    tm = model.model
    cos, sin = tm.mrope_tables(pos3)
    lora_refresh(tm.layers)
    for li, layer in enumerate(tm.layers):
        at = layer.self_attn
        lq, lv = _lora_parts(at.q_proj), _lora_parts(at.v_proj)
        pq, pv = _lora_dropout(at)
        seeds = (next_dropout_seed(li, 0), next_dropout_seed(li, 1, advance=False)) if (pq > 0.0 or pv > 0.0) else None
        x = DecoderLayerFn.apply(x, lq[0] if lq else None, lq[1] if lq else None, lv[0] if lv else None, lv[1] if lv else None, layer, cos, sin,
                                 cu, max_len, seeds)
    plan = plan if plan is not None else {}
    if "train_targets" not in plan:
        B, S = labels_np.shape
        nxt = np.full((B, S), -100, dtype=np.int64)
        nxt[:, :-1] = labels_np[:, 1:]
        tgt = nxt.reshape(-1)[flat_keep]
        valid = np.flatnonzero(tgt != -100)
        dev = x.device
        plan["train_targets"] = (upload(valid.astype(np.int64), dev), upload(tgt[valid], dev), int(valid.size))
    valid_dev, tgt_dev, n_valid = plan["train_targets"]
    loss, hn = NormHeadCEFn.apply(x, model.lm_head.weight, tm.norm.weight, tm.norm.variance_epsilon, valid_dev, tgt_dev, n_valid)
    return loss, hn
```

Before: 7.788.

## Fuse SwiGLU backward into down-proj GEMM and inverse RoPE into attention backward

Adds a GEMM epilogue that reads the saved gate/up activations and writes the SwiGLU gradient directly from the down-projection transpose GEMM, so the intermediate da tensor and the separate swiglu_bwd pass are no longer needed. It also folds the inverse rotary embedding into the attention backward epilogues (dq, dk and the split dk/dv reduce), which removes the separate rope_ pass over dqkv and the cached negated-sin table. Both changes cut memory round trips in the decoder backward. In exchange, the GEMM epilogue does extra gu loads and permlane shuffles that may affect register pressure, and the rope path only covers D=128.

```diff
diff --git a/include/rga3_hip.h b/include/rga3_hip.h
--- a/include/rga3_hip.h
+++ b/include/rga3_hip.h
@@ -29,6 +29,8 @@
                        int64_t norm_width, float eps, uint64_t* row_sumsq_out, void* stream);
 int rga3_gemm_swiglu_pre_bf16(const void* A, const void* W, const void* bias, void* C, void* pre, int64_t M, int64_t N, int64_t K, int64_t lda, int64_t ldw,
                               int64_t ldc, int64_t ldpre, int tile, void* workspace, int64_t workspace_bytes, void* stream);
+int rga3_gemm_swiglu_bwd_bf16(const void* dY, const void* Wt, const void* gu, void* dgu, int64_t M, int64_t N, int64_t K, int64_t lda, int64_t ldw,
+                              int64_t ldgu, int64_t lddgu, int tile, void* workspace, int64_t workspace_bytes, void* stream);
 int rga3_gemm_cat_bf16(const void* A, const void* W, const void* bias, void* C, int64_t M, int64_t N, int64_t K, int64_t lda, int64_t ldw, int64_t ldc,
                        const void* A2, const void* W2, int64_t K2, int64_t lda2, int64_t ldw2, const void* Wn, void* Cn, int64_t N2, int64_t ldwn, int64_t ldcn,
                        int tile, void* stream);
@@ -110,6 +112,10 @@
                          void* dk, void* dv, float* delta_ws, const int32_t* cu_q, const int32_t* cu_k, int nseg, int max_q,
                          int max_k, int64_t total_q, int Hq, int Hkv, int D, const int64_t* strides16, float scale, int causal,
                          float* dkv_ws, int64_t total_k, void* stream);
+int rga3_attn_varlen_bwd_rope(const void* q, const void* k, const void* v, const void* o, const void* dout, const float* lse, void* dq,
+                              void* dk, void* dv, float* delta_ws, const int32_t* cu_q, const int32_t* cu_k, int nseg, int max_q,
+                              int max_k, int64_t total_q, int Hq, int Hkv, int D, const int64_t* strides16, float scale, int causal,
+                              float* dkv_ws, int64_t total_k, const float* cos, const float* sin, void* stream);
 int rga3_hiera_mlp144(const void* x, const void* w1f, const float* c1, const void* d1, const void* w2, const void* b2, void* y, int64_t M, float eps, void* stream);
 int64_t rga3_hiera_mlp288_pack_bytes(void);
 int rga3_hiera_mlp288_pack(const void* w1f, const float* c1, const void* d1, const void* w2, void* pack, void* stream);
diff --git a/rga3-release_amd/csrc/attn_bwd.hip b/rga3-release_amd/csrc/attn_bwd.hip
--- a/rga3-release_amd/csrc/attn_bwd.hip
+++ b/rga3-release_amd/csrc/attn_bwd.hip
@@ -19,12 +19,27 @@
     float* dkv_ws;
     long total_k;
     int gx, gy;
+    const float *rope_cos = nullptr, *rope_sin = nullptr;
 };
 
+template <int DP>
+__device__ __forceinline__ void unrope_quads(const float* cr, const float* sr, int dd, const f32x4& a, const f32x4& b, f32x4& oa, f32x4& ob) {
+    const f32x4 c1 = *(const f32x4*)(cr + dd), s1 = *(const f32x4*)(sr + dd), c2 = *(const f32x4*)(cr + dd + DP / 2), s2 = *(const f32x4*)(sr + dd + DP / 2);
+    oa = a * c1 + b * s1;
+    ob = b * c2 - a * s2;
+}
+__device__ __forceinline__ u32x2 pack_quad(const f32x4& v) {
+    u32x2 pk;
+    pk[0] = pack_bf2(v[0], v[1]);
+    pk[1] = pack_bf2(v[2], v[3]);
+    return pk;
+}
+
 constexpr int BT = 64;
 
-template <int DP, int QT, int NWAVE, bool PAIR>
+template <int DP, int QT, int NWAVE, bool PAIR, bool ROPE = false>
 __global__ __launch_bounds__(64 * NWAVE) void attn_bwd_dq_kernel(AttnBwdArgs p) {
+    static_assert(!ROPE || DP == 128, "the rotary fold is built for the decoder's head size");
     constexpr int NT = 64 * NWAVE;
     constexpr int BLOCK_M = NWAVE * QT * 16;
     constexpr int CH = DP / 8;
@@ -205,6 +220,19 @@
         const int qi = qw0 + t * 16 + c;
         if (qi < Lq) {
             unsigned short* row = p.dq + (long)(qs + qi) * p.dq_st + (long)hq * p.dq_sh;
+            if constexpr (ROPE) {
+                const float* cr = p.rope_cos + (long)(qs + qi) * DP;
+                const float* sr = p.rope_sin + (long)(qs + qi) * DP;
+#pragma unroll
+                for (int d = 0; d < DT / 2; ++d) {
+                    const int dd = d * 16 + 4 * g;
+                    f32x4 oa, ob;
+                    unrope_quads<DP>(cr, sr, dd, dqacc[t][d], dqacc[t][d + DT / 2], oa, ob);
+                    *(u32x2*)(row + dd) = pack_quad(oa);
+                    *(u32x2*)(row + dd + DP / 2) = pack_quad(ob);
+                }
+                continue;
+            }
 #pragma unroll
             for (int d = 0; d < DT; ++d) {
                 const int dd = d * 16 + 4 * g;
@@ -220,8 +248,9 @@
     }
 }
 
-template <int DP, int NWAVE, bool SPLIT, bool PAIR>
+template <int DP, int NWAVE, bool SPLIT, bool PAIR, bool ROPE = false>
 __global__ __launch_bounds__(64 * NWAVE) void attn_bwd_dkv_kernel(AttnBwdArgs p) {
+    static_assert(!ROPE || (DP == 128 && !SPLIT), "the rotary fold is built for the decoder's head size; the split form rotates in attn_dkv_reduce_kernel");
     constexpr int NT = 64 * NWAVE;
     constexpr int BLOCK_N = NWAVE * 16;
     constexpr int CH = DP / 8;
@@ -397,6 +426,21 @@
     if (key < Lk) {
         unsigned short* rk = p.dk + (long)(ks + key) * p.dk_st + (long)hk * p.dk_sh;
         unsigned short* rv = p.dv + (long)(ks + key) * p.dv_st + (long)hk * p.dv_sh;
+        if constexpr (ROPE) {
+            const float* cr = p.rope_cos + (long)(ks + key) * DP;
+            const float* sr = p.rope_sin + (long)(ks + key) * DP;
+#pragma unroll
+            for (int d = 0; d < DT / 2; ++d) {
+                const int dd = d * 16 + 4 * g;
+                f32x4 oa, ob;
+                unrope_quads<DP>(cr, sr, dd, dkacc[d], dkacc[d + DT / 2], oa, ob);
+                *(u32x2*)(rk + dd) = pack_quad(oa);
+                *(u32x2*)(rk + dd + DP / 2) = pack_quad(ob);
+                *(u32x2*)(rv + dd) = pack_quad(dvacc[d]);
+                *(u32x2*)(rv + dd + DP / 2) = pack_quad(dvacc[d + DT / 2]);
+            }
+            continue;
+        }
 #pragma unroll
         for (int d = 0; d < DT; ++d) {
             const int dd = d * 16 + 4 * g;
@@ -436,7 +480,37 @@
     *(u32x2*)(p.dv + key * p.dv_st + (long)hk * p.dv_sh + dd) = b;
 }
 
-template <int DP>
+__global__ __launch_bounds__(256) void attn_dkv_reduce_rope_kernel(AttnBwdArgs p) {
+    constexpr int DP = 128;
+    const int group = p.Hq / p.Hkv;
+    constexpr int d8 = DP / 8;
+    const long idx = (long)blockIdx.x * 256 + threadIdx.x;
+    const long total = p.total_k * p.Hkv * d8;
+    if (idx >= total) return;
+    const int dd = (int)(idx % d8) * 4;
+    const long row = idx / d8;
+    const int hk = (int)(row % p.Hkv);
+    const long key = row / p.Hkv;
+    const long plane = p.total_k * p.Hkv * (long)DP, half = (long)group * plane;
+    const float* w = p.dkv_ws + row * DP + dd;
+    f32x4 ka = *(const f32x4*)w, kb = *(const f32x4*)(w + DP / 2), va = *(const f32x4*)(w + half), vb = *(const f32x4*)(w + half + DP / 2);
+    for (int h = 1; h < group; ++h) {
+        ka += *(const f32x4*)(w + h * plane);
+        kb += *(const f32x4*)(w + h * plane + DP / 2);
+        va += *(const f32x4*)(w + half + h * plane);
+        vb += *(const f32x4*)(w + half + h * plane + DP / 2);
+    }
+    f32x4 oa, ob;
+    unrope_quads<DP>(p.rope_cos + key * DP, p.rope_sin + key * DP, dd, ka, kb, oa, ob);
+    unsigned short* rk = p.dk + key * p.dk_st + (long)hk * p.dk_sh + dd;
+    unsigned short* rv = p.dv + key * p.dv_st + (long)hk * p.dv_sh + dd;
+    *(u32x2*)rk = pack_quad(oa);
+    *(u32x2*)(rk + DP / 2) = pack_quad(ob);
+    *(u32x2*)rv = pack_quad(va);
+    *(u32x2*)(rv + DP / 2) = pack_quad(vb);
+}
+
+template <int DP, bool ROPE = false>
 static int launch_bwd(const AttnBwdArgs& a0, int nseg, int max_q, int max_k, hipStream_t st) {
     AttnBwdArgs a = a0;
     a.gx = 1; a.gy = 1;
@@ -465,12 +539,12 @@
     const unsigned nqb = (unsigned)cdiv(max_q, BLOCK_M), nkb = (unsigned)cdiv(max_k, 16 * NW);
     const bool pair = a.causal && nqb >= 4 && nkb >= 4;
     if (pair) {
-        auto kq = attn_bwd_dq_kernel<DP, QT, NWQ, true>;
+        auto kq = attn_bwd_dq_kernel<DP, QT, NWQ, true, ROPE>;
         if (int rc = prep((const void*)kq, LDS_DQ)) return rc;
         a.gx = (int)((nqb + 1) / 2); a.gy = a.Hq;
         hipLaunchKernelGGL(kq, dim3((unsigned)a.gx * (unsigned)a.gy * (unsigned)nseg), dim3(64 * NWQ), LDS_DQ, st, a);
     } else {
-        auto kq = attn_bwd_dq_kernel<DP, QT, NWQ, false>;
+        auto kq = attn_bwd_dq_kernel<DP, QT, NWQ, false, ROPE>;
         if (int rc = prep((const void*)kq, LDS_DQ)) return rc;
         a.gx = (int)nqb; a.gy = a.Hq;
         hipLaunchKernelGGL(kq, dim3((unsigned)a.gx * (unsigned)a.gy * (unsigned)nseg), dim3(64 * NWQ), LDS_DQ, st, a);
@@ -491,17 +565,18 @@
         }
         RGA3_CHECK_LAUNCH("attn_bwd_dkv_kernel<split>");
         const long rows = a.total_k * a.Hkv;
-        hipLaunchKernelGGL(attn_dkv_reduce_kernel, dim3((unsigned)cdiv(rows * (a.D / 4), 256)), dim3(256), 0, st, a);
+        if constexpr (ROPE) hipLaunchKernelGGL(attn_dkv_reduce_rope_kernel, dim3((unsigned)cdiv(rows * (DP / 8), 256)), dim3(256), 0, st, a);
+        else hipLaunchKernelGGL(attn_dkv_reduce_kernel, dim3((unsigned)cdiv(rows * (a.D / 4), 256)), dim3(256), 0, st, a);
         RGA3_CHECK_LAUNCH("attn_dkv_reduce_kernel");
         return 0;
     }
     if (pair) {
-        auto kk = attn_bwd_dkv_kernel<DP, NW, false, true>;
+        auto kk = attn_bwd_dkv_kernel<DP, NW, false, true, ROPE>;
         if (int rc = prep((const void*)kk, LDS_DKV)) return rc;
         a.gx = (int)gx; a.gy = a.Hkv;
         hipLaunchKernelGGL(kk, dim3((unsigned)a.gx * (unsigned)a.gy * (unsigned)nseg), dim3(64 * NW), LDS_DKV, st, a);
     } else {
-        auto kk = attn_bwd_dkv_kernel<DP, NW, false, false>;
+        auto kk = attn_bwd_dkv_kernel<DP, NW, false, false, ROPE>;
         if (int rc = prep((const void*)kk, LDS_DKV)) return rc;
         a.gx = (int)gx; a.gy = a.Hkv;
         hipLaunchKernelGGL(kk, dim3((unsigned)a.gx * (unsigned)a.gy * (unsigned)nseg), dim3(64 * NW), LDS_DKV, st, a);
@@ -514,10 +589,10 @@
 
 using namespace rga3;
 
-extern "C" int rga3_attn_varlen_bwd(const void* q, const void* k, const void* v, const void* o, const void* dout, const float* lse,
-                                    void* dq, void* dk, void* dv, float* delta_ws, const int32_t* cu_q, const int32_t* cu_k, int nseg,
-                                    int max_q, int max_k, int64_t total_q, int Hq, int Hkv, int D, const int64_t* strides16, float scale,
-                                    int causal, float* dkv_ws, int64_t total_k, void* stream) {
+static int attn_bwd_impl(const void* q, const void* k, const void* v, const void* o, const void* dout, const float* lse,
+                         void* dq, void* dk, void* dv, float* delta_ws, const int32_t* cu_q, const int32_t* cu_k, int nseg,
+                         int max_q, int max_k, int64_t total_q, int Hq, int Hkv, int D, const int64_t* strides16, float scale,
+                         int causal, float* dkv_ws, int64_t total_k, const float* rope_cos, const float* rope_sin, void* stream) {
     RGA3_CHECK_ARG(q && k && v && o && dout && lse && dq && dk && dv && delta_ws && cu_q && cu_k && strides16, "attn_bwd: null pointer");
     RGA3_CHECK_ARG(nseg > 0 && max_q > 0 && max_k > 0 && total_q > 0, "attn_bwd: sizes");
     RGA3_CHECK_ARG(Hq > 0 && Hkv > 0 && Hq % Hkv == 0, "attn_bwd: Hq=%d Hkv=%d", Hq, Hkv);
@@ -533,10 +608,31 @@
     a.dk_st = strides16[12]; a.dk_sh = strides16[13]; a.dv_st = strides16[14]; a.dv_sh = strides16[15];
     a.Hq = Hq; a.Hkv = Hkv; a.D = D; a.total_q = total_q; a.scale = scale; a.scale_log2 = scale * 1.4426950408889634f; a.causal = causal;
     a.dkv_ws = dkv_ws; a.total_k = total_k;
+    a.rope_cos = rope_cos; a.rope_sin = rope_sin;
     RGA3_CHECK_ARG(!dkv_ws || (total_k > 0 && D % 4 == 0), "attn_bwd: dkv_ws needs total_k");
     hipStream_t st = (hipStream_t)stream;
+    if (rope_cos) return launch_bwd<128, true>(a, nseg, max_q, max_k, st);
     if (D <= 32) return launch_bwd<32>(a, nseg, max_q, max_k, st);
     if (D <= 64) return launch_bwd<64>(a, nseg, max_q, max_k, st);
     if (D <= 96) return launch_bwd<96>(a, nseg, max_q, max_k, st);
     return launch_bwd<128>(a, nseg, max_q, max_k, st);
 }
+
+extern "C" int rga3_attn_varlen_bwd(const void* q, const void* k, const void* v, const void* o, const void* dout, const float* lse,
+                                    void* dq, void* dk, void* dv, float* delta_ws, const int32_t* cu_q, const int32_t* cu_k, int nseg,
+                                    int max_q, int max_k, int64_t total_q, int Hq, int Hkv, int D, const int64_t* strides16, float scale,
+                                    int causal, float* dkv_ws, int64_t total_k, void* stream) {
+    return attn_bwd_impl(q, k, v, o, dout, lse, dq, dk, dv, delta_ws, cu_q, cu_k, nseg, max_q, max_k, total_q, Hq, Hkv, D, strides16, scale, causal, dkv_ws, total_k,
+                         nullptr, nullptr, stream);
+}
+
+extern "C" int rga3_attn_varlen_bwd_rope(const void* q, const void* k, const void* v, const void* o, const void* dout, const float* lse,
+                                         void* dq, void* dk, void* dv, float* delta_ws, const int32_t* cu_q, const int32_t* cu_k, int nseg,
+                                         int max_q, int max_k, int64_t total_q, int Hq, int Hkv, int D, const int64_t* strides16, float scale,
+                                         int causal, float* dkv_ws, int64_t total_k, const float* cos, const float* sin, void* stream) {
+    RGA3_CHECK_ARG(cos && sin && ((((uintptr_t)cos | (uintptr_t)sin) & 15) == 0), "attn_bwd_rope: cos / sin tables must be given and 16-byte aligned");
+    RGA3_CHECK_ARG(D == 128, "attn_bwd_rope: head dim %d (the rotary fold is built for D = 128; use rga3_attn_varlen_bwd + rga3_rope_inplace)", D);
+    RGA3_CHECK_ARG(total_k == total_q, "attn_bwd_rope: total_k %ld != total_q %ld (queries and keys share the rows of the tables)", (long)total_k, (long)total_q);
+    return attn_bwd_impl(q, k, v, o, dout, lse, dq, dk, dv, delta_ws, cu_q, cu_k, nseg, max_q, max_k, total_q, Hq, Hkv, D, strides16, scale, causal, dkv_ws, total_k,
+                         cos, sin, stream);
+}
diff --git a/rga3-release_amd/csrc/gemm_bf16.hip b/rga3-release_amd/csrc/gemm_bf16.hip
--- a/rga3-release_amd/csrc/gemm_bf16.hip
+++ b/rga3-release_amd/csrc/gemm_bf16.hip
@@ -8,6 +8,7 @@
 
 
 enum { ACT_NONE = 0, ACT_GELU = 1, ACT_SWIGLU = 2, ACT_RELU = 3 };
+constexpr int ACT_SWIGLU_BWD = 4;
 
 struct GemmArgs {
     const unsigned short* A;
@@ -42,6 +43,8 @@
     void* Cn = nullptr;
     long ldwn = 0, ldcn = 0;
     int N2 = 0;
+    const unsigned short* gu = nullptr;
+    long ldgu = 0;
 };
 
 constexpr float kRowSumFix = 1048576.0f;
@@ -110,7 +113,8 @@
                                               int wm, int wn, const f32x4* part1 = nullptr, const f32x4* part2 = nullptr, const char* resl = nullptr,
                                               float poison = 0.f, int nwn = 1) {
     constexpr bool LNF = LNM == 1, LNP = LNM == 2;
-    static_assert(!(LNM != 0 && ACT == ACT_SWIGLU), "the LayerNorm-folded epilogues have no SwiGLU form");
+    static_assert(!(LNM != 0 && (ACT == ACT_SWIGLU || ACT == ACT_SWIGLU_BWD)), "the LayerNorm-folded epilogues have no SwiGLU form");
+    static_assert(!(ACT == ACT_SWIGLU_BWD && OUT_F32), "the SwiGLU-backward epilogue writes bf16");
     static_assert(!(LNP && (OUT_F32 || PARTS)), "the LayerNorm-sum producer writes bf16 from the single-pass kernels");
     constexpr int PD = 1;
     f32x4 pn[PD][NTL];
@@ -209,6 +213,18 @@
             }
         }
     }
+    u32x4 gun[(ACT == ACT_SWIGLU_BWD) ? 2 : 1][(ACT == ACT_SWIGLU_BWD) ? NTL : 1];
+    const int sb_col = 2 * (n0 + wn * WTN) + ((lane >> 4) & 1) * 16 + (lane >> 5) * 8;
+    auto load_gu = [&](int i) {
+        const int row = m0 + wm * WTM + i * 16 + (lane & 15);
+#pragma unroll
+        for (int j = 0; j < NTL; ++j) {
+            u32x4 v = {0u, 0u, 0u, 0u};
+            if (row < p.M && sb_col + 32 * j < 2 * p.N) v = *(const u32x4*)(p.gu + (long)row * p.ldgu + sb_col + 32 * j);
+            gun[i & 1][j] = v;
+        }
+    };
+    if constexpr (ACT == ACT_SWIGLU_BWD) load_gu(0);
     if (resl) asm volatile("s_waitcnt vmcnt(0)" ::: "memory");
 #pragma unroll
     for (int i = 0; i < MT; ++i) {
@@ -244,6 +260,27 @@
             for (int j = 0; j < NTL; ++j)
                 x[j] += f32x4{__uint_as_float(bpk[j][0] << 16), __uint_as_float(bpk[j][0] & 0xffff0000u), __uint_as_float(bpk[j][1] << 16),
                               __uint_as_float(bpk[j][1] & 0xffff0000u)};
+        }
+        if constexpr (ACT == ACT_SWIGLU_BWD) {
+            if (i + 1 < MT) load_gu(i + 1);
+            const int row = m0 + wm * WTM + i * 16 + (lane & 15);
+#pragma unroll
+            for (int j = 0; j < NTL; ++j) {
+                const u32x4 gv = gun[i & 1][j];
+                const auto t0 = __builtin_amdgcn_permlane16_swap(gv[0], gv[2], false, false);
+                const auto t1 = __builtin_amdgcn_permlane16_swap(gv[1], gv[3], false, false);
+                const f32x2 g01 = widen_bf2((unsigned)t0[0]), u01 = widen_bf2((unsigned)t0[1]), g23 = widen_bf2((unsigned)t1[0]), u23 = widen_bf2((unsigned)t1[1]);
+                float dg[4], du[4];
+                swiglu_bwd_elem(g01[0], u01[0], x[j][0], dg[0], du[0]);
+                swiglu_bwd_elem(g01[1], u01[1], x[j][1], dg[1], du[1]);
+                swiglu_bwd_elem(g23[0], u23[0], x[j][2], dg[2], du[2]);
+                swiglu_bwd_elem(g23[1], u23[1], x[j][3], dg[3], du[3]);
+                const auto q0 = __builtin_amdgcn_permlane16_swap(pack_bf2(dg[0], dg[1]), pack_bf2(du[0], du[1]), false, false);
+                const auto q1 = __builtin_amdgcn_permlane16_swap(pack_bf2(dg[2], dg[3]), pack_bf2(du[2], du[3]), false, false);
+                const u32x4 ov = {(unsigned)q0[0], (unsigned)q1[0], (unsigned)q0[1], (unsigned)q1[1]};
+                if (row < p.M && sb_col + 32 * j < 2 * p.N) *(u32x4*)((unsigned short*)p.C + (long)row * p.ldc + sb_col + 32 * j) = ov;
+            }
+            continue;
         }
         f32x4 v[OUT_NT];
 #pragma unroll
@@ -2405,6 +2442,25 @@
     }
 }
 
+static bool swiglu_bwd_tile_ok(int tile) {
+    return tile == 3 || tile == 12 || tile == 20 || tile == 21 || tile == 22 || tile == 26 || tile == 27 || tile == 31 || tile == 32;
+}
+static int launch_swiglu_bwd(const GemmArgs& a, int tile, hipStream_t st) {
+    constexpr int ACT = ACT_SWIGLU_BWD;
+    switch (tile) {
+        case 3: return launch_cfg<128, 256, 2, 4, ACT, false, 0>(a, st);
+        case 12: return launch_cfg<128, 128, 2, 2, ACT, false, 0>(a, st);
+        case 20: return launch_pp<ACT, false>(a, st);
+        case 21: return launch_sk<ACT, false>(a, false, st);
+        case 22: return launch_sk<ACT, false>(a, true, st);
+        case 26: return launch_sk<ACT, false>(a, true, st, true);
+        case 27: return launch_sk<ACT, false>(a, false, st, true);
+        case 31: return launch_sk<ACT, false, 3>(a, false, st);
+        case 32: return launch_sk<ACT, false, 3>(a, true, st);
+        default: return fail(-1, "gemm_swiglu_bwd: tile %d has no SwiGLU-backward epilogue", tile);
+    }
+}
+
 }
 
 using namespace rga3;
@@ -2527,6 +2583,26 @@
     RGA3_CHECK_ARG(pre, "gemm_swiglu_pre: null pre-activation output");
     return gemm_bf16_impl(A, W, bias, nullptr, nullptr, C, M, N, K, lda, ldw, ldc, 0, ACT_SWIGLU, RGA3_BF16, tile, workspace, workspace_bytes, nullptr, 0, 0.f, nullptr, stream, pre,
                           ldpre);
+}
+
+extern "C" int rga3_gemm_swiglu_bwd_bf16(const void* dY, const void* Wt, const void* gu, void* dgu, int64_t M, int64_t N, int64_t K, int64_t lda, int64_t ldw,
+                                         int64_t ldgu, int64_t lddgu, int tile, void* workspace, int64_t workspace_bytes, void* stream) {
+    RGA3_CHECK_ARG(dY && Wt && gu && dgu, "gemm_swiglu_bwd: null pointer");
+    RGA3_CHECK_ARG(M > 4 && N > 0 && K > 0 && N % 16 == 0 && K % 8 == 0, "gemm_swiglu_bwd: bad shape M=%ld N=%ld K=%ld (M > 4, N %% 16, K %% 8)", (long)M, (long)N, (long)K);
+    RGA3_CHECK_ARG(lda % 8 == 0 && ldw % 8 == 0 && lda >= K && ldw >= K, "gemm_swiglu_bwd: lda/ldw must be multiples of 8 elements, at least K");
+    RGA3_CHECK_ARG(ldgu % 8 == 0 && lddgu % 8 == 0 && ldgu >= 2 * N && lddgu >= 2 * N, "gemm_swiglu_bwd: ldgu/lddgu must be multiples of 8 elements, at least 2 N");
+    RGA3_CHECK_ARG((((uintptr_t)dY | (uintptr_t)Wt | (uintptr_t)gu | (uintptr_t)dgu) & 15) == 0, "gemm_swiglu_bwd: pointers must be 16-byte aligned");
+    RGA3_CHECK_ARG(tile == -1 || swiglu_bwd_tile_ok(tile), "gemm_swiglu_bwd: tile %d (3 / 12 / 20 / 21 / 22 / 26 / 27 / 31 / 32)", tile);
+    RGA3_CHECK_ARG(M * lda < (1LL << 32) && N * ldw < (1LL << 32), "gemm_swiglu_bwd: operands must be < 2^32 elements (32-bit staging offsets)");
+    GemmArgs a;
+    a.A = (const unsigned short*)dY; a.W = (const unsigned short*)Wt; a.C = dgu;
+    a.bias = nullptr; a.res = nullptr; a.colscale = nullptr;
+    a.M = (int)M; a.N = (int)N; a.K = (int)K;
+    a.lda = lda; a.ldw = ldw; a.ldc = lddgu; a.ldr = 0;
+    a.ws = workspace; a.ws_bytes = workspace_bytes; a.ksl = 0; a.rowstat = nullptr; a.colc = nullptr;
+    a.gu = (const unsigned short*)gu; a.ldgu = ldgu;
+    if (tile == -1) tile = pick_tile((int)M, (int)N, (int)K, false, -1) == 20 ? 20 : 12;
+    return launch_swiglu_bwd(a, tile, (hipStream_t)stream);
 }
 
 extern "C" int rga3_gemm_cat_bf16(const void* A, const void* W, const void* bias, void* C, int64_t M, int64_t N, int64_t K, int64_t lda, int64_t ldw, int64_t ldc,
diff --git a/rga3-release_amd/rga3/hip/lib.py b/rga3-release_amd/rga3/hip/lib.py
--- a/rga3-release_amd/rga3/hip/lib.py
+++ b/rga3-release_amd/rga3/hip/lib.py
@@ -17,6 +17,7 @@
     "rga3_gemm_tn_bf16": [_p, _p, _p, _p, _i64, _i64, _i64, _i64, _i64, _i64, _i, _p, _i64, _p, _p],
     "rga3_gemm_tn_many": [_p, _p, _i, _p, _i64, _p],
     "rga3_gemm_swiglu_pre_bf16": [_p, _p, _p, _p, _p, _i64, _i64, _i64, _i64, _i64, _i64, _i64, _i, _p, _i64, _p],
+    "rga3_gemm_swiglu_bwd_bf16": [_p, _p, _p, _p, _i64, _i64, _i64, _i64, _i64, _i64, _i64, _i, _p, _i64, _p],
     "rga3_gemm_cat_bf16": [_p, _p, _p, _p, _i64, _i64, _i64, _i64, _i64, _i64, _p, _p, _i64, _i64, _i64, _p, _p, _i64, _i64, _i64, _i, _p],
     "rga3_attn_varlen_fwd": [_p, _p, _p, _p, _p, _p, _p, _i, _i, _i64, _i, _i, _i, _i64, _i64, _i64, _i64, _i64, _i64,
                              _i64, _i64, _f, _i, _i, _p, _i64, _i, _i, _i, _p],
@@ -52,6 +53,7 @@
     "rga3_bce_dice_sums_ws_floats": [_i64, _i64],
     "rga3_bce_dice_sums_det": [_p, _p, _p, _p, _i64, _i64, _i64, _p],
     "rga3_attn_varlen_bwd": [_p, _p, _p, _p, _p, _p, _p, _p, _p, _p, _p, _p, _i, _i, _i, _i64, _i, _i, _i, _p, _f, _i, _p, _i64, _p],
+    "rga3_attn_varlen_bwd_rope": [_p, _p, _p, _p, _p, _p, _p, _p, _p, _p, _p, _p, _i, _i, _i, _i64, _i, _i, _i, _p, _f, _i, _p, _i64, _p, _p, _p],
     "rga3_transpose16_many": [_p, _p, _i, _p],
     "rga3_hiera_mlp144": [_p, _p, _p, _p, _p, _p, _p, _i64, _f, _p],
     "rga3_hiera_mlp288_pack_bytes": [],
diff --git a/rga3-release_amd/rga3/hip/ops.py b/rga3-release_amd/rga3/hip/ops.py
--- a/rga3-release_amd/rga3/hip/ops.py
+++ b/rga3-release_amd/rga3/hip/ops.py
@@ -78,12 +78,41 @@
 _LNSUM_TILES = (20, 3, 5, 12, 13, 23)
 
 
+_SWIGLU_BWD_TILES = (3, 12, 20, 21, 22, 26, 27, 31, 32)
+
+
+def _gemm_swiglu_bwd(a, w, gu, out, tile):
+    _need_cuda(a, w, gu, out)
+    M, K = a.shape
+    N = w.shape[0]
+    assert gu.dtype == torch.bfloat16 and gu.shape == (M, 2 * N) and gu.stride(1) == 1 and N % 16 == 0 and M > 4 and K % 8 == 0
+    if out is None:
+        out = torch.empty((M, 2 * N), dtype=torch.bfloat16, device=a.device)
+    assert out.dtype == torch.bfloat16 and out.shape == (M, 2 * N) and out.stride(1) == 1
+    ws = gemm_workspace(a.device)
+    fn = _lib.load().rga3_gemm_swiglu_bwd_bf16
+
+    def run(t):
+        _lib.check(fn(a.data_ptr(), w.data_ptr(), gu.data_ptr(), out.data_ptr(), M, N, K, a.stride(0), w.stride(0), gu.stride(0), out.stride(0), t,
+                      ws.data_ptr(), ws.numel(), _stream()), "gemm_swiglu_bwd_bf16")
+
+    if tile == -1 and M * N * K >= (1 << 24):
+        tile = _tuner.pick(_tuner.key_of(M, N, K, "swiglu_bwd", BF16, False, False), run, candidates=tuple(t for t in _tuner.CANDIDATES if t in _SWIGLU_BWD_TILES))
+    if tile != -1 and tile not in _SWIGLU_BWD_TILES:
+        tile = -1
+    run(tile)
+    return out
+
+
 def gemm(a: torch.Tensor, w: torch.Tensor, bias=None, residual=None, act: str = "none", out_dtype=torch.bfloat16,
-         out=None, tile: int = -1, colscale=None, rms_in=None, rms_out=None) -> torch.Tensor:
+         out=None, tile: int = -1, colscale=None, rms_in=None, rms_out=None, swiglu_bwd_gu=None) -> torch.Tensor:
     _need_cuda(a, w, bias, residual, out, colscale)
     assert a.dtype == torch.bfloat16 and w.dtype == torch.bfloat16
     assert a.dim() == 2 and w.dim() == 2 and a.shape[1] == w.shape[1], (a.shape, w.shape)
     assert a.stride(1) == 1 and w.stride(1) == 1
+    if swiglu_bwd_gu is not None:
+        assert bias is None and residual is None and act == "none" and colscale is None and rms_in is None and rms_out is None and out_dtype == torch.bfloat16
+        return _gemm_swiglu_bwd(a, w, swiglu_bwd_gu, out, tile)
     M, K = a.shape
     N = w.shape[0]
     if K % 8 != 0 or a.stride(0) % 8 != 0 or w.stride(0) % 8 != 0:
@@ -870,7 +899,7 @@
     return out
 
 
-def attn_varlen_bwd(q, k, v, o, dout, lse, cu_q, cu_k, max_q: int, max_k: int, scale: float, causal: bool, dq=None, dk=None, dv=None):
+def attn_varlen_bwd(q, k, v, o, dout, lse, cu_q, cu_k, max_q: int, max_k: int, scale: float, causal: bool, dq=None, dk=None, dv=None, rope=None):
     import ctypes
     _need_cuda(q, k, v, o, dout, lse)
     Tq, Hq, D = q.shape
@@ -885,10 +914,25 @@
     dkv_ws = torch.empty((2 * Hq * Tk * D,), dtype=torch.float32, device=q.device) if (Hq > Hkv and D % 4 == 0) else None
     st = (ctypes.c_int64 * 16)(q.stride(0), q.stride(1), k.stride(0), k.stride(1), v.stride(0), v.stride(1), o.stride(0), o.stride(1),
                                dout.stride(0), dout.stride(1), dq.stride(0), dq.stride(1), dk.stride(0), dk.stride(1), dv.stride(0), dv.stride(1))
+    if rope is not None:
+        cos, sin = rope
+        _need_cuda(cos, sin)
+        assert cos.dtype == sin.dtype == torch.float32 and cos.is_contiguous() and sin.is_contiguous() and cos.shape == sin.shape == (Tq, D) and Tk == Tq
+        if D == 128:
+            rc = _lib.load().rga3_attn_varlen_bwd_rope(q.data_ptr(), k.data_ptr(), v.data_ptr(), o.data_ptr(), dout.data_ptr(), lse.data_ptr(), dq.data_ptr(),
+                                                       dk.data_ptr(), dv.data_ptr(), delta.data_ptr(), cu_q.data_ptr(), cu_k.data_ptr(), cu_q.numel() - 1, int(max_q),
+                                                       int(max_k), Tq, Hq, Hkv, D, ctypes.cast(st, ctypes.c_void_p), float(scale), int(bool(causal)), _ptr(dkv_ws), Tk,
+                                                       cos.data_ptr(), sin.data_ptr(), _stream())
+            _lib.check(rc, "attn_varlen_bwd_rope")
+            return dq, dk, dv
     rc = _lib.load().rga3_attn_varlen_bwd(q.data_ptr(), k.data_ptr(), v.data_ptr(), o.data_ptr(), dout.data_ptr(), lse.data_ptr(), dq.data_ptr(),
                                           dk.data_ptr(), dv.data_ptr(), delta.data_ptr(), cu_q.data_ptr(), cu_k.data_ptr(), cu_q.numel() - 1, int(max_q),
                                           int(max_k), Tq, Hq, Hkv, D, ctypes.cast(st, ctypes.c_void_p), float(scale), int(bool(causal)), _ptr(dkv_ws), Tk, _stream())
     _lib.check(rc, "attn_varlen_bwd")
+    if rope is not None:
+        nsin = (-sin).contiguous()
+        rope_(dq, cos, nsin, 0, Hq)
+        rope_(dk, cos, nsin, 0, Hkv)
     return dq, dk, dv
 
 
diff --git a/rga3-release_amd/rga3/model/qwen_train.py b/rga3-release_amd/rga3/model/qwen_train.py
--- a/rga3-release_amd/rga3/model/qwen_train.py
+++ b/rga3-release_amd/rga3/model/qwen_train.py
@@ -91,15 +91,18 @@
 _fp8_tap = [None]
 
 
-def _fgemm(x, owner, key, srcs, build, bias=None, residual=None, out=None):
+def _fgemm(x, owner, key, srcs, build, bias=None, residual=None, out=None, swiglu_bwd_gu=None):
     if _fp8["on"] and x.shape[1] % 128 == 0:
         q, sc = _fp8_pack(owner, key, *srcs, build=build)
         xq, xs = ops.quant_fp8_rows(x)
         if _fp8_tap[0] is not None:
             _fp8_tap[0](key, xq, xs)
-        return ops.gemm_fp8(xq, xs, q, sc, bias=bias, residual=residual, out=out)
+        y = ops.gemm_fp8(xq, xs, q, sc, bias=bias, residual=residual, out=out)
+        return y if swiglu_bwd_gu is None else ops.swiglu_bwd(swiglu_bwd_gu, y)
     w = _wt(owner, key, *srcs, build=build)
-    return ops.gemm(x, w, bias, residual=residual, out=out)
+    if swiglu_bwd_gu is not None and x.shape[0] <= 4:
+        return ops.swiglu_bwd(swiglu_bwd_gu, ops.gemm(x, w, bias, residual=residual, out=out))
+    return ops.gemm(x, w, bias, residual=residual, out=out, swiglu_bwd_gu=swiglu_bwd_gu)
 
 
 def _fgemm_q(xq, xs, owner, key, srcs, build, bias=None, residual=None, out=None):
@@ -354,17 +357,6 @@
     return y, (h1, qkv, att, lse, x1, h2, gu, tq, tv, hq_in, hv_in)
 
 
-_neg = {}
-
-
-def _neg_table(sin):
-    key = (sin.data_ptr(), sin._version, tuple(sin.shape))
-    if _neg.get("key") != key:
-        _neg["key"], _neg["t"] = key, (-sin).contiguous()
-        _neg["src"] = sin
-    return _neg["t"]
-
-
 class DecoderLayerFn(torch.autograd.Function):
 
     @staticmethod
@@ -420,23 +412,22 @@
                 h2 = ops.rmsnorm(x1, w2.weight, w2.variance_epsilon)
                 gu = _fgemm(h2, mlp, "wgu", (mlp.gate_proj.weight, mlp.up_proj.weight), lambda: wgu, bias=bgu)
             q, k, v = qkv[:, :Hq], qkv[:, Hq:Hq + Hk], qkv[:, Hq + Hk:]
-            da = _fgemm(dy, mlp, "wd_t", (mlp.down_proj.weight,), lambda: ops.transpose(wd))
             if _fp8_fused(gu.shape[1]):
+                da = _fgemm(dy, mlp, "wd_t", (mlp.down_proj.weight,), lambda: ops.transpose(wd))
                 dq, dsc = ops.swiglu_bwd_quant(gu, da)
                 del gu, da
                 dh2 = _fgemm_q(dq, dsc, mlp, "wgu_t", (mlp.gate_proj.weight, mlp.up_proj.weight), lambda: ops.transpose(wgu))
                 del dq
             else:
-                dgu = ops.swiglu_bwd(gu, da)
-                del gu, da
+                dgu = _fgemm(dy, mlp, "wd_t", (mlp.down_proj.weight,), lambda: ops.transpose(wd), swiglu_bwd_gu=gu)
+                del gu
                 dh2 = _fgemm(dgu, mlp, "wgu_t", (mlp.gate_proj.weight, mlp.up_proj.weight), lambda: ops.transpose(wgu))
                 del dgu
             dx1 = ops.rmsnorm_bwd(x1, w2.weight, dh2, w2.variance_epsilon, add=dy)
             datt = _fgemm(dx1, at, "wo_t", (at.o_proj.weight,), lambda: ops.transpose(at.o_proj.weight.detach())).view(T, Hq, D)
             dqkv = torch.empty_like(qkv)
             ops.attn_varlen_bwd(q, k, v, att, datt, lse, cu, cu, max_len, max_len, D ** -0.5, True, dq=dqkv[:, :Hq], dk=dqkv[:, Hq:Hq + Hk],
-                                dv=dqkv[:, Hq + Hk:])
-            ops.rope_(dqkv, cos, _neg_table(sin), 0, Hq + Hk)
+                                dv=dqkv[:, Hq + Hk:], rope=(cos, sin))
             dqkv2 = dqkv.view(T, (Hq + 2 * Hk) * D)
             fold = (not _fp8["on"]) and T > 16 and _lora_cat_ok(at)
             dtt = None
```

Result: no change. 7.736 (-0.7%).
